# SunYangtian/UniGeo

Hardware: AMD Instinct MI355X
Metric: frames/sec (384x512, 25-frame clip, 25 denoise steps) (higher is better)
Workload: dtype fp16; 1 GPU; DepthCrafter SVD-UNet fp16, 25-step Euler, 25-frame 384x512 clips (BASELINE configs[1]); CLIP + VAE enc/dec + depth post-proc inside the timed region; one clip per ug_dc_run call, one call at a time (SURVEY 8d; reference eval.py:33-39); frames=25, height=384, width=512, denoise_steps=25, parallelism=clip-sharded x1, RCCL all_gather of depth, clips_in_flight_per_gpu=1, lanes=1

## Files before the change

### unigeo_amd/_lib.py

```python
import ctypes as C
import dataclasses
import json
import os

import numpy as np

_HERE = os.path.dirname(os.path.abspath(__file__))
LIB_PATH = os.environ.get("UG_LIB_PATH") or os.path.join(_HERE, "csrc", "libunigeo_hip.so")

EXPORTS = [
    "ug_unet_config_default", "ug_vae_config_default", "ug_clip_config_default",
    "ug_create", "ug_destroy", "ug_last_error", "ug_workspace_peak",
    "ug_load_tensor", "ug_bind_unet", "ug_bind_vae", "ug_bind_clip",
    "ug_dc_set_inputs", "ug_dc_run", "ug_dc_run_windows", "ug_dc_get_outputs", "ug_dc_device_ptrs", "ug_dc_set_trace", "ug_dc_set_guidance", "ug_unet_forward_pair", "ug_dc_set_inputs_ex", "ug_dc_get_noise", "ug_op_philox_u32", "ug_op_randn", "ug_op_u8_to_frames", "ug_set_vae_encode_fp32", "ug_set_concurrency", "ug_set_coscheduled", "ug_set_fp8_linears", "ug_op_linear_mx8", "ug_set_ff_fused", "ug_op_ff", "ug_op_ln_ff", "ug_bench_ff", "ug_bench_flash", "ug_tune_flash", "ug_tune_ff",
    "ug_eval_depth", "ug_eval_normal", "ug_depth_eval_opts_default", "ug_eval_depth_ex", "ug_op_masked_median", "ug_clip_embed", "ug_vae_encode", "ug_vae_decode", "ug_unet_forward", "ug_normals_from_depth",
    "ug_op_linear", "ug_op_conv", "ug_op_conv_gn", "ug_op_groupnorm", "ug_op_layernorm", "ug_op_flash_attn",
    "ug_op_temporal_attn", "ug_op_attention_generic", "ug_op_flash_attn_dh", "ug_op_euler_step",
    "ug_bind_stablenormal", "ug_sn_run", "ug_sn_unet_forward", "ug_sn_dino", "ug_sn_vae_decode", "ug_sn_vae_encode", "ug_resize_bilinear",
    "ug_profile_begin", "ug_profile_begin_shapes", "ug_profile_end", "ug_bench_gemm", "ug_bench_groupnorm", "ug_bench_mfma_peak", "ug_tune_force",
]


class UNetConfigC(C.Structure):
    _fields_ = [("in_channels", C.c_int), ("out_channels", C.c_int), ("num_levels", C.c_int),
                ("block_out_channels", C.c_int * 8), ("num_attention_heads", C.c_int * 8),
                ("down_has_attn", C.c_int * 8),
                ("layers_per_block", C.c_int), ("cross_attention_dim", C.c_int),
                ("addition_time_embed_dim", C.c_int), ("projection_class_embeddings_input_dim", C.c_int),
                ("norm_groups", C.c_int),
                ("eps_cross_attn_blocks", C.c_float), ("eps_plain_down_block", C.c_float),
                ("eps_mid_block", C.c_float), ("eps_up_blocks", C.c_float)]


class VAEConfigC(C.Structure):
    _fields_ = [("in_channels", C.c_int), ("out_channels", C.c_int), ("latent_channels", C.c_int),
                ("num_levels", C.c_int), ("block_out_channels", C.c_int * 8),
                ("layers_per_block", C.c_int), ("norm_groups", C.c_int), ("scaling_factor", C.c_float)]


class CLIPConfigC(C.Structure):
    _fields_ = [("hidden_size", C.c_int), ("intermediate_size", C.c_int), ("num_hidden_layers", C.c_int),
                ("num_attention_heads", C.c_int), ("image_size", C.c_int), ("patch_size", C.c_int),
                ("projection_dim", C.c_int), ("layer_norm_eps", C.c_float)]


class DepthEvalOptsC(C.Structure):
    _fields_ = [("alignment", C.c_int), ("max_depth", C.c_float), ("pre_clip_min", C.c_float), ("pre_clip_max", C.c_float),
                ("post_clip_min", C.c_float), ("post_clip_max", C.c_float)]


DEPTH_ALIGNMENTS = {"lstsq": 0, "median": 1, "scale": 2, "metric": 3}

_lib = None


def load_library():
    global _lib
    if _lib is not None:
        return _lib
    if not os.path.exists(LIB_PATH):
        raise RuntimeError(
            f"{LIB_PATH} not found: build it with `python -c 'import __graft_entry__ as g; g.build()'` "
            "(or `make -C unigeo_amd/csrc`).  The MI355X path has no CPU / PyTorch fallback.")
    lib = C.CDLL(LIB_PATH)
    fp, ip, vp = C.POINTER(C.c_float), C.c_int, C.c_void_p
    lib.ug_create.restype = vp
    lib.ug_create.argtypes = [ip, C.c_size_t, C.c_size_t]
    lib.ug_destroy.argtypes = [vp]
    lib.ug_last_error.restype = C.c_char_p
    lib.ug_last_error.argtypes = [vp]
    lib.ug_workspace_peak.restype = C.c_size_t
    lib.ug_workspace_peak.argtypes = [vp]
    lib.ug_load_tensor.argtypes = [vp, C.c_char_p, ip, ip, C.POINTER(C.c_int64), vp]
    lib.ug_bind_unet.argtypes = [vp, C.POINTER(UNetConfigC)]
    lib.ug_bind_vae.argtypes = [vp, C.POINTER(VAEConfigC)]
    lib.ug_bind_clip.argtypes = [vp, C.POINTER(CLIPConfigC)]
    lib.ug_dc_set_inputs.argtypes = [vp, vp, ip, ip, ip, vp, vp, vp]
    lib.ug_dc_run.argtypes = [vp, ip, ip, ip]
    lib.ug_dc_run_windows.argtypes = [vp, ip, ip, ip, ip, ip]
    lib.ug_dc_get_outputs.argtypes = [vp, vp, vp, vp]
    lib.ug_dc_set_trace.argtypes = [vp, vp, ip]
    lib.ug_set_vae_encode_fp32.argtypes = [vp, ip]
    try:
        lib.ug_set_fp8_linears.argtypes = [vp, ip]
        lib.ug_set_concurrency.argtypes = [vp, ip]
        lib.ug_set_coscheduled.argtypes = [vp, ip]
        lib.ug_set_ff_fused.argtypes = [vp, ip]
        lib.ug_bench_ff.argtypes = [vp, ip, ip, ip, ip, vp]
        lib.ug_bench_flash.argtypes = [vp, ip, ip, ip, ip, ip, vp]
        lib.ug_tune_flash.argtypes = [vp, ip]
        lib.ug_tune_ff.argtypes = [vp, ip]
        lib.ug_op_ff.argtypes = [vp, vp, ip, ip, vp, vp, vp, vp, vp, C.c_float, C.c_float, ip, vp]
        lib.ug_op_ln_ff.argtypes = [vp, vp, ip, ip, vp, vp, C.c_float, vp, ip, vp, vp, vp, vp, C.c_float, C.c_float, ip, vp]
        lib.ug_op_linear_mx8.argtypes = [vp, vp, ip, ip, vp, ip, vp, ip, vp, vp, vp]
    except AttributeError:
        if not os.environ.get("UG_LIB_PATH"):
            raise
    lib.ug_dc_device_ptrs.argtypes = [vp, C.POINTER(vp), C.POINTER(vp), C.POINTER(vp)]
    lib.ug_eval_depth.argtypes = [vp, vp, vp, vp, C.c_long, C.c_float, vp]
    lib.ug_eval_normal.argtypes = [vp, vp, vp, vp, C.c_long, vp]
    lib.ug_depth_eval_opts_default.restype = None
    lib.ug_depth_eval_opts_default.argtypes = [C.POINTER(DepthEvalOptsC)]
    lib.ug_eval_depth_ex.argtypes = [vp, vp, vp, vp, C.c_long, C.POINTER(DepthEvalOptsC), vp, vp]
    lib.ug_op_masked_median.argtypes = [vp, vp, vp, C.c_long, C.c_float, C.c_float, C.c_float, vp, C.POINTER(C.c_long)]
    lib.ug_clip_embed.argtypes = [vp, vp, ip, ip, ip, vp]
    lib.ug_vae_encode.argtypes = [vp, vp, ip, ip, ip, vp]
    lib.ug_vae_decode.argtypes = [vp, vp, ip, ip, ip, vp]
    lib.ug_unet_forward.argtypes = [vp, vp, ip, ip, ip, C.c_float, vp, vp]
    try:
        lib.ug_dc_set_guidance.argtypes = [vp, C.c_float]
        lib.ug_unet_forward_pair.argtypes = [vp, vp, vp, vp, vp, ip, ip, ip, C.c_float, vp, vp]
    except AttributeError:
        if not os.environ.get("UG_LIB_PATH"):
            raise
    try:
        lib.ug_dc_set_inputs_ex.argtypes = [vp, vp, ip, ip, ip, ip, vp, vp, C.c_uint64, vp]
        lib.ug_dc_get_noise.argtypes = [vp, vp, vp]
        lib.ug_op_philox_u32.argtypes = [vp, C.c_uint64, C.c_uint32, C.c_uint64, C.c_long, vp]
        lib.ug_op_randn.argtypes = [vp, C.c_uint64, C.c_uint32, C.c_uint64, C.c_long, C.c_long, vp]
        lib.ug_op_u8_to_frames.argtypes = [vp, vp, ip, ip, ip, vp]
    except AttributeError:
        if not os.environ.get("UG_LIB_PATH"):
            raise
    lib.ug_normals_from_depth.argtypes = [vp, vp, vp, ip, ip, ip, vp]
    lib.ug_op_linear.argtypes = [vp, vp, ip, ip, vp, ip, vp, vp, C.c_float, C.c_float, ip, ip, vp]
    lib.ug_op_conv.argtypes = [vp, vp, ip, vp, ip, ip, ip, ip, vp, vp, ip, ip, ip, ip, ip, ip, ip, vp]
    lib.ug_op_groupnorm.argtypes = [vp, vp, ip, vp, ip, ip, ip, ip, C.c_float, ip, ip, vp, vp, vp]
    lib.ug_op_conv_gn.argtypes = [vp, vp, ip, ip, ip, ip, vp, vp, vp, ip, ip, ip, ip, C.c_float, ip, vp, vp, vp, vp, vp, vp]
    lib.ug_op_layernorm.argtypes = [vp, vp, ip, ip, C.c_float, vp, vp, vp, ip, vp, vp]
    lib.ug_op_flash_attn.argtypes = [vp, vp, ip, ip, ip, vp]
    lib.ug_op_temporal_attn.argtypes = [vp, vp, ip, ip, ip, vp]
    lib.ug_op_attention_generic.argtypes = [vp, vp, ip, ip, ip, ip, vp]
    lib.ug_op_flash_attn_dh.argtypes = [vp, vp, ip, ip, ip, ip, vp]
    lib.ug_op_euler_step.argtypes = [vp, vp, vp, C.c_long, C.c_float, C.c_float]
    lib.ug_bind_stablenormal.argtypes = [vp, C.POINTER(UNetConfigC), C.POINTER(VAEConfigC), C.POINTER(CLIPConfigC)]
    lib.ug_sn_run.argtypes = [vp, vp, ip, ip, ip, vp, C.c_float, ip, vp, vp, vp, vp]
    lib.ug_sn_unet_forward.argtypes = [vp, ip, vp, vp, ip, ip, ip, C.c_float, C.c_float, vp, vp, ip, vp]
    lib.ug_sn_dino.argtypes = [vp, vp, ip, ip, ip, vp]
    lib.ug_sn_vae_decode.argtypes = [vp, vp, ip, ip, ip, vp]
    lib.ug_sn_vae_encode.argtypes = [vp, vp, ip, ip, ip, vp]
    lib.ug_resize_bilinear.argtypes = [vp, vp, ip, ip, ip, ip, ip, ip, ip, vp]
    lib.ug_profile_begin.argtypes = [vp]
    lib.ug_bench_gemm.argtypes = [vp] + [ip] * 16 + [vp]
    lib.ug_bench_groupnorm.argtypes = [vp, ip, ip, ip, ip, ip, ip, ip, vp]
    lib.ug_tune_force.argtypes = [vp, ip, ip]
    lib.ug_profile_begin_shapes.argtypes = [vp]
    lib.ug_profile_end.restype = C.c_char_p
    lib.ug_profile_end.argtypes = [vp]
    _lib = lib
    return lib


def _f32(a):
    return np.ascontiguousarray(a, dtype=np.float32)


def _ptr(a):
    return None if a is None else a.ctypes.data_as(C.c_void_p)


def _fill8(dst, vals):
    for i in range(8):
        dst[i] = int(vals[i]) if i < len(vals) else 0


class Engine:

    def __init__(self, device_id=0, workspace_bytes=2 << 30, persist_bytes=1 << 30):
        self.lib = load_library()
        self.ctx = self.lib.ug_create(int(device_id), int(workspace_bytes), int(persist_bytes))
        if not self.ctx:
            raise RuntimeError("ug_create failed: " + self.lib.ug_last_error(None).decode())
        self.device_id = device_id

    def close(self):
        if getattr(self, "ctx", None):
            self.lib.ug_destroy(self.ctx)
            self.ctx = None

    def __del__(self):
        try:
            self.close()
        except Exception:
            pass

    def _ck(self, rc):
        if rc != 0:
            raise RuntimeError("libunigeo_hip: " + self.lib.ug_last_error(self.ctx).decode())

    def load_state(self, prefix, state):
        for name, arr in state.items():
            a = np.ascontiguousarray(arr)
            if a.dtype == np.float16:
                dt = 0
            elif a.dtype == np.float32:
                dt = 1
            else:
                a = a.astype(np.float32); dt = 1
            shape = (C.c_int64 * max(a.ndim, 1))(*(a.shape if a.ndim else (1,)))
            self._ck(self.lib.ug_load_tensor(self.ctx, (prefix + name).encode(), dt, max(a.ndim, 1), shape, _ptr(a)))

    def bind_unet(self, cfg):
        c = UNetConfigC()
        c.in_channels, c.out_channels = cfg.in_channels, cfg.out_channels
        c.num_levels = len(cfg.block_out_channels)
        _fill8(c.block_out_channels, cfg.block_out_channels)
# ... 274 lines not shown
        k = _f32(intrinsics).reshape(T, 3, 3)
        out = np.empty((T, H, W, 3), np.float32)
        self._ck(self.lib.ug_normals_from_depth(self.ctx, _ptr(d), _ptr(k), T, H, W, _ptr(out)))
        return out

    DEPTH_KEYS = ["Abs Rel", "Sq Rel", "RMSE", "Log RMSE", "delta < 1.", "delta < 1.25", "delta < 1.25^2", "delta < 1.25^3"]
    NORMAL_KEYS = ["normal mean", "normal median", "normal rmse", "angle < 5", "angle < 7.5", "angle < 11.25", "angle < 22.5", "angle < 30"]

    def eval_depth(self, gt, mask=None, pred=None, max_depth=80.0, alignment="lstsq", pre_clip_min=None, pre_clip_max=None,
                   post_clip_min=None, post_clip_max=None, return_error_map=False):
        if alignment not in DEPTH_ALIGNMENTS:
            raise ValueError(f"alignment must be one of {sorted(DEPTH_ALIGNMENTS)}, not {alignment!r}")
        g = _f32(gt); n = g.size
        p = None if pred is None else _f32(pred)
        m = None if mask is None else np.ascontiguousarray(np.asarray(mask).astype(np.uint8))
        out = np.zeros(11, np.float64)
        clips = (pre_clip_min, pre_clip_max, post_clip_min, post_clip_max)
        emap = None
        if alignment == "lstsq" and max_depth is not None and not return_error_map and all(c is None for c in clips):
            self._ck(self.lib.ug_eval_depth(self.ctx, _ptr(p), _ptr(g), _ptr(m), n, float(max_depth), _ptr(out)))
        else:
            o = DepthEvalOptsC(DEPTH_ALIGNMENTS[alignment], float("nan") if max_depth is None else float(max_depth),
                               *[float("nan") if c is None else float(c) for c in clips])
            emap = np.empty(g.shape, np.float32) if return_error_map else None
            self._ck(self.lib.ug_eval_depth_ex(self.ctx, _ptr(p), _ptr(g), _ptr(m), n, C.byref(o), _ptr(out), _ptr(emap)))
        res = dict(zip(self.DEPTH_KEYS, out[:8].tolist()))
        res["valid_pixels"] = int(out[8])
        if return_error_map:
            return res, (float(out[9]), float(out[10])), emap
        return res, (float(out[9]), float(out[10]))

    def op_masked_median(self, pred, gt, max_depth=80.0, pre_clip_min=None, pre_clip_max=None):
        p, g = _f32(pred).reshape(-1), _f32(gt).reshape(-1)
        med = np.zeros(2, np.float32); cnt = C.c_long(0)
        nan = float("nan")
        self._ck(self.lib.ug_op_masked_median(self.ctx, _ptr(p), _ptr(g), p.size, nan if max_depth is None else float(max_depth),
                                              nan if pre_clip_min is None else float(pre_clip_min),
                                              nan if pre_clip_max is None else float(pre_clip_max), _ptr(med), C.byref(cnt)))
        return med[0], med[1], int(cnt.value)

    def eval_normal(self, gt, mask=None, pred=None):
        g = _f32(gt); n = g.size // 3
        p = None if pred is None else _f32(pred)
        m = None if mask is None else np.ascontiguousarray(np.asarray(mask).astype(np.uint8))
        out = np.zeros(8, np.float64)
        self._ck(self.lib.ug_eval_normal(self.ctx, _ptr(p), _ptr(g), _ptr(m), n, _ptr(out)))
        return dict(zip(self.NORMAL_KEYS, out.tolist()))

    def op_linear(self, A, W, bias=None, R1=None, c0=1.0, c1=1.0, act=0, geglu=False):
        A, W = _f32(A), _f32(W); M, K = A.shape; N = W.shape[0]
        b = None if bias is None else _f32(bias); r = None if R1 is None else _f32(R1)
        out = np.empty((M, N // 2 if geglu else N), np.float32)
        self._ck(self.lib.ug_op_linear(self.ctx, _ptr(A), M, K, _ptr(W), N, _ptr(b), _ptr(r), c0, c1, act, int(geglu), _ptr(out)))
        return out

    def op_conv(self, x0, weight, bias=None, x1=None, kt=1, k=3, stride=1, pad_t=1, pad_l=1, ups=1):
        x0 = _f32(x0); T, H, W, C0 = x0.shape
        x1a = None if x1 is None else _f32(x1); C1 = 0 if x1 is None else x1a.shape[-1]
        w = _f32(weight); O = w.shape[0]
        b = None if bias is None else _f32(bias)
        Ho, Wo = H * ups // stride, W * ups // stride
        out = np.empty((T, Ho, Wo, O), np.float32)
        self._ck(self.lib.ug_op_conv(self.ctx, _ptr(x0), C0, _ptr(x1a), C1, T, H, W, _ptr(w), _ptr(b), O, kt, k,
                                     stride, pad_t, pad_l, ups, _ptr(out)))
        return out

    def op_groupnorm(self, x0, G, eps, gamma, beta, x1=None, temporal=False, silu=False):
        x0 = _f32(x0); T, HW, C0 = x0.shape
        x1a = None if x1 is None else _f32(x1); C1 = 0 if x1 is None else x1a.shape[-1]
        out = np.empty((T, HW, C0 + C1), np.float32)
        self._ck(self.lib.ug_op_groupnorm(self.ctx, _ptr(x0), C0, _ptr(x1a), C1, T, HW, G, eps, int(temporal), int(silu),
                                          _ptr(_f32(gamma)), _ptr(_f32(beta)), _ptr(out)))
        return out

    def op_conv_gn(self, x, w, b, G, eps, gamma, beta, res=None, kt=1, k=3, temporal=False):
        x = _f32(x); T, H, W, C0 = x.shape; w = _f32(w); O = w.shape[0]
        r = None if res is None else _f32(res)
        co = np.empty((T, H, W, O), np.float32); y1 = np.empty_like(co); y2 = np.empty_like(co)
        rb = C.c_int(0)
        self._ck(self.lib.ug_op_conv_gn(self.ctx, _ptr(x), C0, T, H, W, _ptr(w), _ptr(None if b is None else _f32(b)), _ptr(r), O, kt, k, G, eps, int(temporal),
                                        _ptr(_f32(gamma)), _ptr(_f32(beta)), _ptr(co), _ptr(y1), _ptr(y2), C.byref(rb)))
        return co, y1, y2, rb.value

    def op_layernorm(self, x, eps, gamma, beta, addvec=None, rows_per_vec=1):
        x = _f32(x); M, Cc = x.shape
        out = np.empty((M, Cc), np.float32); xout = np.empty((M, Cc), np.float32)
        av = None if addvec is None else _f32(addvec)
        self._ck(self.lib.ug_op_layernorm(self.ctx, _ptr(x), M, Cc, eps, _ptr(_f32(gamma)), _ptr(_f32(beta)), _ptr(av),
                                          rows_per_vec, _ptr(out), _ptr(xout)))
        return (out, xout) if addvec is not None else out

    def op_flash_attn(self, qkv, B, H, S):
        q = _f32(qkv); out = np.empty((B * S, H * 64), np.float32)
        self._ck(self.lib.ug_op_flash_attn(self.ctx, _ptr(q), B, H, S, _ptr(out)))
        return out

    def op_temporal_attn(self, qkv, T, HW, H):
        q = _f32(qkv); out = np.empty((T * HW, H * 64), np.float32)
        self._ck(self.lib.ug_op_temporal_attn(self.ctx, _ptr(q), T, HW, H, _ptr(out)))
        return out

    def op_attention_generic(self, qkv, B, S, H, d):
        q = _f32(qkv); out = np.empty((B * S, H * d), np.float32)
        self._ck(self.lib.ug_op_attention_generic(self.ctx, _ptr(q), B, S, H, d, _ptr(out)))
        return out

    def op_flash_attn_dh(self, qkv, B, S, H, d):
        q = _f32(qkv); out = np.empty((B * S, H * d), np.float32)
        self._ck(self.lib.ug_op_flash_attn_dh(self.ctx, _ptr(q), B, S, H, d, _ptr(out)))
        return out

    def op_euler_step(self, v, lat, sigma, sigma_next):
        v = _f32(v); l = _f32(lat).copy()
        self._ck(self.lib.ug_op_euler_step(self.ctx, _ptr(v), _ptr(l), l.size, sigma, sigma_next))
        return l

    def bench_gemm(self, M=0, N=0, K=0, conv=None, cfg=-1, split=0, iters=20):
        out = np.zeros(8, np.float32)
        cv = conv or {}
        self._ck(self.lib.ug_bench_gemm(self.ctx, M, N, K, int(conv is not None), cv.get("T", 0), cv.get("H", 0), cv.get("W", 0),
                                        cv.get("C0", 0), cv.get("C1", 0), cv.get("kt", 1), cv.get("k", 1), cv.get("stride", 1),
                                        cv.get("ups", 1), cfg, split, iters, _ptr(out)))
        Mr, Kr = float(out[3]), float(out[4])
        return float(out[0]), 2.0 * Mr * N * Kr / (out[0] * 1e-3) / 1e12, int(out[1]), int(out[2])

    def bench_mfma_peak(self, iters=20000):
        out = np.zeros(1, np.float32)
        self.lib.ug_bench_mfma_peak.argtypes = [C.c_void_p, C.c_int, C.c_void_p]
        self._ck(self.lib.ug_bench_mfma_peak(self.ctx, int(iters), _ptr(out)))
        return float(out[0])

    def tune_force(self, cfg=-1, split=-1):
        self._ck(self.lib.ug_tune_force(self.ctx, int(cfg), int(split)))

    def bench_groupnorm(self, C0, C1, T, HW, temporal, mode, iters=20):
        out = np.zeros(1, np.float32)
        self._ck(self.lib.ug_bench_groupnorm(self.ctx, C0, C1, T, HW, int(temporal), mode, iters, _ptr(out)))
        return float(out[0])

    def profile_begin(self, shapes=False):
        self._ck((self.lib.ug_profile_begin_shapes if shapes else self.lib.ug_profile_begin)(self.ctx))

    def profile_end(self):
        prof = json.loads(self.lib.ug_profile_end(self.ctx).decode())
        self.last_profile_order = prof.pop("__order__", None)
        return prof

    def workspace_peak(self):
        return int(self.lib.ug_workspace_peak(self.ctx))
```

### unigeo_amd/csrc/capi.hip

```cpp
#include <math.h>
#include <stdlib.h>
#include <string.h>

#include <algorithm>
#include <cmath>
#include <vector>

#include "../../include/unigeo_hip.h"
#include "../../include/unigeo_hip_test.h"
#include "engine.h"

using namespace ug;

struct ug_ctx { Ctx c; };
static std::string g_create_err;

#define UG_TRY(ctx, ...)                                   \
  if (!(ctx)) return -1;                                   \
  try { UG_CHECK(hipSetDevice((ctx)->c.device)); __VA_ARGS__; return 0; } \
  catch (const std::exception& e) { (ctx)->c.err = e.what(); (void)hipGetLastError(); return 1; } \
  catch (...) { (ctx)->c.err = "unknown error"; return 2; }

extern "C" {

// ... 761 lines not shown
    f16* dO = c.ws.get<f16>((long)M * nout);
    GemmP p; memset(&p, 0, sizeof(p));
    p.A0 = (const f16*)a8; p.C0 = K; p.M = M; p.N = N; p.K = K; p.W = (const f16*)w8; p.ldw = K; p.bias = db; p.c0 = 1.f;
    p.Out = dO; p.ldo = nout; p.flags = geglu ? UG_F_GEGLU : 0; p.zero = c.zero; p.nb_inner = 1;
    p.sa = sa; p.ld_sa = ld_sa; p.sw = sw; p.ld_sw = ld_sw;
    gemm_apply_tune(p, c.tune);
    launch_gemm_mx8(p, c.stream);
    down16(c, dO, out, (long)M * nout);
    if (a8_out) UG_CHECK(hipMemcpy(a8_out, a8, (size_t)M * K, hipMemcpyDeviceToHost));
    if (sa_out) UG_CHECK(hipMemcpy(sa_out, sa, (size_t)(K / 128) * ld_sa * 4, hipMemcpyDeviceToHost));
  });
}

int ug_op_conv(ug_ctx* x, const float* x0, int C0, const float* x1, int C1, int T, int H, int W, const float* weight,
               const float* bias, int O, int kt, int k, int stride, int pad_t, int pad_l, int ups, float* out) {
  UG_TRY(x, {
    Ctx& c = x->c; Scope sc(c);
    const int I = C0 + C1, taps = kt * k * k;
    std::vector<float> wp((size_t)O * taps * I);
    const bool kch = (I % 64 == 0) && taps > 1 && !getenv("UG_NO_KCHUNK");
    for (int o = 0; o < O; ++o) for (int i = 0; i < I; ++i) for (int tp = 0; tp < taps; ++tp)
      wp[kch ? (((size_t)o * (I / 64) + i / 64) * taps + tp) * 64 + i % 64 : ((size_t)o * taps + tp) * I + i] = weight[((size_t)o * I + i) * taps + tp];
    const long px = (long)T * H * W;
    f16* d0 = up16(c, x0, px * C0); f16* d1 = C1 ? up16(c, x1, px * C1) : nullptr;
    f16* dW = up16(c, wp.data(), (long)wp.size()); f16* db = up16_opt(c, bias, O);
    const int Ho = H * ups / stride, Wo = W * ups / stride;
    f16* dO = c.ws.get<f16>((long)T * Ho * Wo * O);
    GemmP p; memset(&p, 0, sizeof(p));
    p.conv = 1; p.A0 = d0; p.A1 = d1; p.C0 = C0; p.C1 = C1; p.T = T; p.Hi = H; p.Wi = W; p.Ho = Ho; p.Wo = Wo;
    p.ups = ups; p.stride = stride; p.pad_t = pad_t; p.pad_l = pad_l; p.kt = kt; p.ky = k; p.kx = k;
    p.M = T * Ho * Wo; p.N = O; p.K = I * taps; p.W = dW; p.ldw = p.K; p.bias = db; p.c0 = 1.f;
    p.Out = dO; p.ldo = O; p.zero = c.zero; p.nb_inner = 1; p.kchunk = kch;
    gemm_apply_tune(p, c.tune);
    { int cf, sp; gemm_plan(p, 1, &cf, &sp); p.cfg_p1 = cf + 1; p.splitk = sp; if (sp > 1) p.partial = c.ws.get<float>((long)sp * p.M * p.N); }
    launch_gemm(p, 1, c.stream);
    down16(c, dO, out, (long)T * Ho * Wo * O);
  });
}

int ug_op_conv_gn(ug_ctx* x, const float* x0, int C0, int T, int H, int W, const float* weight, const float* bias, const float* res, int O, int kt, int k,
                  int G, float eps, int temporal, const float* gamma, const float* beta, float* conv_out, float* y_pass, float* y_epi, int* rb_out) {
  UG_TRY(x, {
    Ctx& c = x->c; Scope sc(c);
    const int I = C0, taps = kt * k * k;
    UG_REQUIRE(I % 64 == 0, "ug_op_conv_gn: channels must be a multiple of 64");
    std::vector<float> wp((size_t)O * taps * I);
    for (int o = 0; o < O; ++o) for (int i = 0; i < I; ++i) for (int tp = 0; tp < taps; ++tp)
      wp[(((size_t)o * (I / 64) + i / 64) * taps + tp) * 64 + i % 64] = weight[((size_t)o * I + i) * taps + tp];
    const long M = (long)T * H * W;
    f16* d0 = up16(c, x0, M * C0); f16* dW = up16(c, wp.data(), (long)wp.size()); f16* db = up16_opt(c, bias, O);
    f16* dR = up16_opt(c, res, M * O);
    f16* dg = up16(c, gamma, O); f16* dbt = up16(c, beta, O);
    f16* o1 = c.ws.get<f16>(M * O); f16* o2 = c.ws.get<f16>(M * O); f16* y1 = c.ws.get<f16>(M * O); f16* y2 = c.ws.get<f16>(M * O);
    float2* part = (float2*)c.ws.get<float>(((M + 47) / 48) * (long)O * 2);
    int rb = 0;
    for (int pass = 0; pass < 2; ++pass) {
      GemmP p; memset(&p, 0, sizeof(p));
      p.conv = 1; p.A0 = d0; p.C0 = C0; p.T = T; p.Hi = H; p.Wi = W; p.Ho = H; p.Wo = W;
      p.ups = 1; p.stride = 1; p.pad_t = k / 2; p.pad_l = k / 2; p.kt = kt; p.ky = k; p.kx = k;
      p.M = (int)M; p.N = O; p.K = I * taps; p.W = dW; p.ldw = p.K; p.bias = db; p.c0 = 1.f; p.R1 = dR; p.ldr1 = O; p.c1 = 1.f;
      p.Out = pass ? o2 : o1; p.ldo = O; p.zero = c.zero; p.nb_inner = 1; p.kchunk = taps > 1;
      gemm_apply_tune(p, c.tune);
      const size_t mk = c.ws.mark();
      { int cf, sp; gemm_plan(p, 1, &cf, &sp); p.cfg_p1 = cf + 1; p.splitk = sp; if (sp > 1) p.partial = c.ws.get<float>((long)sp * p.M * p.N); }
      if (pass) { p.stat_part = part; p.stat_hw = H * W; launch_gemm(p, 1, c.stream, &rb); } else launch_gemm(p, 1, c.stream);
      c.ws.release(mk);
      GroupNormP g; memset(&g, 0, sizeof(g));
      g.X0 = pass ? o2 : o1; g.C0 = O; g.T = T; g.HW = H * W; g.G = G; g.eps = eps; g.temporal = temporal; g.silu = 1; g.gamma = dg; g.beta = dbt;
      g.Y = pass ? y2 : y1; g.ws = c.ws.get<float>((long)groupnorm_ws_floats(T, H * W, O, G));
      if (pass && rb > 0) { g.part = part; g.part_rb = rb; }
      const bool used = launch_groupnorm(g, c.stream);
      if (pass && !used) rb = 0;
      c.ws.release(mk);
    }
    *rb_out = rb;
    down16(c, o1, conv_out, M * O);
    std::vector<float> tmp((size_t)M * O);
    down16(c, o2, tmp.data(), M * O);
    UG_REQUIRE(memcmp(tmp.data(), conv_out, tmp.size() * 4) == 0, "ug_op_conv_gn: the statistics epilogue changed the convolution's output");
    down16(c, y1, y_pass, M * O); down16(c, y2, y_epi, M * O);
  });
}

int ug_op_groupnorm(ug_ctx* x, const float* x0, int C0, const float* x1, int C1, int T, int HW, int G, float eps,
                    int temporal, int silu, const float* gamma, const float* beta, float* out) {
  UG_TRY(x, {
    Ctx& c = x->c; Scope sc(c);
    const int C = C0 + C1; const long M = (long)T * HW;
    GroupNormP p; memset(&p, 0, sizeof(p));
    p.X0 = up16(c, x0, M * C0); p.X1 = C1 ? up16(c, x1, M * C1) : nullptr; p.C0 = C0; p.C1 = C1;
    p.T = T; p.HW = HW; p.G = G; p.eps = eps; p.temporal = temporal; p.silu = silu;
    p.gamma = up16(c, gamma, C); p.beta = up16(c, beta, C);
    f16* y = c.ws.get<f16>(M * C); p.Y = y;
    p.ws = c.ws.get<float>((long)groupnorm_ws_floats(T, HW, C, G));
    launch_groupnorm(p, c.stream);
    down16(c, y, out, M * C);
  });
}

int ug_bench_groupnorm(ug_ctx* x, int C0, int C1, int T, int HW, int temporal, int mode, int iters, float* us_out) {
  UG_TRY(x, {
    Ctx& c = x->c; Scope sc(c);
    const int C = C0 + C1; const long M = (long)T * HW;
    GroupNormP p; memset(&p, 0, sizeof(p));
    f16* a0 = c.ws.get<f16>(M * C0); f16* a1 = C1 ? c.ws.get<f16>(M * C1) : nullptr;
    launch_fill_random(a0, M * C0, 1, c.stream); if (C1) launch_fill_random(a1, M * C1, 2, c.stream);
    f16* gm = c.ws.get<f16>(C); f16* bt = c.ws.get<f16>(C);
    launch_fill_random(gm, C, 3, c.stream); launch_fill_random(bt, C, 4, c.stream);
    p.X0 = a0; p.X1 = a1; p.C0 = C0; p.C1 = C1; p.T = T; p.HW = HW; p.G = 32; p.eps = 1e-5f; p.temporal = temporal; p.silu = 1;
    p.gamma = gm; p.beta = bt; p.Y = c.ws.get<f16>(M * C); p.mode = mode;
    p.ws = c.ws.get<float>((long)groupnorm_ws_floats(T, HW, C, 32));
    for (int i = 0; i < 3; ++i) launch_groupnorm(p, c.stream);
    hipEvent_t e0, e1; UG_CHECK(hipEventCreate(&e0)); UG_CHECK(hipEventCreate(&e1));
    UG_CHECK(hipEventRecord(e0, c.stream));
    for (int i = 0; i < iters; ++i) launch_groupnorm(p, c.stream);
    UG_CHECK(hipEventRecord(e1, c.stream)); UG_CHECK(hipEventSynchronize(e1));
    float ms; UG_CHECK(hipEventElapsedTime(&ms, e0, e1));
    (void)hipEventDestroy(e0); (void)hipEventDestroy(e1);
    us_out[0] = ms * 1000.f / iters;
  });
}

int ug_op_layernorm(ug_ctx* x, const float* xin, int M, int C, float eps, const float* gamma, const float* beta,
                    const float* addvec, int rows_per_vec, float* out, float* xout) {
  UG_TRY(x, {
    Ctx& c = x->c; Scope sc(c);
    LayerNormP p; memset(&p, 0, sizeof(p));
    p.X = up16(c, xin, (long)M * C); p.M = M; p.C = C; p.eps = eps; p.gamma = up16(c, gamma, C); p.beta = up16(c, beta, C);
    f16* y = c.ws.get<f16>((long)M * C); p.Y = y;
    f16* xo = nullptr;
    if (addvec) {
      const int nv = (M + rows_per_vec - 1) / rows_per_vec;
      p.addvec = up16(c, addvec, (long)nv * C); p.rows_per_vec = rows_per_vec;
      xo = c.ws.get<f16>((long)M * C); p.Xout = xo;
    }
    launch_layernorm(p, c.stream);
    down16(c, y, out, (long)M * C);
    if (xo && xout) down16(c, xo, xout, (long)M * C);
  });
}

int ug_op_flash_attn(ug_ctx* x, const float* qkv, int B, int H, int S, float* out) {
  UG_TRY(x, {
    Ctx& c = x->c; Scope sc(c);
    const int C = H * 64; const long M = (long)B * S;
    f16* d = up16(c, qkv, M * 3 * C); f16* o = c.ws.get<f16>(M * C);
    FlashP p; p.Q = d; p.K = d + C; p.V = d + 2 * C; p.ldq = p.ldk = p.ldv = 3 * C; p.O = o; p.ldo = C; p.variant = c.flash_variant;
    p.B = B; p.H = H; p.S = S; p.scale = 0.125f;
    launch_flash_attn64(p, c.stream);
    down16(c, o, out, M * C);
  });
}

int ug_op_temporal_attn(ug_ctx* x, const float* qkv, int T, int HW, int H, float* out) {
  UG_TRY(x, {
    Ctx& c = x->c; Scope sc(c);
    const int C = H * 64; const long M = (long)T * HW;
    f16* d = up16(c, qkv, M * 3 * C); f16* o = c.ws.get<f16>(M * C);
    TemporalAttnP p; p.Q = d; p.K = d + C; p.V = d + 2 * C; p.ld = 3 * C; p.O = o; p.ldo = C;
    p.T = T; p.HW = HW; p.H = H; p.scale = 0.125f;
    launch_temporal_attn64(p, c.stream);
    down16(c, o, out, M * C);
  });
}

int ug_op_attention_generic(ug_ctx* x, const float* qkv, int B, int S, int H, int d, float* out) {
// ... 152 lines not shown
```

### unigeo_amd/csrc/common.h

```cpp
#pragma once
#include <hip/hip_runtime.h>
#include <hip/hip_fp16.h>
#include <stdint.h>
#include <stdio.h>
#include <stdexcept>
#include <string>

typedef _Float16 f16;
typedef _Float16 f16x2 __attribute__((ext_vector_type(2)));
typedef _Float16 f16x4 __attribute__((ext_vector_type(4)));
typedef _Float16 f16x8 __attribute__((ext_vector_type(8)));
typedef float f32x4 __attribute__((ext_vector_type(4)));
typedef float f32x16 __attribute__((ext_vector_type(16)));

#define UG_CHECK(expr)                                                                        \
  do {                                                                                        \
    hipError_t _e = (expr);                                                                   \
    if (_e != hipSuccess)                                                                     \
      throw std::runtime_error(std::string(#expr) + " failed: " + hipGetErrorString(_e) +    \
                               " at " + __FILE__ + ":" + std::to_string(__LINE__));           \
  } while (0)

#define UG_REQUIRE(cond, msg)                                                                 \
  do {                                                                                        \
    if (!(cond))                                                                              \
      throw std::runtime_error(std::string("requirement failed: ") + #cond + " : " + (msg) + \
                               " at " + __FILE__ + ":" + std::to_string(__LINE__));           \
  } while (0)

static inline int cdiv(long a, long b) { return (int)((a + b - 1) / b); }
static inline int ug_dev_slot() { int d = 0; (void)hipGetDevice(&d); return d & 31; }

enum { UG_ACT_NONE = 0, UG_ACT_SILU = 1, UG_ACT_GELU = 2 };
enum { UG_F_GEGLU = 1, UG_F_OUT_F32 = 2, UG_F_NOXCD = 4, UG_F_PRIO = 8 ,
       UG_F_XCDROUND = 32 ,
       UG_F_R1_F32 = 16  };

struct GemmP {
  const f16* A0; const f16* A1;
  int C0, C1;
  int M, N, K;
  int conv;
  int T, Hi, Wi, Ho, Wo;
  int ups, stride, pad_t, pad_l;
  int kt, ky, kx;
  const f16* W; long ldw;
  const f16* bias; const f16* bias2;
  const f16* R1; long ldr1; float c1;
  const f16* R2; long ldr2; float c2;
  float c0;
  void* Out; long ldo;
  int act, flags;
  const f16* zero;
  int nb_inner;
  long sA_o, sA_i, sW_o, sW_i, sO_o, sO_i;
  int cfg_p1;
  int splitk;
  float* partial;
  void* trace;
  int up_phase;
  const unsigned* sa; const unsigned* sw; long ld_sa, ld_sw;
  int kchunk;
  int tm_T, tm_nb;
  int m_off;
  int group_m;
  int halo_tw, halo_lg;
  int tune_cfg_p1, tune_split_p1, tune_knobs;
  float2* stat_part; int stat_hw;
};
struct GemmTune { int cfg = -1, split = -1, knobs = 0; };
static inline void gemm_apply_tune(GemmP& p, const GemmTune& t) { p.tune_cfg_p1 = t.cfg + 1; p.tune_split_p1 = t.split + 1; p.tune_knobs = t.knobs; }
void launch_gemm_mx8(const GemmP& p, hipStream_t s);
void launch_quant_mx8(const f16* x, long ldx, long M, int K, unsigned char* q, unsigned* scales, long ld_s, hipStream_t s);
void launch_gemm(const GemmP& p, int batch, hipStream_t s, int* stat_rb = nullptr);
bool gemm_stream_supported(const GemmP& p, int batch);
void launch_gemm_stream(const GemmP& p, hipStream_t s);
bool conv_halo_supported(const GemmP& p, int batch, int bm, int bn);
void launch_conv_halo(const GemmP& p, int bm, int bn, hipStream_t s);
void gemm_plan(const GemmP& p, int batch, int* cfg_out, int* split_out);

struct FFusedP {
  const f16* X; const f16* W1; const f16* b1; const f16* W2; const f16* b2;
  const f16* R1; const f16* R2; float c0, c1, c2;
  f16* Out; int M, C; const f16* zero;
  const f16* ln_g; const f16* ln_b; float ln_eps; const f16* addvec; int rows_per_vec;
  int variant;
};
bool ff_fused_supported(int C);
void launch_ff_fused(const FFusedP& p, hipStream_t s);

struct GroupNormP {
  const f16* X0; const f16* X1; int C0, C1;
  int T, HW, G; float eps; int temporal; int silu;
  const f16* gamma; const f16* beta;
  f16* Y;
  float* ws;
  int mode;
  const float2* part; int part_rb;
};
bool launch_groupnorm(const GroupNormP& p, hipStream_t s);
bool groupnorm_uses_part(const GroupNormP& p, int part_rb);
size_t groupnorm_ws_floats(int T, int HW, int C, int G);

struct LayerNormP {
  const f16* X; f16* Y; int M, C; float eps;
  const f16* gamma; const f16* beta;
  const f16* addvec; int rows_per_vec; f16* Xout;
  long row0;
  unsigned char* Y8; unsigned* S8; long ld_s8;
};
void launch_layernorm(const LayerNormP& p, hipStream_t s);

struct FlashP {
  const f16* Q; const f16* K; const f16* V; long ldq, ldk, ldv;
  f16* O; long ldo;
  int B, H, S; float scale;
  int Sk = 0; int kv_shared = 0;
  int variant = -1;
};
void launch_flash_attn64(const FlashP& p, hipStream_t s);
bool flash_attn_dh_supported(int d);
void launch_flash_attn_dh(const FlashP& p, int d, hipStream_t s);

struct TemporalAttnP {
  const f16* Q; const f16* K; const f16* V; long ld;
  f16* O; long ldo;
  int T, HW, H; float scale;
  int nv = 1;
};
void launch_temporal_attn64(const TemporalAttnP& p, hipStream_t s);

void launch_softmax_rows(const float* in, long ld_in, f16* out, long ld_out, long rows, int S,
                         hipStream_t s);
void launch_transpose(const f16* in, long ldi, long sbi, f16* out, long ldo, long sbo, int B, int R,
                      int C, int nb_inner, long sbi_inner, long sbo_inner, hipStream_t s);

void launch_cast_f32_f16(const float* in, f16* out, long n, hipStream_t s);
void launch_cast_f16_f32(const f16* in, float* out, long n, hipStream_t s);
void launch_permute_conv_w(const f16* in, f16* out, int O, int I, int taps, int Ipad, int Opad,
                           hipStream_t s);
void launch_upsample_phase_w(const f16* w9, f16* w4, int O, int I, int Ipad, hipStream_t s);
void launch_rechunk_conv_w(const f16* in, f16* out, long O, int taps, int Ipad, hipStream_t s);
void launch_gather_rows(const f16* in, f16* out, const int* rowmap, int rows, int cols, hipStream_t s);
void launch_copy2d(const f16* in, long ldi, f16* out, long ldo, long rows, int cols, hipStream_t s);
void launch_fill_f16(f16* p, float v, long n, hipStream_t s);
void launch_fill_random(f16* p, long n, unsigned seed, hipStream_t s);
void launch_add_rowvec(const f16* x, const f16* vec, f16* y, long M, int C, int rows_per_vec,
                       hipStream_t s);
void launch_axpby(const f16* a, const f16* b, f16* y, float ca, float cb, long n, hipStream_t s);

void launch_prep_video(const float* frames, const float* noise, f16* clip_src, f16* vae_in,
                       int T, int H, int W, float noise_aug, hipStream_t s);
void launch_clip_patchify(const f16* video_m11, f16* patches, int T, int H, int W, int S224,
                          int P, int Kpad, hipStream_t s, int imagenet_norm = 0);
void launch_scale_rows(f16* w, const f16* gamma, int N, int K, hipStream_t s);
void launch_add_grid_nearest(f16* x, const f16* grid, int B, int h, int w, int g, int C, hipStream_t s);
void launch_sn_normals_out(const f16* dec, int ldd, float* out, long pixels, hipStream_t s);
void launch_resize_bilinear_aa(const float* in, float* out, int B, int Hi, int Wi, int Ho, int Wo, int C, int normalise, hipStream_t s);
void launch_init_latents2(const float* noise, f16* lat, float sigma0, int T, long hw, hipStream_t s);
void launch_silu_f16(const f16* in, f16* out, long n, hipStream_t s);
void launch_clip_assemble(const f16* patches, const f16* cls, const f16* pos, f16* tok, int T, int np, int d,
                          hipStream_t s);
void launch_make_unet_input(const f16* lat, const f16* cond, f16* x, long pixels, float inv_scale,
                            hipStream_t s);
void launch_euler_step(const f16* v, f16* lat, long n, float sigma, float sigma_next, hipStream_t s);
void launch_make_unet_input_cfg(const f16* lat, const f16* cond, f16* x, long pixels, float inv_scale, hipStream_t s);
void launch_euler_step_cfg(const f16* vc, const f16* vu, float g, f16* lat, long n, float sigma, float sigma_next, hipStream_t s);
void launch_scale_f16(const f16* in, f16* out, float sc, long n, hipStream_t s);
void launch_axpby_f16(const f16* x, float a, const f16* y, float b, f16* out, long n, hipStream_t s);
void launch_crossfade_f16(const f16* cur, f16* all, long frame_elems, int overlap, hipStream_t s);
void launch_pad_channels(const f16* in, int Cin, f16* out, int Cout, long pixels, hipStream_t s);
void launch_time_conv_out(const f16* x, const f16* w, const f16* b, float* frames_out, int T,
                          long HW, int Cs, hipStream_t s);
void launch_depth_post(const float* frames, float* depth, float* minmax_ws, long pixels,
                       hipStream_t s);
void launch_normals(const float* depth, const float* K33, float* normals, int T, int H, int W,
                    hipStream_t s);

void launch_philox_u32(uint32_t* out, long nblocks, uint64_t seed, uint32_t stream, uint64_t q0, hipStream_t s);
void launch_randn(float* out, long n, uint64_t seed, uint32_t stream, uint64_t e0, hipStream_t s);
void launch_u8_to_frames(const unsigned char* in_tchw, float* out_thwc, int T, long HW, hipStream_t s);

void launch_split_pair(const float* x, f16* y, long M, int C, hipStream_t s);
void launch_add_f32(const float* a, const float* b, float* y, long n, hipStream_t s);
void launch_take_cols_f16(const float* x, long ldx, f16* y, long M, int C, hipStream_t s);
// ... 27 lines not shown
```

### unigeo_amd/csrc/engine.hip

```cpp
#include "engine.h"
#include <chrono>

#include <math.h>
#include <stdlib.h>
#include <string.h>

#include <algorithm>
#include <exception>
#include <sstream>

namespace ug {

void Arena::init(size_t bytes) {
  UG_CHECK(hipMalloc((void**)&base_, bytes));
  cap_ = bytes; off_ = 0; peak_ = 0;
}
void Arena::destroy() { if (base_) (void)hipFree(base_); base_ = nullptr; cap_ = 0; }
void* Arena::alloc(size_t bytes) {
  const size_t a = (bytes + 255) & ~(size_t)255;
  if (off_ + a > cap_)
    throw std::runtime_error("device arena exhausted: need " + std::to_string(off_ + a) + " bytes, capacity " +
                             std::to_string(cap_) + " (raise workspace_bytes / persist_bytes in ug_create)");
  void* p = base_ + off_;
  off_ += a;
// ... 74 lines not shown
  for (int i : order) { const int l = (int)(std::min_element(load.begin(), load.end()) - load.begin()); plan[l].push_back(i); load[l] += need[i] + 1; }
  try {
    for (size_t k = 0;; ++k) {
      bool any = false;
      for (int l = 0; l < nl; ++l) {
        if (k >= plan[l].size()) continue;
        any = true;
        c.stream = c.lanes[l].stream;
        c.ws.view(base + (size_t)l * slice, slice);
        c.cur_lane = l + 1;
        body(plan[l][k]);
      }
      if (!any) break;
    }
  } catch (...) {
    c.stream = main_stream; c.ws = main_ws; c.cur_lane = 0;
    for (int l = 0; l < nl; ++l) (void)hipStreamSynchronize(c.lanes[l].stream);
    c.ws.release(mk);
    throw;
  }
  c.stream = main_stream; c.ws = main_ws; c.cur_lane = 0;
  for (int l = 0; l < nl; ++l) {
    UG_CHECK(hipEventRecord(c.lanes[l].done, c.lanes[l].stream));
    UG_CHECK(hipStreamWaitEvent(main_stream, c.lanes[l].done, 0));
  }
  c.ws.release(mk);
}

struct ProfScope {
  Ctx& c; int idx = -1;
  ProfScope(Ctx& c_, const char* name, double flops, double bytes) : c(c_) {
    if (!c.prof_on) return;
    ProfRec r; r.name = name; r.flops = flops; r.bytes = bytes;
    UG_CHECK(hipEventCreate(&r.e0)); UG_CHECK(hipEventCreate(&r.e1));
    UG_CHECK(hipEventRecord(r.e0, c.stream));
    c.prof.push_back(r); idx = (int)c.prof.size() - 1;
  }
  ~ProfScope() { if (idx >= 0) (void)hipEventRecord(c.prof[idx].e1, c.stream); }
};
void prof_begin(Ctx& c, bool shapes) { c.prof.clear(); c.prof_on = true; c.prof_shapes = shapes; }
std::string prof_end(Ctx& c) {
  c.prof_on = false;
  UG_CHECK(hipStreamSynchronize(c.stream));
  struct Agg { double ms = 0, flops = 0, bytes = 0; long calls = 0; };
  std::map<std::string, Agg> agg;
  for (auto& r : c.prof) {
    float ms = 0.f;
    UG_CHECK(hipEventElapsedTime(&ms, r.e0, r.e1));
    Agg& a = agg[r.name]; a.ms += ms; a.flops += r.flops; a.bytes += r.bytes; a.calls++;
    (void)hipEventDestroy(r.e0); (void)hipEventDestroy(r.e1);
  }
  std::ostringstream o;
  o << "{";
  bool first = true;
  if (c.prof_shapes) {
    o << "\"__order__\":[";
    bool f2 = true;
    for (auto& r : c.prof) {
      if (r.name.compare(0, 5, "gemm_") != 0) continue;
      if (!f2) o << ",";
      f2 = false;
      o << "[\"" << r.name << "\"," << r.bytes << "]";
    }
    o << "]";
    first = false;
  }
  c.prof.clear();
  for (auto& kv : agg) {
    if (!first) o << ",";
    first = false;
    o << "\"" << kv.first << "\":{\"ms\":" << kv.second.ms << ",\"calls\":" << kv.second.calls
      << ",\"flops\":" << kv.second.flops << ",\"bytes\":" << kv.second.bytes << "}";
  }
  o << "}";
  return o.str();
}

struct Epi {
  const f16* bias2 = nullptr; const f16* R1 = nullptr; long ldr1 = 0; float c1 = 1.f;
  const f16* R2 = nullptr; long ldr2 = 0; float c2 = 1.f; float c0 = 1.f; int act = 0; int flags = 0;
  const unsigned char* a8 = nullptr; const unsigned* sa8 = nullptr; long ld_sa8 = 0;
  float alg = 1.f;
  struct StatPart* so = nullptr; int stat_hw = 0;
};
struct StatPart { float2* part = nullptr; int rb = 0; };
static StatPart stat_alloc(Ctx& c, long M, int N, int T, int hw, int G, int temporal) {
  StatPart s;
  GroupNormP g; memset(&g, 0, sizeof(g));
  g.C0 = N; g.T = T; g.HW = hw; g.G = G; g.temporal = temporal; g.gamma = c.zero; g.beta = c.zero;
  if (!(c.tune.knobs & 131072) && M >= 8192 && N % G == 0 && groupnorm_uses_part(g, 16))
    s.part = (float2*)c.ws.get<float>(((M + 47) / 48) * (long)N * 2);
  return s;
}

static void run_gemm(Ctx& c, GemmP p, int batch, const char* tag, float alg = 1.f, StatPart* so = nullptr, int stat_hw = 0) {
  p.zero = c.zero;
  gemm_apply_tune(p, c.tune);
  if (p.nb_inner < 1) p.nb_inner = 1;
  char nm[128];
  if (c.prof_on && c.prof_shapes) snprintf(nm, sizeof(nm), "%s:%dx%dx%d%s", tag, p.M, p.N, p.K, batch > 1 ? "b" : "");
  else snprintf(nm, sizeof(nm), "%s", tag);
  int cfg, split;
  gemm_plan(p, batch, &cfg, &split);
  p.cfg_p1 = cfg + 1; p.splitk = split;
  const size_t mk = c.ws.mark();
  if (split > 1) p.partial = c.ws.get<float>((long)split * p.M * p.N);
  {
    const double nout = (p.flags & UG_F_GEGLU) ? p.N / 2 : p.N;
    const double a_el = p.conv ? (double)p.T * p.Hi * p.Wi * (p.C0 + p.C1) : (double)p.M * p.K;
    const double bytes = 2.0 * batch * (a_el + (double)p.N * p.K + (double)p.M * nout * ((p.flags & UG_F_OUT_F32) ? 2 : 1) +
                                        (p.R1 ? (double)p.M * nout : 0.0) + (p.R2 ? (double)p.M * nout : 0.0));
    ProfScope ps(c, nm, 2.0 * p.M * p.N * (double)p.K * batch * (p.up_phase ? 2.25 : 1.0) * alg, bytes);
    if (so && so->part) { p.stat_part = so->part; p.stat_hw = p.conv ? p.Ho * p.Wo : stat_hw; }
    launch_gemm(p, batch, c.stream, so && so->part ? &so->rb : nullptr);
  }
  c.ws.release(mk);
}

void* pinned(Ctx& c, int slot, size_t bytes) {
  if (c.pin_sz[slot] < bytes) {
    if (c.pin[slot]) UG_CHECK(hipHostFree(c.pin[slot]));
    c.pin[slot] = nullptr; c.pin_sz[slot] = 0;
    UG_CHECK(hipHostMalloc(&c.pin[slot], bytes, hipHostMallocDefault));
    c.pin_sz[slot] = bytes;
  }
  return c.pin[slot];
}

static inline long pad256(long x) { return (x + 255) / 256 * 256; }
static void linear(Ctx& c, const f16* A, long M, const Lin& l, f16* out, const Epi& e = Epi(), long lda = 0,
                   long ldo = 0) {
  GemmP p; memset(&p, 0, sizeof(p));
  if (c.fp8_linears && l.w8 && M >= 256 && !(e.flags & UG_F_OUT_F32)) {
    const size_t mk = c.ws.mark();
    const int K = l.in;
    const unsigned char* a8 = e.a8; const unsigned* sa = e.sa8; long ld_sa = e.ld_sa8;
    unsigned char* a8w = nullptr; unsigned* saw = nullptr;
    if (!a8) {
      a8w = (unsigned char*)c.ws.alloc((size_t)M * K);
      ld_sa = pad256(M);
      saw = (unsigned*)c.ws.alloc((size_t)(K / 128) * ld_sa * 4);
      a8 = a8w; sa = saw;
    }
    char nmq[96], nmg[96];
    if (c.prof_on && c.prof_shapes) { snprintf(nmq, sizeof(nmq), "quant_mx8:%ldx%d", M, K); snprintf(nmg, sizeof(nmg), "gemm_linear_mx8:%ldx%dx%d", M, l.out, K); }
    else { snprintf(nmq, sizeof(nmq), "quant_mx8"); snprintf(nmg, sizeof(nmg), "gemm_linear_mx8"); }
    if (a8w) {
      ProfScope ps(c, nmq, 0, (double)M * K * 3.0);
      launch_quant_mx8(A, lda ? lda : K, M, K, a8w, saw, ld_sa, c.stream);
    }
    p.A0 = (const f16*)a8; p.C0 = K; p.M = (int)M; p.N = l.out; p.K = K;
    p.W = (const f16*)l.w8; p.ldw = K; p.bias = l.b; p.bias2 = e.bias2;
    p.R1 = e.R1; p.ldr1 = e.ldr1; p.c1 = e.c1; p.R2 = e.R2; p.ldr2 = e.ldr2; p.c2 = e.c2; p.c0 = e.c0;
    p.act = e.act; p.flags = e.flags;
    const int nout = (e.flags & UG_F_GEGLU) ? l.out / 2 : l.out;
    p.Out = out; p.ldo = ldo ? ldo : nout;
    if (p.R1 && !p.ldr1) p.ldr1 = nout;
    if (p.R2 && !p.ldr2) p.ldr2 = nout;
    p.sa = sa; p.ld_sa = ld_sa; p.sw = l.sw8; p.ld_sw = l.ld_sw8; p.zero = c.zero; p.nb_inner = 1;
    gemm_apply_tune(p, c.tune);
    {
      ProfScope ps(c, nmg, 2.0 * M * (double)l.out * K, (double)M * K + (double)l.out * K + 2.0 * M * nout);
      launch_gemm_mx8(p, c.stream);
    }
    c.ws.release(mk);
    return;
  }
  p.A0 = A; p.C0 = (int)(lda ? lda : l.in); p.M = (int)M; p.N = l.out; p.K = l.in;
  p.W = l.w; p.ldw = l.in; p.bias = l.b; p.bias2 = e.bias2;
  p.R1 = e.R1; p.ldr1 = e.ldr1; p.c1 = e.c1; p.R2 = e.R2; p.ldr2 = e.ldr2; p.c2 = e.c2; p.c0 = e.c0;
  p.act = e.act; p.flags = e.flags;
  const int nout = (e.flags & UG_F_GEGLU) ? l.out / 2 : l.out;
  p.Out = out; p.ldo = ldo ? ldo : nout;
  if (p.R1 && !p.ldr1) p.ldr1 = nout;
  if (p.R2 && !p.ldr2) p.ldr2 = nout;
  run_gemm(c, p, 1, "gemm_linear", e.alg, e.so, e.stat_hw);
}

static void conv(Ctx& c, const f16* x0, int C0, const f16* x1, int C1, int T, int Hi, int Wi, const Conv& cv,
                 int stride, int pad_t, int pad_l, int ups, f16* out, const Epi& e = Epi(), long ldo = 0) {
  UG_REQUIRE(C0 + C1 == cv.cinp, "conv input channels do not match the bound weight");
  if (ups == 2 && cv.wphase && stride == 1 && pad_t == 1 && pad_l == 1) {
    for (int ph = 0; ph < 4; ++ph) {
      GemmP p; memset(&p, 0, sizeof(p));
      p.conv = 1; p.A0 = x0; p.A1 = x1; p.C0 = C0; p.C1 = C1;
      p.T = T; p.Hi = Hi; p.Wi = Wi; p.ups = 1; p.stride = 1; p.pad_t = (ph >> 1) ? 0 : 1; p.pad_l = (ph & 1) ? 0 : 1;
      p.kt = 1; p.ky = 2; p.kx = 2; p.Ho = Hi; p.Wo = Wi;
      p.M = T * Hi * Wi; p.N = cv.cout; p.K = cv.cinp * 4;
      p.W = cv.wphase + (long)ph * cv.cout * 4 * cv.cinp; p.ldw = p.K; p.bias = cv.b; p.bias2 = e.bias2;
      p.c0 = e.c0; p.act = e.act; p.flags = e.flags; p.Out = out; p.ldo = ldo ? ldo : cv.cout; p.up_phase = 1 + ph; p.kchunk = cv.kchunk;
      UG_REQUIRE(!e.R1 && !e.R2, "sub-pixel upsample conv does not take residuals");
      run_gemm(c, p, 1, "gemm_conv_up2x2");
    }
    return;
  }
  GemmP p; memset(&p, 0, sizeof(p));
  p.conv = 1; p.A0 = x0; p.A1 = x1; p.C0 = C0; p.C1 = C1;
  p.T = T; p.Hi = Hi; p.Wi = Wi; p.ups = ups; p.stride = stride; p.pad_t = pad_t; p.pad_l = pad_l;
  p.kt = cv.kt; p.ky = cv.ky; p.kx = cv.kx;
  p.Ho = (Hi * ups) / stride; p.Wo = (Wi * ups) / stride;
  p.M = T * p.Ho * p.Wo; p.N = cv.cout; p.K = cv.cinp * cv.kt * cv.ky * cv.kx;
  p.W = cv.w; p.ldw = p.K; p.bias = cv.b; p.bias2 = e.bias2;
  p.R1 = e.R1; p.ldr1 = e.ldr1 ? e.ldr1 : cv.cout; p.c1 = e.c1;
  p.R2 = e.R2; p.ldr2 = e.ldr2 ? e.ldr2 : cv.cout; p.c2 = e.c2; p.c0 = e.c0; p.act = e.act; p.flags = e.flags;
  p.Out = out; p.ldo = ldo ? ldo : cv.cout; p.kchunk = cv.kchunk;
  run_gemm(c, p, 1, cv.kt > 1 ? "gemm_tconv" : (cv.ky > 1 ? "gemm_conv3x3" : "gemm_conv1x1"), e.alg, e.so);
}

static void groupnorm(Ctx& c, const f16* x0, int C0, const f16* x1, int C1, int T, int HW, int G, const Norm& n,
                      int temporal, int silu, f16* y, const StatPart* sp = nullptr) {
  UG_REQUIRE(C0 + C1 == n.c, "groupnorm channel mismatch");
  GroupNormP p; memset(&p, 0, sizeof(p));
  if (sp && sp->part && sp->rb > 0 && C1 == 0 && HW % sp->rb == 0) { p.part = sp->part; p.part_rb = sp->rb; }
  p.X0 = x0; p.X1 = x1; p.C0 = C0; p.C1 = C1; p.T = T; p.HW = HW; p.G = G; p.eps = n.eps;
  p.temporal = temporal; p.silu = silu; p.gamma = n.g; p.beta = n.b; p.Y = y;
  const size_t mk = c.ws.mark();
  p.ws = c.ws.get<float>((long)groupnorm_ws_floats(T, HW, n.c, G));
  {
    char nm[96];
    if (c.prof_on && c.prof_shapes) snprintf(nm, sizeof(nm), "groupnorm:T%dxHW%dxC%d%s", T, HW, n.c, temporal ? "t" : "");
    else snprintf(nm, sizeof(nm), "groupnorm");
    ProfScope ps(c, nm, 0, (double)T * HW * n.c * 2.0 * 3.0);
    const bool from_part = launch_groupnorm(p, c.stream);
    if (from_part && ps.idx >= 0 && c.prof_shapes) c.prof[ps.idx].name += ":ep";
  }
  c.ws.release(mk);
}

struct QAct { unsigned char* a8 = nullptr; unsigned* sa = nullptr; long ld = 0; };
static QAct qact_alloc(Ctx& c, long M, int K) {
  QAct q; q.a8 = (unsigned char*)c.ws.alloc((size_t)M * K); q.ld = pad256(M);
  q.sa = (unsigned*)c.ws.alloc((size_t)(K / 128) * q.ld * 4);
  return q;
}
static void layernorm(Ctx& c, const f16* x, long M, const Norm& n, f16* y, const f16* addvec = nullptr,
                      long rows_per_vec = 1, f16* xout = nullptr, const QAct* q = nullptr, long row0 = 0) {
  LayerNormP p; memset(&p, 0, sizeof(p));
  p.X = x; p.Y = y; p.M = (int)M; p.C = n.c; p.eps = n.eps; p.gamma = n.g; p.beta = n.b;
  p.addvec = addvec; p.rows_per_vec = (int)rows_per_vec; p.Xout = xout; p.row0 = row0;
  if (q) { p.Y8 = q->a8; p.S8 = q->sa; p.ld_s8 = q->ld; }
  ProfScope ps(c, "layernorm", 0, (double)M * n.c * 2.0 * (addvec ? 3.0 : 2.0));
  launch_layernorm(p, c.stream);
}


void upload_raw(Ctx& c, const std::string& name, int dtype, const std::vector<long>& shape, const void* host) {
  UG_REQUIRE(dtype == 0 || dtype == 1, "dtype must be 0 (fp16) or 1 (fp32)");
  RawTensor t; t.dtype = dtype; t.shape = shape; t.numel = 1;
  for (long d : shape) t.numel *= d;
  const size_t bytes = (size_t)t.numel * (dtype == 0 ? 2 : 4);
  UG_CHECK(hipMalloc(&t.dev, bytes ? bytes : 4));
  UG_CHECK(hipMemcpy(t.dev, host, bytes, hipMemcpyHostToDevice));
  auto it = c.raw.find(name);
  if (it != c.raw.end()) { (void)hipFree(it->second.dev); c.raw.erase(it); }
  c.raw[name] = t;
}

static RawTensor& raw_get(Ctx& c, const std::string& name, std::initializer_list<long> shape) {
  auto it = c.raw.find(name);
  if (it == c.raw.end()) throw std::runtime_error("missing weight tensor: " + name);
  RawTensor& t = it->second;
  std::vector<long> want(shape);
  if (t.shape != want) {
    std::string s = "weight " + name + " has shape [";
    for (long d : t.shape) s += std::to_string(d) + ",";
    s += "] expected [";
    for (long d : want) s += std::to_string(d) + ",";
    throw std::runtime_error(s + "]");
  }
  t.used = true;
  return t;
}

static const f16* raw_f16(Ctx& c, RawTensor& t, bool copy) {
  if (t.dtype == 0 && !copy) return (const f16*)t.dev;
  f16* d = c.persist.get<f16>(t.numel);
  if (t.dtype == 0) UG_CHECK(hipMemcpyAsync(d, t.dev, (size_t)t.numel * 2, hipMemcpyDeviceToDevice, c.stream));
  else launch_cast_f32_f16((const float*)t.dev, d, t.numel, c.stream);
  return d;
}
static const f16* persist_f16(Ctx& c, RawTensor& t) { return raw_f16(c, t, true); }

static float raw_scalar(Ctx& c, const std::string& name) {
  RawTensor& t = raw_get(c, name, {1});
  UG_CHECK(hipStreamSynchronize(c.stream));
  if (t.dtype == 1) { float v; UG_CHECK(hipMemcpy(&v, t.dev, 4, hipMemcpyDeviceToHost)); return v; }
  uint16_t h; UG_CHECK(hipMemcpy(&h, t.dev, 2, hipMemcpyDeviceToHost));
  f16 hv; memcpy(&hv, &h, 2);
  return (float)hv;
}

static Norm bind_norm(Ctx& c, const std::string& p, int ch, float eps) {
  Norm n; n.c = ch; n.eps = eps;
  n.g = persist_f16(c, raw_get(c, p + ".weight", {ch}));
  n.b = persist_f16(c, raw_get(c, p + ".bias", {ch}));
  return n;
}
static Lin bind_lin(Ctx& c, const std::string& p, int in, int out, bool bias) {
  Lin l; l.in = in; l.out = out;
  l.w = persist_f16(c, raw_get(c, p + ".weight", {out, in}));
  l.b = bias ? persist_f16(c, raw_get(c, p + ".bias", {out})) : nullptr;
  return l;
}
static Lin bind_lin_cat(Ctx& c, const std::vector<std::string>& ps, int in, int out_each, bool bias) {
  Lin l; l.in = in; l.out = out_each * (int)ps.size();
  f16* w = c.persist.get<f16>((long)l.out * in);
  f16* b = bias ? c.persist.get<f16>(l.out) : nullptr;
  for (size_t i = 0; i < ps.size(); ++i) {
    RawTensor& t = raw_get(c, ps[i] + ".weight", {out_each, in});
// ... 336 lines not shown
  {
    RawTensor& t = raw_get(c, v + "embeddings.patch_embedding.weight", {d, 3, P, P});
    const int K = 3 * P * P; m.patch_k = pad8(K);
    f16* w = c.persist.get<f16>((long)d * m.patch_k);
    const size_t mk = c.persist.mark();
    launch_permute_conv_w(raw_f16(c, t, false), w, d, K, 1, m.patch_k, d, c.stream);
    UG_CHECK(hipStreamSynchronize(c.stream));
    c.persist.release(mk);
    m.patch_w = w;
  }
  m.pre = bind_norm(c, v + "pre_layrnorm", d, cfg.eps);
  for (int i = 0; i < cfg.layers; ++i) {
    const std::string p = v + "encoder.layers." + std::to_string(i);
    CLIPLayer l;
    l.ln1 = bind_norm(c, p + ".layer_norm1", d, cfg.eps);
    l.qkv = bind_lin_cat(c, {p + ".self_attn.q_proj", p + ".self_attn.k_proj", p + ".self_attn.v_proj"}, d, d, true);
    l.out = bind_lin(c, p + ".self_attn.out_proj", d, d, true);
    l.ln2 = bind_norm(c, p + ".layer_norm2", d, cfg.eps);
    l.fc1 = bind_lin(c, p + ".mlp.fc1", d, cfg.inter, true);
    l.fc2 = bind_lin(c, p + ".mlp.fc2", cfg.inter, d, true);
    m.layers.push_back(l);
  }
  m.post = bind_norm(c, v + "post_layernorm", d, cfg.eps);
  m.proj = bind_lin(c, pre + "visual_projection", d, cfg.proj, false);
  m.bound = true;
}

void finish_binding(Ctx& c, const std::string& prefix) {
  UG_CHECK(hipStreamSynchronize(c.stream));
  std::vector<std::string> unused;
  for (auto it = c.raw.begin(); it != c.raw.end();) {
    if (it->first.compare(0, prefix.size(), prefix) != 0) { ++it; continue; }
    const bool ignorable = it->first.size() >= 12 && it->first.compare(it->first.size() - 12, 12, "position_ids") == 0;
    if (!it->second.used && !ignorable) unused.push_back(it->first);
    (void)hipFree(it->second.dev);
    it = c.raw.erase(it);
  }
  if (!unused.empty()) {
    std::string s = "unexpected tensors in state dict (architecture restatement mismatch): ";
    for (size_t i = 0; i < unused.size() && i < 8; ++i) s += unused[i] + " ";
    throw std::runtime_error(s + "(" + std::to_string(unused.size()) + " total)");
  }
}

static void unfused_attention(Ctx& c, const f16* qkv, long ldqkv, int B, int S, int heads, int d, f16* out, long ldo) {
  const int Spad = pad8(S), C = heads * d;
  const size_t mk = c.ws.mark();
  float* sc = c.ws.get<float>((long)B * heads * S * Spad);
  f16* P = c.ws.get<f16>((long)B * heads * S * Spad);
  f16* Vt = c.ws.get<f16>((long)B * heads * d * Spad);
  GemmP p; memset(&p, 0, sizeof(p));
  p.A0 = qkv; p.C0 = (int)ldqkv; p.M = S; p.N = S; p.K = d; p.W = qkv + C; p.ldw = ldqkv;
  p.c0 = 1.0f / sqrtf((float)d); p.Out = sc; p.ldo = Spad; p.flags = UG_F_OUT_F32;
  p.nb_inner = heads; p.sA_o = (long)S * ldqkv; p.sA_i = d; p.sW_o = (long)S * ldqkv; p.sW_i = d;
  p.sO_o = (long)heads * S * Spad; p.sO_i = (long)S * Spad;
  run_gemm(c, p, B * heads, "gemm_attn_qk");
  {
    ProfScope ps(c, "softmax_rows", 0, (double)B * heads * S * Spad * 6.0);
    launch_softmax_rows(sc, Spad, P, Spad, (long)B * heads * S, S, c.stream);
  }
  {
    ProfScope ps(c, "transpose", 0, (double)B * heads * S * d * 4.0);
    launch_transpose(qkv + 2 * C, ldqkv, (long)S * ldqkv, Vt, Spad, (long)heads * d * Spad, B * heads, S, d, heads, d,
                     (long)d * Spad, c.stream);
  }
  GemmP q; memset(&q, 0, sizeof(q));
  q.A0 = P; q.C0 = Spad; q.M = S; q.N = d; q.K = Spad; q.W = Vt; q.ldw = Spad; q.c0 = 1.f;
  q.Out = out; q.ldo = ldo; q.nb_inner = heads;
  q.sA_o = (long)heads * S * Spad; q.sA_i = (long)S * Spad; q.sW_o = (long)heads * d * Spad; q.sW_i = (long)d * Spad;
  q.sO_o = (long)S * ldo; q.sO_i = d;
  run_gemm(c, q, B * heads, "gemm_attn_pv");
  c.ws.release(mk);
}

void test_unfused_attention(Ctx& c, const f16* qkv, long ld, int B, int S, int H, int d, f16* out, long ldo) {
  unfused_attention(c, qkv, ld, B, S, H, d, out, ldo);
}

static void res2d_forward(Ctx& c, const Res2D& r, const f16* x0, int C0, const f16* x1, int C1, int T, int h, int w,
                          int G, const f16* tproj, f16* out, StatPart* out_stats = nullptr, const StatPart* in_stats = nullptr) {
  const long M = (long)T * h * w;
  const int cin = C0 + C1, cout = r.c1.cout;
  const size_t mk = c.ws.mark();
  f16* a = c.ws.get<f16>(M * cin);
  groupnorm(c, x0, C0, x1, C1, T, h * w, G, r.n1, 0, 1, a, C1 == 0 ? in_stats : nullptr);
  f16* hb = c.ws.get<f16>(M * cout);
  StatPart sh = stat_alloc(c, M, cout, T, h * w, G, 0);
  { Epi e; e.bias2 = tproj; e.so = &sh; conv(c, a, cin, nullptr, 0, T, h, w, r.c1, 1, 1, 1, 1, hb, e); }
  f16* b = c.ws.get<f16>(M * cout);
  groupnorm(c, hb, cout, nullptr, 0, T, h * w, G, r.n2, 0, 1, b, &sh);
  const f16* res = x0;
  if (r.has_sc) {
    f16* scb = hb;
    conv(c, x0, C0, x1, C1, T, h, w, r.sc, 1, 0, 0, 1, scb);
    res = scb;
  } else {
    UG_REQUIRE(C1 == 0, "identity shortcut needs a single source");
  }
  { Epi e; e.R1 = res; e.ldr1 = cout; e.so = out_stats; conv(c, b, cout, nullptr, 0, T, h, w, r.c2, 1, 1, 1, 1, out, e); }
  c.ws.release(mk);
}

static f16* stres_forward(Ctx& c, const STRes& rb, const f16* x0, int C0, const f16* x1, int C1, int T, int h, int w,
                          int G, const f16* tproj_s, const f16* tproj_t, StatPart* out_stats = nullptr, const StatPart* in_stats = nullptr,
                          int nv = 1) {
  const long Mv = (long)T * h * w, M = nv * Mv;
  const int cout = rb.cout;
  f16* out = c.ws.get<f16>(M * cout);
  if (out_stats) *out_stats = stat_alloc(c, M, cout, nv * T, h * w, G, 0);
  const size_t mk = c.ws.mark();
  f16* xs = c.ws.get<f16>(M * cout);
  StatPart sx = stat_alloc(c, M, cout, T, h * w, G, 1), sh = stat_alloc(c, M, cout, T, h * w, G, 1);
  res2d_forward(c, rb.s, x0, C0, x1, C1, nv * T, h, w, G, tproj_s, xs, &sx, in_stats);
  auto view = [&](const StatPart& sp, int v) {
    StatPart r = sp;
    if (v > 0) { if (sp.part && sp.rb > 0 && Mv % sp.rb == 0) r.part = sp.part + v * (Mv / sp.rb) * cout; else r.rb = 0; }
    return r;
  };
  auto tconv = [&](const Conv& cv, const f16* in, f16* o, Epi e, StatPart* so) {
    if (nv == 1) { e.so = so; conv(c, in, cout, nullptr, 0, T, h, w, cv, 1, 0, 0, 1, o, e); return; }
    const f16* r1 = e.R1;
    int rb0 = 0;
    for (int v = 0; v < nv; ++v) {
      const long off = v * Mv * cout;
      StatPart sv;
      if (so && so->part) { sv.part = so->part; if (v > 0 && rb0 > 0 && Mv % rb0 == 0) sv.part += v * (Mv / rb0) * cout; }
      Epi ev = e; ev.so = (so && so->part) ? &sv : nullptr;
      if (r1) ev.R1 = r1 + off;
      conv(c, in + off, cout, nullptr, 0, T, h, w, cv, 1, 0, 0, 1, o + off, ev);
      if (v == 0) rb0 = sv.rb; else if (sv.rb != rb0) rb0 = 0;
    }
    if (so && so->part) so->rb = (rb0 > 0 && Mv % rb0 == 0) ? rb0 : 0;
  };
  f16* a = c.ws.get<f16>(M * cout);
  for (int v = 0; v < nv; ++v) { const StatPart sv = view(sx, v); groupnorm(c, xs + v * Mv * cout, cout, nullptr, 0, T, h * w, G, rb.t.n1, 1, 1, a + v * Mv * cout, &sv); }
  f16* hb = c.ws.get<f16>(M * cout);
  { Epi e; e.bias2 = tproj_t; tconv(rb.t.c1, a, hb, e, &sh); }
  for (int v = 0; v < nv; ++v) { const StatPart sv = view(sh, v); groupnorm(c, hb + v * Mv * cout, cout, nullptr, 0, T, h * w, G, rb.t.n2, 1, 1, a + v * Mv * cout, &sv); }
  { Epi e; e.c0 = 1.f - rb.alpha; e.R1 = xs; e.ldr1 = cout; e.c1 = 1.f; tconv(rb.t.c2, a, out, e, out_stats); }
  c.ws.release(mk);
  return out;
}

static bool ff_pair_fusable(const Ctx& c, long M, const Lin& f1, const Lin& f2, const Epi& e2) {
  const int C4 = f1.out / 2, C = f2.out;
  return (c.ff_fused & 1) && !c.fp8_linears && ff_fused_supported(C) && f1.in == C && C4 == 4 * C && M >= 32768 && f1.b && !e2.act && !e2.flags &&
         (!e2.R1 || !e2.ldr1 || e2.ldr1 == C) && (!e2.R2 || !e2.ldr2 || e2.ldr2 == C) && !e2.bias2;
}
struct PreNorm { const f16* g; const f16* b; float eps; const f16* addvec; long rows_per_vec; };
static long ff_fused_rows(const Ctx& c, long M) {
  const long ntile = (M + 127) / 128, full = ntile / 256 * 256, rem = ntile - full;
  static const bool nosplit = getenv("UG_FF_NOSPLIT") != nullptr;
  return (full > 0 && rem > 0 && rem <= 160 && !nosplit && !c.cosched) ? full * 128 : M;
}
static void ff_pair(Ctx& c, const f16* a, long M, const Lin& f1, const Lin& f2, f16* mid, f16* out, const Epi& e2, const QAct* q = nullptr,
                    const PreNorm* pre = nullptr, bool no_fuse = false) {
  const int C4 = f1.out / 2, C = f2.out;
  UG_REQUIRE(!pre || ff_pair_fusable(c, M, f1, f2, e2), "ff_pair: pre-norm only with the fused kernel");
  if (ff_pair_fusable(c, M, f1, f2, e2) && !no_fuse) {
    FFusedP p; memset(&p, 0, sizeof(p));
    p.X = a; p.W1 = f1.w; p.b1 = f1.b; p.W2 = f2.w; p.b2 = f2.b; p.R1 = e2.R1; p.R2 = e2.R2; p.c0 = e2.c0; p.c1 = e2.c1; p.c2 = e2.c2;
    p.Out = out; p.M = (int)M; p.C = C; p.zero = c.zero; p.variant = c.ff_variant;
    if (pre) { p.ln_g = pre->g; p.ln_b = pre->b; p.ln_eps = pre->eps; p.addvec = pre->addvec; p.rows_per_vec = (int)pre->rows_per_vec; }
    char nm[64];
    if (c.prof_on && c.prof_shapes) snprintf(nm, sizeof(nm), "gemm_ff_fused:%ldx%d", M, C); else snprintf(nm, sizeof(nm), "gemm_ff_fused");
    ProfScope ps(c, nm, 2.0 * M * (double)(2 * C4) * C + 2.0 * M * (double)C * C4,
                 2.0 * ((double)M * C * (2 + (e2.R1 ? 1 : 0) + (e2.R2 ? 1 : 0)) + 3.0 * (double)C4 * C));
    launch_ff_fused(p, c.stream);
    return;
  }
  const long bytes = M * C4 * 2;
  int nchunk = 1;
  if (bytes > (96L << 20) && getenv("UG_FF_CHUNK") && !q) nchunk = (int)((bytes + (48L << 20) - 1) / (48L << 20));
  const long rows = ((M + nchunk - 1) / nchunk + 255) / 256 * 256;
  for (long r0 = 0; r0 < M; r0 += rows) {
    const long m = std::min(rows, M - r0);
    { Epi e; e.flags = UG_F_GEGLU; if (q && nchunk == 1) { e.a8 = q->a8; e.sa8 = q->sa; e.ld_sa8 = q->ld; } linear(c, a + r0 * f1.in, m, f1, mid + r0 * C4, e); }
    Epi e = e2;
    if (e.R1) e.R1 += r0 * (e.ldr1 ? e.ldr1 : C);
    if (e.R2) e.R2 += r0 * (e.ldr2 ? e.ldr2 : C);
    linear(c, mid + r0 * C4, m, f2, out + r0 * C, e);
  }
// ... 735 lines not shown
```

### unigeo_amd/csrc/kernels/conv_halo.hip

```cpp
#include "gemm_common.h"
#include <algorithm>
#include <cstdlib>
#include <type_traits>

template <int BM, int BN, int LG, bool ST = false>
__global__ __launch_bounds__(12 * 64, 3) void conv_halo_kernel(const GemmP p) {
  constexpr int BK = 64, NCW = 8, WMW = 4, WNW = 2;
  constexpr unsigned SENT = 0x80000000u;
  constexpr int WTM = BM / WMW, WTN = BN / WNW;
  constexpr int MT = WTM / 16, NT = WTN / 16;
  constexpr int WID = 4 * NT;
  constexpr int LB = BN / 32;
  constexpr int WSLOT = BN * BK;
  constexpr int TW = 1 << LG, TH = BM >> LG;
  constexpr int PITCH = (TW + 2 + 7) & ~7;
  constexpr int GPR = PITCH / 8;
  constexpr int NG = (TH + 2) * GPR;
  constexpr int HALO = NG * 8 * BK;
  constexpr int HL = 2;
  constexpr int HSLOTS = 7 * HL;
  static_assert(TH * TW == BM && TW >= 16 && (NG + 3) / 4 <= HSLOTS, "tile geometry");
  static_assert((2 * HALO + 3 * WSLOT) * 2 <= 160 * 1024, "LDS");
  extern __shared__ __attribute__((aligned(16))) f16 smem[];
  f16* halo = smem;
  f16* ring = smem + 2 * HALO;

  const int tid = threadIdx.x, lane = tid & 63;
  const int wave = __builtin_amdgcn_readfirstlane(tid >> 6);
  const bool producer = wave >= NCW;
  const int ntn = (p.N + BN - 1) / BN, ntm = p.M / BM;
  const int ntiles = ntm * ntn;
  const int Cin = p.C0 + p.C1, nchunks = Cin / BK, nk = nchunks * 9;
  const int txn = p.Wo >> LG, tpf = (p.Ho / TH) * txn;

  const int nwg = gridDim.x, w = blockIdx.x;
  const TileWalk tw = tile_walk(p.flags, ntiles, nwg, w);
  const int my_tiles = tw.count;
  const int total_it = my_tiles * nk;

  auto tile_origin = [&](int tile, int& t, int& y0, int& x0, int& n0) {
    int tm, tn; tile_coord_p(p, tile, ntm, ntn, tm, tn);
    const int tmg = tm + p.m_off / BM;
    t = tmg / tpf;
    const int rem = tmg - t * tpf;
    const int tyi = rem / txn, txi = rem - tyi * txn;
    y0 = tyi * TH; x0 = txi * TW; n0 = tn * BN;
  };

  if (producer) {
    const int pw = wave - NCW;
    const int pc = lane & 7, lrow = lane >> 3;
    const int lc16_0 = (pc ^ ((0 + (lrow >> 1)) & 7)) * 16, lc16_1 = (pc ^ ((4 + (lrow >> 1)) & 7)) * 16;
    const int lc16_h = (pc ^ (((lrow >> 1) & 3) * 2)) * 16;
    const __amdgpu_buffer_rsrc_t rA0 = __builtin_amdgcn_make_buffer_rsrc((void*)p.A0, 0, (int)SENT, 0x00020000);
    const __amdgpu_buffer_rsrc_t rA1 = __builtin_amdgcn_make_buffer_rsrc((void*)(p.A1 ? p.A1 : p.A0), 0, (int)SENT, 0x00020000);
    const __amdgpu_buffer_rsrc_t rW = __builtin_amdgcn_make_buffer_rsrc((void*)p.W, 0, (int)SENT, 0x00020000);
    constexpr int ngw_max = (NG + 3) / 4;
    const int ngw = (NG - pw + 3) >> 2;
    int h_pix[HSLOTS];
    auto halo_setup = [&](int tile) {
      int t, y0, x0, n0; tile_origin(tile, t, y0, x0, n0);
#pragma unroll
      for (int k = 0; k < ngw_max; ++k) {
        const int grp = pw + 4 * k;
        const int hy = grp / GPR, hx = (grp - hy * GPR) * 8 + lrow;
        const int y = y0 - 1 + hy, x = x0 - 1 + hx;
        const bool ok = grp < NG && hx < TW + 2 && y >= 0 && y < p.Hi && x >= 0 && x < p.Wi;
        h_pix[k] = ok ? (t * p.Hi + y) * p.Wi + x : -1;
      }
    };
    auto halo_issue = [&](int k, int chunk, int hb) {
      const int cb = chunk * BK;
      const bool src0 = cb < p.C0;
      const int Cs2 = (src0 ? p.C0 : p.C1) * 2;
      const int soff = (src0 ? cb : cb - p.C0) * 2;
      const unsigned voff = h_pix[k] >= 0 ? (unsigned)h_pix[k] * (unsigned)Cs2 + (unsigned)lc16_h : SENT;
      __builtin_amdgcn_raw_ptr_buffer_load_lds(src0 ? rA0 : rA1, (lptr_t)(halo + hb * HALO + (pw + 4 * k) * 8 * BK), 16, (int)voff, soff, 0, 0);
    };
    unsigned b_off[LB];
    int ld_ti = 0, ld_ks = 0, ld_slot = 0;
    int ld_gc = 0;
    int h_tile = -1;
    auto issue = [&]() -> int {
      if (ld_ks == 0) {
        int t, y0, x0, n0; tile_origin(tw.first + ld_ti * tw.step, t, y0, x0, n0);
#pragma unroll
        for (int l = 0; l < LB; ++l) {
          const int rg = pw * LB + l;
          const int lr = rg * 8 + lrow;
          const int part = lr / WTN, rem = lr % WTN;
          const int jj = rem >> 4, i = rem & 15;
          const int n = n0 + part * WTN + (i >> 2) * WID + jj * 4 + (i & 3);
          b_off[l] = n < p.N ? (unsigned)n * (unsigned)(p.ldw * 2) + ((rg & 1) ? lc16_1 : lc16_0) : SENT;
        }
      }
      f16* Bs = ring + ld_slot * WSLOT;
      const int kt2 = ld_ks * BK * 2;
#pragma unroll
      for (int l = 0; l < LB; ++l)
        __builtin_amdgcn_raw_ptr_buffer_load_lds(rW, (lptr_t)(Bs + (pw * LB + l) * 8 * BK), 16, (int)b_off[l], kt2, 0, 0);
      int nh = 0;
      const int chunk = ld_ks / 9, sp = ld_ks - chunk * 9;
      if (sp >= 2) {
        int tchunk = chunk + 1, ttile = ld_ti;
        if (tchunk == nchunks) { tchunk = 0; ++ttile; }
        if (ttile < my_tiles) {
          if (ttile != h_tile) { halo_setup(tw.first + ttile * tw.step); h_tile = ttile; }
#pragma unroll
          for (int u = 0; u < HL; ++u) {
            const int k = (sp - 2) * HL + u;
            if (k < ngw) {
#pragma unroll
              for (int kk = 0; kk < ngw_max; ++kk) if (kk == k) halo_issue(kk, tchunk, (ld_gc + 1) & 1);
              ++nh;
            }
          }
        }
      }
      if (++ld_ks == nk) { ld_ks = 0; ++ld_ti; }
      if (ld_ks % 9 == 0) ++ld_gc;
      if (++ld_slot == 3) ld_slot = 0;
      return nh;
    };
    if (total_it > 0) {
      halo_setup(tw.first); h_tile = 0;
#pragma unroll
      for (int k = 0; k < ngw_max; ++k) if (k < ngw) halo_issue(k, 0, 0);
      issue();
    }
    if (total_it > 1) issue();
    if (total_it > 1) asm volatile("s_waitcnt vmcnt(%0)" ::"n"(LB) : "memory");
    else asm volatile("s_waitcnt vmcnt(0)" ::: "memory");
    __builtin_amdgcn_s_barrier();
    for (int fi = 0; fi < total_it; ++fi) {
      if (fi + 2 < total_it) {
        const int nh = issue();
        if (nh == 2) asm volatile("s_waitcnt vmcnt(%0)" ::"n"(LB + 2) : "memory");
        else if (nh == 1) asm volatile("s_waitcnt vmcnt(%0)" ::"n"(LB + 1) : "memory");
        else asm volatile("s_waitcnt vmcnt(%0)" ::"n"(LB) : "memory");
      } else {
        asm volatile("s_waitcnt vmcnt(0)" ::: "memory");
      }
      __builtin_amdgcn_s_barrier();
    }
    return;
  }

  const int wm = wave / WNW, wn = wave % WNW;
  f32x4 acc[MT][NT];
#pragma unroll
  for (int i = 0; i < MT; ++i)
#pragma unroll
    for (int j = 0; j < NT; ++j) acc[i][j] = (f32x4){0.f, 0.f, 0.f, 0.f};
  const int l15 = lane & 15, g = lane >> 4;
  const int sw = swz<BK>(l15);
  const int r0 = wm * WTM;
  const int hpb = (r0 >> LG) * PITCH + (r0 & (TW - 1)) + l15;
  auto DI = [](int i) constexpr { return TW >= 64 ? i * 16 : TW == 32 ? (i >> 1) * PITCH + (i & 1) * 16 : i * PITCH; };
  static_assert(TW >= 64 || (TW == 32 && WTM % 32 == 0) || TW == 16, "row-block offsets");
  int a_pre[3][2], b_pre[2];
#pragma unroll
  for (int dx = 0; dx < 3; ++dx)
#pragma unroll
    for (int kk = 0; kk < 2; ++kk) {
      const int hp = hpb + dx;
      a_pre[dx][kk] = (hp * BK + (((kk * 4 + g) ^ (((hp >> 1) & 3) * 2)) * 8)) * 2;
    }
#pragma unroll
  for (int kk = 0; kk < 2; ++kk) b_pre[kk] = ((wn * WTN + l15) * BK + (((kk * 4 + g) ^ sw) * 8)) * 2;
  const char* ringb = (const char*)ring;
  int cp_ti = 0, cp_gc = 0;
  __builtin_amdgcn_s_barrier();
  asm volatile("" ::: "memory");
  const char* Hb = nullptr;
  int ti = 0;
  bool last_chunk = false;
  const bool lean = !ST && BN != 160 && tile_epilogue_lean_ok(p, WTN, true) && !(p.tune_knobs & 8388608);
  auto step = [&](auto TAP) {
    constexpr int tap = decltype(TAP)::value;
    constexpr int dy = tap / 3, dx = tap - dy * 3;
    constexpr int slot = tap % 3;
    {
      f16x8 af[2][MT], bf[2][NT];
#pragma unroll
      for (int kk = 0; kk < 2; ++kk) {
#pragma unroll
        for (int j = 0; j < NT; ++j) bf[kk][j] = *(const f16x8*)(ringb + b_pre[kk] + (slot * WSLOT + j * 16 * BK) * 2);
#pragma unroll
        for (int i = 0; i < MT; ++i) af[kk][i] = *(const f16x8*)(Hb + a_pre[dx][kk] + (dy * PITCH + DI(i)) * BK * 2);
      }
#pragma unroll
      for (int kk = 0; kk < 2; ++kk)
#pragma unroll
        for (int i = 0; i < MT; ++i)
#pragma unroll
          for (int j = 0; j < NT; ++j)
            acc[i][j] = __builtin_amdgcn_mfma_f32_16x16x32_f16(bf[kk][j], af[kk][i], acc[i][j], 0, 0, 0);
      constexpr int R = MT + NT, Q = MT * NT;
      __builtin_amdgcn_sched_group_barrier(0x100, R, 0);
#pragma unroll
      for (int r = 0; r < R; ++r) {
        __builtin_amdgcn_sched_group_barrier(0x008, Q / R, 0);
        __builtin_amdgcn_sched_group_barrier(0x100, 1, 0);
      }
      __builtin_amdgcn_sched_group_barrier(0x008, Q - R * (Q / R), 0);
      __builtin_amdgcn_sched_group_barrier(0x008, Q, 0);
    }
    asm volatile("s_waitcnt lgkmcnt(0)" ::: "memory");
    __builtin_amdgcn_s_barrier();
    asm volatile("" ::: "memory");
    if (tap == 8 && last_chunk) {
      int t, y0, x0, n0; tile_origin(tw.first + ti * tw.step, t, y0, x0, n0);
      const int m0 = (t * p.Ho + y0) * p.Wo + x0 - p.m_off;
      if constexpr (ST) tile_epilogue_stats<MT, NT, WTM, WTN>(p, acc, m0, n0, wm, wn, lane, (t * tpf + (y0 / TH) * txn + (x0 >> LG)) * (BM / WTM) + wm);
      else if constexpr (BN != 160) { if (lean) tile_epilogue_lean<MT, NT, WTM, WTN, false, true>(p, acc, m0, n0, wm, wn, lane, 0, nullptr); else tile_epilogue<MT, NT, WTM, WTN>(p, acc, m0, n0, wm, wn, lane, 0); }
      else tile_epilogue<MT, NT, WTM, WTN>(p, acc, m0, n0, wm, wn, lane, 0);
    }
  };
  for (ti = 0; ti < my_tiles; ++ti) {
    for (int c = 0; c < nchunks; ++c, ++cp_gc) {
      Hb = (const char*)(halo + (cp_gc & 1) * HALO);
      last_chunk = c == nchunks - 1;
      step(std::integral_constant<int, 0>{}); step(std::integral_constant<int, 1>{}); step(std::integral_constant<int, 2>{});
      step(std::integral_constant<int, 3>{}); step(std::integral_constant<int, 4>{}); step(std::integral_constant<int, 5>{});
      step(std::integral_constant<int, 6>{}); step(std::integral_constant<int, 7>{}); step(std::integral_constant<int, 8>{});
    }
  }
  (void)cp_ti;
}

static bool halo_geom_ok(const GemmP& p, int bm, int lg) {
  const int tw = 1 << lg, th = bm >> lg;
  if (th < 1 || th * tw != bm || p.Wo % tw || p.Ho % th) return false;
  const long band = (long)th * p.Wo;
  return p.m_off % band == 0 && p.M % band == 0;
}
static int halo_pick_lg(const GemmP& p, int bm, int bn) {
  if (bm == 256 && bn == 160) return halo_geom_ok(p, 256, 5) ? 5 : -1;
  if (bm == 256) { for (int lg : {4, 5, 6}) if (halo_geom_ok(p, 256, lg)) return lg; return -1; }
  return halo_geom_ok(p, 192, 4) ? 4 : -1;
}

bool conv_halo_supported(const GemmP& p, int batch, int bm, int bn) {
  if (!p.conv || batch != 1 || p.kt != 1 || p.ky != 3 || p.kx != 3 || p.stride != 1 || p.ups != 1 || p.pad_t != 1 || p.pad_l != 1) return false;
  if (!p.kchunk || p.up_phase || p.splitk > 1 || p.Hi != p.Ho || p.Wi != p.Wo) return false;
  const int Cin = p.C0 + p.C1;
  if (Cin % 64 || p.C0 % 64 || p.M % bm || p.m_off % bm || p.N % 16) return false;
  const long lim = (1L << 31) - 64;
  if ((long)p.T * p.Hi * p.Wi * std::max(p.C0, p.C1) * 2 >= lim || (long)p.N * p.ldw * 2 >= lim) return false;
  if (p.m_off == 0 && p.M != p.T * p.Ho * p.Wo) return false;
  return halo_pick_lg(p, bm, bn) >= 0;
}

template <int BM, int BN, int LG, bool ST = false>
static void launch_halo_t(const GemmP& p, hipStream_t s) {
  constexpr int TW = 1 << LG, TH = BM >> LG, PITCH = (TW + 2 + 7) & ~7, NG = (TH + 2) * (PITCH / 8);
  const size_t lds = 2 * (size_t)NG * 1024 + 3 * (size_t)BN * 128;
  static bool attr[32] = {};
  bool& at = attr[ug_dev_slot()];
  if (!at) {
    UG_CHECK(hipFuncSetAttribute((const void*)conv_halo_kernel<BM, BN, LG, ST>, hipFuncAttributeMaxDynamicSharedMemorySize, 160 * 1024));
    at = true;
  }
  const int ntiles = (p.M / BM) * cdiv(p.N, BN);
  int gx = std::min(256, ntiles);
  static const bool dbg = getenv("UG_HALO_DEBUG") != nullptr;
  if (dbg) fprintf(stderr, "[halo] %dx%d M %d (m_off %d) N %d C %d+%d  %dx%d  tile %dx%d pitch %d  lds %zu  grid %d\n", BM, BN, p.M, p.m_off, p.N, p.C0, p.C1, p.Ho, p.Wo, TH, TW, PITCH, lds, gx);
  GemmP q = p; q.halo_lg = LG; q.halo_tw = TW; q.splitk = 1;
  hipLaunchKernelGGL((conv_halo_kernel<BM, BN, LG, ST>), dim3(gx), dim3(12 * 64), lds, s, q);
}

void launch_conv_halo(const GemmP& p, int bm, int bn, hipStream_t s) {
  const int lg = halo_pick_lg(p, bm, bn);
  UG_REQUIRE(lg >= 0, "halo conv: no tile geometry");
  if (p.stat_part) {
    UG_REQUIRE(bn == 128, "halo conv: epilogue statistics on 128-column tiles only");
    if (bm == 192) launch_halo_t<192, 128, 4, true>(p, s);
    else if (lg == 4) launch_halo_t<256, 128, 4, true>(p, s); else if (lg == 5) launch_halo_t<256, 128, 5, true>(p, s); else launch_halo_t<256, 128, 6, true>(p, s);
    return;
  }
  if (bm == 256 && bn == 160) launch_halo_t<256, 160, 5>(p, s);
  else if (bm == 256) { if (lg == 4) launch_halo_t<256, 128, 4>(p, s); else if (lg == 5) launch_halo_t<256, 128, 5>(p, s); else launch_halo_t<256, 128, 6>(p, s); }
  else if (bn == 160) launch_halo_t<192, 160, 4>(p, s);
  else launch_halo_t<192, 128, 4>(p, s);
}
```

### unigeo_amd/csrc/kernels/gemm.hip

```cpp
#include "../common.h"
#include <algorithm>

#include "gemm_common.h"

template <int BM, int BN, int BK, int NST, int WMW, int WNW> struct GemmOcc {
  static constexpr int lds = NST * (BM + BN) * BK * 2;
  static constexpr int wg_lds = (160 * 1024) / lds;
  static constexpr int wg = wg_lds < 1 ? 1 : (wg_lds > 4 ? 4 : wg_lds);
  static constexpr int wps_raw = wg * WMW * WNW / 4;
  static constexpr int wps = wps_raw < 1 ? 1 : (wps_raw > 4 ? 4 : wps_raw);
};

#ifdef UG_GEMM_TRACE
#define UG_STAMP(slot)                                                                                   \
  do {                                                                                                   \
    if (traced && fi >= 8 && fi < 32) {                                                                  \
      unsigned long long c_;                                                                             \
      asm volatile("s_memtime %0\n\ts_waitcnt lgkmcnt(0)" : "=s"(c_)::"memory");                         \
      if (lane == 0) tr_lds[(fi - 8) * 5 + (slot)] = (unsigned)c_;                                       \
    }                                                                                                    \
  } while (0)
#else
#define UG_STAMP(slot) do {} while (0)
#endif
// ... 1159 lines not shown
      } else if (!p.conv && t64 <= 64 && nk >= 16) {
        const int sp = (int)std::min<long>(256 / t64, nk / 5);
        if (sp >= 2) { cfg = 3; split = sp; }
      }
    }
    if (!(p.tune_knobs & 8192) && plain_epi && p.N >= 128) {
      const long t192 = (long)cdiv(p.M, 192) * cdiv(p.N, 128), t64b = (long)cdiv(p.M, 128) * cdiv(p.N, 64);
      if (p.conv && p.M > 128 && t192 <= 128 && nk >= 16 && gemm_can_bufa(p, 64, true)) {
        cfg = 63; split = (int)std::max<long>(1, std::min<long>(std::min<long>(160 / t192, nk / 8), 8));
      } else if (p.conv && p.M <= 128 && nk >= 64) {
        const int sp = (int)std::min<long>(std::min<long>(240 / t64b, nk / 7), 24);
        if (sp >= 2) { cfg = 3; split = sp; }
      } else if (!p.conv && split == 1 && nk >= 32 && t64b <= 128 && t64b > 64) split = 2;
    }
    if (!(p.tune_knobs & 2048) && plain_epi && p.M > 1024 && p.N >= 1024 && p.N < 2048 && gemm_can_bufa(p, 64, true)) {
      if (p.conv && nk >= 128) { cfg = 59; split = 4; }
      else if (p.conv && nk >= 48) { cfg = 63; split = 3; }
      else if (!p.conv && nk >= 64) { cfg = 59; split = 3; }
    }
  } else if (!(p.tune_knobs & 512) && plain_epi && p.M <= 8192 && tiles128 <= 256 && p.N >= 128 && p.N < 2048 && (p.conv ? nk >= 32 : nk >= 16)) {
    const long t192u = (long)cdiv(p.M, 192) * cdiv(p.N, 128);
    if (p.conv && !(p.tune_knobs & 8192) && t192u <= 128 && gemm_can_bufa(p, 64, true)) {
      cfg = 63; split = (int)std::max<long>(1, std::min<long>(std::min<long>(160 / t192u, nk / 8), 8));
    } else if (p.conv) {
      int sp = (int)std::min<long>(std::min<long>(512 / tiles128, nk / 8), 8);
      while (sp >= 2 && (512 / sp) < tiles128) --sp;
      cfg = 0; split = std::max(1, sp);
    } else {
      const long t64 = (long)cdiv(p.M, 128) * cdiv(p.N, 64);
      cfg = 3;
      const int sp = (int)std::min<long>(std::min<long>(512 / t64, nk / 8), 8);
      split = std::max(1, sp);
      if (!(p.tune_knobs & 8192) && t64 > 128) split = 1;
    }
  } else if (!geglu && !p.conv && p.M <= 512 && p.N >= 2048) {
    cfg = 3;
  } else if (!(p.tune_knobs & 8192) && !geglu && !p.conv && batch == 1 && p.M <= 8192 && p.K <= 384 && p.N <= 384) {
    cfg = 3;
  }
  if ((p.tune_cfg_p1 - 1) >= 0 && !(geglu && (p.tune_cfg_p1 - 1) != 0 && (p.tune_cfg_p1 - 1) != 4 && (p.tune_cfg_p1 - 1) != 8 && (p.tune_cfg_p1 - 1) != 15 && (p.tune_cfg_p1 - 1) != 35 && (p.tune_cfg_p1 - 1) != 54 && (p.tune_cfg_p1 - 1) != 62 && (p.tune_cfg_p1 - 1) != 64)) cfg = (p.tune_cfg_p1 - 1);
  if ((p.tune_split_p1 - 1) >= 0) split = plain_epi ? std::max(1, (p.tune_split_p1 - 1)) : 1;
  *cfg_out = cfg; *split_out = split;
}

static int pick_group_m(const GemmP& p, int cfg, int batch, int split) {
  if ((p.conv && (p.tune_knobs & 64)) || batch > 1 || (p.tune_knobs & 32)) return 1;
  if ((double)p.N * p.K * 2.0 <= 3.0 * (1 << 20)) return 1;
  int bm = 256, bn = 128, percu = 1;
  switch (cfg) {
    case 0: bm = 128; bn = 128; percu = 2; break;
    case 1: case 3: bm = 128; bn = 64; percu = cfg == 1 ? 3 : 2; break;
    case 12: bm = 64; bn = 64; percu = 5; break;
    case 14: case 34: bm = 256; bn = 64; percu = 2; break;
    case 15: case 35: bm = 256; bn = 256; break;
    case 60: case 70: bm = 256; bn = 160; break;
    case 61: case 62: case 63: case 64: case 72: bm = 192; bn = 128; break;
    case 73: bm = 192; bn = 160; break;
    default: break;
  }
  const int ntm = cdiv(p.M, bm), ntn = cdiv(p.N, bn);
  if (ntm < 2 || ntn < 2) return 1;
  const double P = 32.0 * percu;
  int g = 1;
  while (g * 2 <= ntm && (double)(g * 2) * (g * 2) <= P * bn / bm * 1.5) g *= 2;
  if (!(p.tune_knobs & 1048576) && (double)g * ntn <= P) g = 1;
  return g;
}

static bool cfg_geom(int cfg, int& bm, int& bn, int& wmw, int& wnw) {
  switch (cfg) {
    case 0: bm = 128; bn = 128; wmw = 2; wnw = 2; return true;
    case 1: case 3: bm = 128; bn = 64; wmw = 2; wnw = 2; return true;
    case 4: case 8: case 54: bm = 256; bn = 128; wmw = 4; wnw = 2; return true;
    case 12: bm = 64; bn = 64; wmw = 2; wnw = 2; return true;
    case 14: case 34: bm = 256; bn = 64; wmw = 4; wnw = 2; return true;
    case 15: case 35: bm = 256; bn = 256; wmw = 2; wnw = 4; return true;
    case 19: case 39: case 59: bm = 256; bn = 128; wmw = 2; wnw = 4; return true;
    case 61: case 63: bm = 192; bn = 128; wmw = 2; wnw = 4; return true;
    case 62: case 64: bm = 192; bn = 128; wmw = 4; wnw = 2; return true;
    default: return false;
  }
}

void launch_gemm(const GemmP& p0, int batch, hipStream_t s, int* stat_rb) {
  GemmP p = p0;
  if (stat_rb) *stat_rb = 0;
  if (!stat_rb) p.stat_part = nullptr;
  if (p.tune_knobs & 2) p.flags |= UG_F_NOXCD;
  if (p.tune_knobs & 128) p.flags |= UG_F_XCDROUND;
  if (p.tune_knobs & 16) p.flags |= UG_F_PRIO;
  UG_REQUIRE(p.K % 8 == 0, "GEMM K must be a multiple of 8");
  UG_REQUIRE(p.ldw % 8 == 0, "GEMM ldw must be a multiple of 8");
  UG_REQUIRE(p.M > 0 && p.N > 0 && p.K > 0, "empty GEMM");
  UG_REQUIRE(p.zero != nullptr, "zero page missing");
  UG_REQUIRE(p.nb_inner >= 1, "nb_inner");
  if (p.flags & UG_F_GEGLU) UG_REQUIRE(p.N % 128 == 0, "GEGLU GEMM needs N % 128 == 0");
  if (p.conv) {
    UG_REQUIRE(p.C0 % 8 == 0 && p.C1 % 8 == 0, "conv channel counts must be multiples of 8");
    UG_REQUIRE(p.K == (p.C0 + p.C1) * p.kt * p.ky * p.kx, "conv K mismatch");
    UG_REQUIRE(p.M == p.T * p.Ho * p.Wo && p.m_off == 0, "conv M mismatch");
    UG_REQUIRE(p.ups == 1 || p.ups == 2, "ups");
  } else {
    UG_REQUIRE(p.C0 % 8 == 0, "dense lda must be a multiple of 8");
  }
  int cfg = p.cfg_p1 - 1, split = p.splitk;
  if (cfg < 0 || split < 1) { int c2, s2; gemm_plan(p, batch, &c2, &s2); if (cfg < 0) cfg = c2; if (split < 1) split = s2; }
  if (p.flags & UG_F_GEGLU) UG_REQUIRE(cfg == 0 || cfg == 4 || cfg == 8 || cfg == 15 || cfg == 35 || cfg == 54 || cfg == 62 || cfg == 64, "GEGLU needs a 64-column wave tile");
  p.splitk = split;
  bool planned = p0.cfg_p1 == 0;
  if (!planned && (p.tune_cfg_p1 - 1) < 0) { int c2, s2; gemm_plan(p0, batch, &c2, &s2); planned = (c2 == cfg && s2 == split); }
  const bool halo_on = planned && !(p.tune_knobs & 16384) && split == 1 && (p.tune_cfg_p1 - 1) < 0 && !(p.flags & UG_F_GEGLU);
  const bool halo_l0 = halo_on && p.N % 160 == 0 && p.N <= 320 && p.C1 == 0 && !(p.tune_knobs & 32768) && conv_halo_supported(p, batch, 256, 128);
  if (!halo_l0 && planned && p.conv && p.kt == 1 && p.ky == 3 && p.kx == 3 && p.N % 160 == 0 && p.N <= 320 && split == 1 && batch == 1 && !p.up_phase && !(p.flags & (UG_F_OUT_F32 | UG_F_GEGLU)) &&
      (p.tune_cfg_p1 - 1) < 0 && !(p.tune_knobs & 1024) && gemm_can_bufa(p, 64, true)) {
    const long ntn = p.N / 160, tiles = (long)cdiv(p.M, 256) * ntn, whole = tiles / 256 * 256, rem = tiles - whole;
    if (whole > 0 && rem > 0 && rem * 2 <= 256) {
      const int M1 = (int)(whole / ntn) * 256;
      const bool halo = false;
      GemmP a = p; a.M = M1; a.cfg_p1 = 61;
      a.stat_part = nullptr;
      GemmP b = p0; b.stat_part = nullptr; b.M = p.M - M1; b.m_off = M1; b.Out = (void*)((f16*)p.Out + (long)M1 * p.ldo);
      b.flags |= p.flags & (UG_F_NOXCD | UG_F_XCDROUND);
      if (b.R1) b.R1 += (long)M1 * p.ldr1;
      if (b.R2) b.R2 += (long)M1 * p.ldr2;
      int cb, sb; gemm_plan(b, 1, &cb, &sb);
      if (cb != 59 && cb != 60 && cb != 63 && cb != 64 && cb != 54) cb = 63;
      b.cfg_p1 = cb + 1; b.splitk = 1;
      a.splitk = 1;
      a.group_m = pick_group_m(a, 60, 1, 1); a.tm_T = a.tm_nb = 0;
      launch_cfg(halo && conv_halo_supported(a, 1, 256, 160) ? 70 : 60, a, 1, s);
      if (halo && conv_halo_supported(b, 1, 256, 160)) cb = 70;
      b.group_m = pick_group_m(b, cb, 1, 1); b.tm_T = b.tm_nb = 0;
      launch_cfg(cb, b, 1, s);
      UG_CHECK(hipGetLastError());
      return;
    }
  }
  if (halo_on) {
    int best = -1; double bfill = 0.0;
    for (int c = 70; c <= 73; ++c) {
      const int bm = c <= 71 ? 256 : 192, bn = (c == 70 || c == 73) ? 160 : 128;
      if (!conv_halo_supported(p, batch, bm, bn)) continue;
      const long tiles = (long)(p.M / bm) * cdiv(p.N, bn);
      const double useful = (double)p.N / (cdiv(p.N, bn) * bn);
      const double fill = (double)tiles / (cdiv(tiles, 256) * 256.0) * useful * (bm == 256 ? 1.0 : 0.97);
      if (fill > bfill) { bfill = fill; best = c; }
    }
    if (halo_l0) best = 71;
    else if (p.N % 160 == 0 && p.N <= 320) best = -1;
    if (best >= 0) cfg = best;
  }
  if (planned && !(p.tune_knobs & 65536) && (p.tune_cfg_p1 - 1) < 0 && split == 1 && gemm_stream_supported(p, batch)) {
    cfg = 80;
  }
  if (split > 1) UG_REQUIRE(p.partial != nullptr, "split-K needs a partial buffer");
  p.group_m = pick_group_m(p, cfg, batch, split);
  p.tm_T = p.tm_nb = 0;
  if (p.conv && p.kt > 1 && p.T > 1 && batch == 1 && !(p.tune_knobs & 256)) {
    int bm = 256;
    switch (cfg) { case 0: case 1: case 3: bm = 128; break; case 12: bm = 64; break; case 61: case 62: case 63: case 64: bm = 192; break; default: break; }
    const long hw = (long)p.Ho * p.Wo;
    if (hw % bm == 0 && hw / bm >= 1) { p.tm_T = p.T; p.tm_nb = (int)(hw / bm); }
  }
  if (p.stat_part) {
    int bm = 0, wmw = 0;
    {
      int gbm, gbn, gwm, gwn;
      const bool sym = (cfg == 14 || cfg == 19) && p.conv && gemm_can_bufa(p, 64, false) && !(p.tune_knobs & 4);
      const bool pk = (cfg == 35 || cfg == 54 || cfg == 59 || cfg == 63 || cfg == 64) && p.conv && gemm_can_bufa(p, 64, true);
      if (cfg == 71) { bm = 256; wmw = 4; }
      else if (cfg == 72) { bm = 192; wmw = 4; }
      else if ((sym || pk) && cfg_geom(cfg, gbm, gbn, gwm, gwn)) { bm = gbm; wmw = gwm; }
    }
    const int wtm = bm ? bm / wmw : 0;
    const bool ok = bm && split == 1 && batch == 1 && !(p.flags & (UG_F_GEGLU | UG_F_OUT_F32 | UG_F_R1_F32)) && !p.up_phase && !(p.tune_knobs & 131072) &&
                    p.M % bm == 0 && p.m_off == 0 && p.stat_hw > 0 && p.stat_hw % wtm == 0 && p.N % 16 == 0 && p.ldo % 8 == 0 &&
                    (!p.R1 || p.ldr1 % 8 == 0) && (!p.R2 || p.ldr2 % 8 == 0);
    static const bool sdbg = getenv("UG_STAT_DEBUG") != nullptr;
    if (sdbg) fprintf(stderr, "[stat] M %d N %d K %d conv %d kt %d hw %d cfg %d split %d -> rb %d\n", p.M, p.N, p.K, p.conv, p.kt, p.stat_hw, cfg, split, ok ? wtm : 0);
    if (ok) *stat_rb = wtm; else p.stat_part = nullptr;
  }
  launch_cfg(cfg, p, batch, s);
  if (split > 1) {
    const long nvec = (long)p.M * (p.N / 8);
    int grid = (int)std::min<long>((nvec + 255) / 256, 256 * 8);
    hipLaunchKernelGGL(splitk_epilogue, dim3(grid), dim3(256), 0, s, p);
  }
  UG_CHECK(hipGetLastError());
}
```

### unigeo_amd/csrc/kernels/gemm_common.h

```cpp
#pragma once
#include "../common.h"
#include <type_traits>

typedef const __attribute__((address_space(1))) void* gptr_t;
typedef __attribute__((address_space(3))) void* lptr_t;

__device__ __forceinline__ float erf_as(float x) {
  const float ax = fabsf(x);
  const float t = __frcp_rn(1.0f + 0.3275911f * ax);
  const float y = ((((1.061405429f * t - 1.453152027f) * t + 1.421413741f) * t - 0.284496736f) * t + 0.254829592f) * t;
  const float r = 1.0f - y * __expf(-ax * ax);
  return copysignf(r, x);
}
__device__ __forceinline__ float gelu_f(float x) { return 0.5f * x * (1.0f + erf_as(x * 0.70710678118654752f)); }
__device__ __forceinline__ float silu_f(float x) { return x * __builtin_amdgcn_rcpf(1.0f + __expf(-x)); }

typedef float f32x2 __attribute__((ext_vector_type(2)));
__device__ __forceinline__ f32x2 geglu2(f32x2 h, f32x2 g) {
  const f32x2 ag = {__builtin_fabsf(g.x), __builtin_fabsf(g.y)};
  const f32x2 u = ag * 0.23164189f + 1.0f;
  const f32x2 t = {__builtin_amdgcn_rcpf(u.x), __builtin_amdgcn_rcpf(u.y)};
  f32x2 y = t * 0.5307027145f - 0.7265760135f;
  y = y * t + 0.7107068705f;
  y = y * t - 0.142248368f;
  y = y * t + 0.127414796f;
  y = y * t;
  const f32x2 w = (g * g) * -0.72134752044f;
  const f32x2 e = {__builtin_amdgcn_exp2f(w.x), __builtin_amdgcn_exp2f(w.y)};
  const f32x2 q = 0.5f - y * e;
  const f32x2 phi = {0.5f + __builtin_copysignf(q.x, g.x), 0.5f + __builtin_copysignf(q.y, g.y)};
  return h * g * phi;
}

template <int BK> __device__ __forceinline__ int swz(int row) {
  if (BK == 64) return (row >> 1) & 7;
  else return (row >> 2) & 3;
}

__device__ __forceinline__ void tile_coord(int tile, int ntm, int ntn, int group_m, int& tm, int& tn) {
  if (group_m <= 1) { tm = tile / ntn; tn = tile - tm * ntn; return; }
  const int per = group_m * ntn;
  const int grp = tile / per, local = tile - grp * per;
  const int first = grp * group_m;
  const int gm = min(ntm - first, group_m);
  tn = local / gm;
  tm = first + (local - tn * gm);
}
__device__ __forceinline__ void tile_coord_p(const GemmP& p, int tile, int ntm, int ntn, int& tm, int& tn) {
  tile_coord(tile, ntm, ntn, p.group_m, tm, tn);
  if (p.tm_T) { const int q = tm / p.tm_T; tm = (tm - q * p.tm_T) * p.tm_nb + q; }
}

struct TileWalk { int first, step, count; };
__device__ __forceinline__ TileWalk tile_walk(int flags, int ntiles, int nwg, int w) {
  TileWalk t;
  if (nwg % 8 != 0 || (flags & UG_F_NOXCD)) { t.first = w; t.step = nwg; t.count = (ntiles - w + nwg - 1) / nwg; return t; }
  const int x = w & 7, j = w >> 3, npx = nwg >> 3;
  if (flags & UG_F_XCDROUND) { t.first = x * npx + j; t.step = nwg; t.count = (ntiles - t.first + nwg - 1) / nwg; return t; }
  const int lo = (int)(((long)x * ntiles) >> 3), hi = (int)(((long)(x + 1) * ntiles) >> 3);
  t.first = lo + j; t.step = npx; t.count = max(0, (hi - lo - j + npx - 1) / npx);
  return t;
}

template <int N> struct HVec;
template <> struct HVec<8> { typedef f16x8 type; };
template <> struct HVec<4> { typedef f16x4 type; };

template <int MT, int NT> struct EpiPre {
  static constexpr int WID = 4 * NT, CH = (WID % 8 == 0) ? 8 : 4, NV = WID / CH;
  typedef typename HVec<CH>::type hvec;
  hvec b1[NV], b2[NV];
  hvec r1[MT][NV];
};
template <int MT, int NT, int WTM, int WTN>
__device__ __forceinline__ void epi_pre_cols(const GemmP& p, int n0, int wn, int lane, EpiPre<MT, NT>& pre) {
  typedef EpiPre<MT, NT> P;
  typedef typename P::hvec hvec;
  const int g = lane >> 4;
  const int nb = n0 + wn * WTN + g * P::WID;
  if (nb + P::WID > p.N) return;
  if (p.bias) {
#pragma unroll
    for (int v = 0; v < P::NV; ++v) pre.b1[v] = *(const hvec*)(p.bias + nb + v * P::CH);
  }
  if (p.bias2) {
#pragma unroll
    for (int v = 0; v < P::NV; ++v) pre.b2[v] = *(const hvec*)(p.bias2 + nb + v * P::CH);
  }
}
__device__ __forceinline__ bool epi_pre_r1_ok(const GemmP& p) {
  return p.R1 && !(p.flags & (UG_F_R1_F32 | UG_F_GEGLU)) && (p.ldo & 7) == 0 && (p.ldr1 & 7) == 0 && (!p.R2 || (p.ldr2 & 7) == 0);
}
template <int MT, int NT, int WTM, int WTN>
__device__ __forceinline__ void epi_pre_rows(const GemmP& p, int m0, int n0, int wm, int wn, int lane, EpiPre<MT, NT>& pre) {
  typedef EpiPre<MT, NT> P;
  typedef typename P::hvec hvec;
  const int l15 = lane & 15, g = lane >> 4;
  const int nb = n0 + wn * WTN + g * P::WID;
// ... 381 lines not shown
```

### unigeo_amd/csrc/kernels/norm.hip

```cpp
#include "../common.h"
#include <algorithm>
#include <cstdlib>
#include <type_traits>

#define GN_THREADS 256
#define GN_MAXV 3

__device__ __forceinline__ float silu_f(float x) { return x * __builtin_amdgcn_rcpf(1.0f + __expf(-x)); }

struct GnGeom { int nvec, tpr, rpi, vpt; };
static __host__ __device__ inline GnGeom gn_geom(int C) {
  GnGeom g;
  g.nvec = C / 8;
  if (g.nvec <= GN_THREADS) { g.tpr = g.nvec; g.rpi = GN_THREADS / g.nvec; g.vpt = 1; }
  else { g.tpr = GN_THREADS; g.rpi = 1; g.vpt = (g.nvec + GN_THREADS - 1) / GN_THREADS; }
  return g;
}

__device__ __forceinline__ f16x8 gn_load(const GroupNormP& p, long m, int c) {
  return (c < p.C0) ? *(const f16x8*)(p.X0 + m * p.C0 + c) : *(const f16x8*)(p.X1 + m * p.C1 + (c - p.C0));
}

__device__ __forceinline__ void gn_stats_body(const GroupNormP& p, int t, int chunk, int nchunk, int rows_per_chunk, float* red) {
  const int C = p.C0 + p.C1;
  const GnGeom gg = gn_geom(C);
  const int tid = threadIdx.x;
  const int rsub = tid / gg.tpr, v0 = tid - rsub * gg.tpr;
  const bool active = rsub < gg.rpi;
  const int r0 = chunk * rows_per_chunk;
  const int r1 = min(r0 + rows_per_chunk, p.HW);
  float s[GN_MAXV][8], q[GN_MAXV][8];
#pragma unroll
  for (int k = 0; k < GN_MAXV; ++k)
#pragma unroll
    for (int e = 0; e < 8; ++e) { s[k][e] = 0.f; q[k][e] = 0.f; }
  if (active) {
    if (gg.vpt == 1) {
      const int c = v0 * 8;
      int r = r0 + rsub;
      for (; r + 3 * gg.rpi < r1; r += 4 * gg.rpi) {
        f16x8 x[4];
#pragma unroll
        for (int u = 0; u < 4; ++u) x[u] = gn_load(p, (long)t * p.HW + r + u * gg.rpi, c);
#pragma unroll
        for (int u = 0; u < 4; ++u)
#pragma unroll
          for (int e = 0; e < 8; ++e) { const float f = (float)x[u][e]; s[0][e] += f; q[0][e] += f * f; }
      }
      for (; r < r1; r += gg.rpi) {
        const f16x8 x = gn_load(p, (long)t * p.HW + r, c);
#pragma unroll
        for (int e = 0; e < 8; ++e) { const float f = (float)x[e]; s[0][e] += f; q[0][e] += f * f; }
      }
    } else
    for (int r = r0 + rsub; r < r1; r += gg.rpi) {
      const long m = (long)t * p.HW + r;
#pragma unroll
      for (int k = 0; k < GN_MAXV; ++k) {
        const int v = v0 + k * GN_THREADS;
        if (k < gg.vpt && v < gg.nvec) {
          const f16x8 x = gn_load(p, m, v * 8);
#pragma unroll
          for (int e = 0; e < 8; ++e) { const float f = (float)x[e]; s[k][e] += f; q[k][e] += f * f; }
        }
      }
    }
#pragma unroll
    for (int k = 0; k < GN_MAXV; ++k) {
      const int v = v0 + k * GN_THREADS;
      if (k < gg.vpt && v < gg.nvec) {
#pragma unroll
        for (int e = 0; e < 8; ++e) {
          red[((long)rsub * C + v * 8 + e) * 2 + 0] = s[k][e];
          red[((long)rsub * C + v * 8 + e) * 2 + 1] = q[k][e];
        }
      }
    }
  }
  __syncthreads();
  const int cpg = C / p.G;
  for (int g = tid; g < p.G; g += GN_THREADS) {
    float a = 0.f, b = 0.f;
    for (int rs = 0; rs < gg.rpi; ++rs)
      for (int c = g * cpg; c < (g + 1) * cpg; ++c) {
        a += red[((long)rs * C + c) * 2 + 0];
        b += red[((long)rs * C + c) * 2 + 1];
      }
    float* dst = p.ws + (((long)t * nchunk + chunk) * p.G + g) * 2;
    dst[0] = a; dst[1] = b;
  }
}
// ... 52 lines not shown
  const int S = p.HW / p.part_rb;
  const bool pooled = p.temporal && !FRAME_PART;
  const int tlo = pooled ? 0 : blockIdx.y, thi = pooled ? p.T : blockIdx.y + 1;
  const int nitem = (thi - tlo) * S * cpg;
  const float2* src = p.part + (long)tlo * S * C + g * cpg;
  double a = 0.0, b = 0.0;
  auto at = [&](int it) { const int bs = it / cpg, cc = it - bs * cpg; return src[(long)bs * C + cc]; };
  int it = tid;
  for (; it + 3 * NT < nitem; it += 4 * NT) {
    const float2 v0 = at(it), v1 = at(it + NT), v2 = at(it + 2 * NT), v3 = at(it + 3 * NT);
    a += (double)v0.x; b += (double)v0.y; a += (double)v1.x; b += (double)v1.y;
    a += (double)v2.x; b += (double)v2.y; a += (double)v3.x; b += (double)v3.y;
  }
  for (; it < nitem; it += NT) { const float2 v = at(it); a += (double)v.x; b += (double)v.y; }
  sa[tid] = a; sb[tid] = b;
  __syncthreads();
  for (int st = NT / 2; st > 0; st >>= 1) {
    if (tid < st) { sa[tid] += sa[tid + st]; sb[tid] += sb[tid + st]; }
    __syncthreads();
  }
  if (FRAME_PART) {
    if (tid == 0) scratch[(long)blockIdx.y * p.G + g] = make_double2(sa[0], sb[0]);
    return;
  }
  const double n = (double)cpg * p.HW * (thi - tlo);
  const double mean = sa[0] / n;
  double var = sb[0] / n - mean * mean;
  if (var < 0.0) var = 0.0;
  const float mf = (float)mean, rf = (float)(1.0 / sqrt(var + (double)p.eps));
  for (int i = tid; i < (thi - tlo) * cpg; i += NT) {
    const int t = tlo + i / cpg, c = g * cpg + i % cpg;
    const float ga = p.gamma ? (float)p.gamma[c] : 1.f, be = p.beta ? (float)p.beta[c] : 0.f;
    const float sc = rf * ga;
    ab[((long)t * C + c) * 2 + 0] = sc;
    ab[((long)t * C + c) * 2 + 1] = be - mf * sc;
  }
}
__global__ __launch_bounds__(64) void gn_finalize_pool(const GroupNormP p, const double2* scratch, float* ab) {
  const int C = p.C0, cpg = C / p.G, g = blockIdx.x, tid = threadIdx.x;
  double a = 0.0, b = 0.0;
  for (int t = 0; t < p.T; ++t) { const double2 v = scratch[(long)t * p.G + g]; a += v.x; b += v.y; }
  const double n = (double)cpg * p.HW * p.T;
  const double mean = a / n;
  double var = b / n - mean * mean;
  if (var < 0.0) var = 0.0;
  const float mf = (float)mean, rf = (float)(1.0 / sqrt(var + (double)p.eps));
  for (int i = tid; i < p.T * cpg; i += 64) {
    const int t = i / cpg, c = g * cpg + i % cpg;
    const float ga = p.gamma ? (float)p.gamma[c] : 1.f, be = p.beta ? (float)p.beta[c] : 0.f;
    const float sc = rf * ga;
    ab[((long)t * C + c) * 2 + 0] = sc;
    ab[((long)t * C + c) * 2 + 1] = be - mf * sc;
  }
}

template <bool SILU, typename F>
__device__ __forceinline__ void gn_apply_body(const GroupNormP& p, int t, int chunk, int rows_per_chunk, F coef) {
  const int C = p.C0 + p.C1;
  const GnGeom gg = gn_geom(C);
  const int tid = threadIdx.x;
  const int rsub = tid / gg.tpr, v0 = tid - rsub * gg.tpr;
  if (rsub >= gg.rpi) return;
  const int r0 = chunk * rows_per_chunk;
  const int r1 = min(r0 + rows_per_chunk, p.HW);
  float a[GN_MAXV][8], b[GN_MAXV][8];
#pragma unroll
  for (int k = 0; k < GN_MAXV; ++k) {
    const int v = v0 + k * GN_THREADS;
    if (k < gg.vpt && v < gg.nvec) {
#pragma unroll
      for (int e = 0; e < 8; ++e) {
        coef(v * 8 + e, a[k][e], b[k][e]);
      }
    }
  }
  if (gg.vpt == 1) {
    const int c = v0 * 8;
    int r = r0 + rsub;
    for (; r + 3 * gg.rpi < r1; r += 4 * gg.rpi) {
      f16x8 x[4];
#pragma unroll
      for (int u = 0; u < 4; ++u) x[u] = gn_load(p, (long)t * p.HW + r + u * gg.rpi, c);
#pragma unroll
      for (int u = 0; u < 4; ++u) {
        f16x8 y;
#pragma unroll
        for (int e = 0; e < 8; ++e) {
          float f = (float)x[u][e] * a[0][e] + b[0][e];
          if (SILU) f = silu_f(f);
          y[e] = (f16)f;
        }
        *(f16x8*)(p.Y + ((long)t * p.HW + r + u * gg.rpi) * C + c) = y;
      }
    }
    for (; r < r1; r += gg.rpi) {
      const f16x8 x = gn_load(p, (long)t * p.HW + r, c);
      f16x8 y;
#pragma unroll
      for (int e = 0; e < 8; ++e) {
        float f = (float)x[e] * a[0][e] + b[0][e];
        if (SILU) f = silu_f(f);
        y[e] = (f16)f;
      }
      *(f16x8*)(p.Y + ((long)t * p.HW + r) * C + c) = y;
    }
    return;
  }
  for (int r = r0 + rsub; r < r1; r += gg.rpi) {
    const long m = (long)t * p.HW + r;
#pragma unroll
    for (int k = 0; k < GN_MAXV; ++k) {
      const int v = v0 + k * GN_THREADS;
      if (k < gg.vpt && v < gg.nvec) {
        const f16x8 x = gn_load(p, m, v * 8);
        f16x8 y;
#pragma unroll
        for (int e = 0; e < 8; ++e) {
          float f = (float)x[e] * a[k][e] + b[k][e];
          if (SILU) f = silu_f(f);
          y[e] = (f16)f;
        }
        *(f16x8*)(p.Y + m * C + v * 8) = y;
      }
    }
  }
}

template <bool SILU>
__global__ __launch_bounds__(GN_THREADS) void gn_apply(const GroupNormP p, int rows_per_chunk, const float* ab) {
  const int C = p.C0 + p.C1, t = blockIdx.y;
  gn_apply_body<SILU>(p, t, blockIdx.x, rows_per_chunk, [&](int c, float& a, float& b) { a = ab[((long)t * C + c) * 2 + 0]; b = ab[((long)t * C + c) * 2 + 1]; });
}
static void launch_gn_apply(const GroupNormP& p, int nchunk, int rpc, const float* ab, hipStream_t s) {
  if (p.silu) hipLaunchKernelGGL(gn_apply<true>, dim3(nchunk, p.T), dim3(GN_THREADS), 0, s, p, rpc, ab);
  else hipLaunchKernelGGL(gn_apply<false>, dim3(nchunk, p.T), dim3(GN_THREADS), 0, s, p, rpc, ab);
}

__global__ __launch_bounds__(256) void gn_small(const GroupNormP p) {
  __shared__ float rs[256], rq[256];
  __shared__ float mr[2];
  const int C = p.C0 + p.C1, cpg = C / p.G, vpg = cpg / 4;
  const int g = blockIdx.x, tid = threadIdx.x;
  const long row0 = p.temporal ? 0 : (long)blockIdx.y * p.HW;
  const long rows = p.temporal ? (long)p.T * p.HW : p.HW;
  const long nitem = rows * vpg;
  auto ld = [&](long m, int c) -> f16x4 {
    return (c < p.C0) ? *(const f16x4*)(p.X0 + m * p.C0 + c) : *(const f16x4*)(p.X1 + m * p.C1 + (c - p.C0));
  };
  float s = 0.f, q = 0.f;
  for (long it = tid; it < nitem; it += 256) {
    const long r = it / vpg; const int v = (int)(it - r * vpg);
    const f16x4 x = ld(row0 + r, g * cpg + v * 4);
#pragma unroll
    for (int e = 0; e < 4; ++e) { const float f = (float)x[e]; s += f; q += f * f; }
  }
  rs[tid] = s; rq[tid] = q;
  __syncthreads();
  for (int o = 128; o > 0; o >>= 1) {
    if (tid < o) { rs[tid] += rs[tid + o]; rq[tid] += rq[tid + o]; }
    __syncthreads();
  }
  if (tid == 0) {
    const double n = (double)rows * cpg;
    const double mean = (double)rs[0] / n;
    double var = (double)rq[0] / n - mean * mean;
    if (var < 0.0) var = 0.0;
    mr[0] = (float)mean; mr[1] = (float)(1.0 / sqrt(var + (double)p.eps));
  }
  __syncthreads();
  const float mean = mr[0], rstd = mr[1];
  for (long it = tid; it < nitem; it += 256) {
    const long r = it / vpg; const int v = (int)(it - r * vpg);
    const int c = g * cpg + v * 4;
    const f16x4 x = ld(row0 + r, c);
    const f16x4 ga = *(const f16x4*)(p.gamma + c), be = *(const f16x4*)(p.beta + c);
    f16x4 y;
#pragma unroll
    for (int e = 0; e < 4; ++e) {
      const float a = rstd * (float)ga[e];
      const float f = (float)x[e] * a + ((float)be[e] - mean * a);
      y[e] = (f16)(p.silu ? silu_f(f) : f);
    }
    *(f16x4*)(p.Y + (row0 + r) * C + c) = y;
  }
}

template <int NT>
__device__ __forceinline__ float gn_block_sum(float v, float* red) {
#pragma unroll
  for (int o = 32; o > 0; o >>= 1) v += __shfl_xor(v, o);
  __syncthreads();
  if ((threadIdx.x & 63) == 0) red[threadIdx.x >> 6] = v;
  __syncthreads();
  float t = 0.f;
#pragma unroll
  for (int w = 0; w < NT / 64; ++w) t += red[w];
  return t;
}

template <int NT, int VMAX, int MODE>
__global__ __launch_bounds__(NT) void gn_slab(const GroupNormP p) {
  typedef unsigned u32x2_t __attribute__((ext_vector_type(2)));
  __shared__ float red[NT / 64];
  const int C = p.C0 + p.C1, cpg = C / p.G, vpg = cpg / 4;
  const int g = blockIdx.x, tid = threadIdx.x;
// ... 84 lines not shown
template <int MODE>
static void gn_slab_launch(const GroupNormP& p, int snt, int svmax, dim3 grid, hipStream_t s) {
  if (snt == 256) {
    if (svmax <= 4) hipLaunchKernelGGL((gn_slab<256, 4, MODE>), grid, dim3(256), 0, s, p);
    else hipLaunchKernelGGL((gn_slab<256, 8, MODE>), grid, dim3(256), 0, s, p);
  } else {
    switch (svmax) {
      case 4: hipLaunchKernelGGL((gn_slab<1024, 4, MODE>), grid, dim3(1024), 0, s, p); break;
      case 8: hipLaunchKernelGGL((gn_slab<1024, 8, MODE>), grid, dim3(1024), 0, s, p); break;
      case 16: hipLaunchKernelGGL((gn_slab<1024, 16, MODE>), grid, dim3(1024), 0, s, p); break;
      case 32: hipLaunchKernelGGL((gn_slab<1024, 32, MODE>), grid, dim3(1024), 0, s, p); break;
      default: hipLaunchKernelGGL((gn_slab<1024, 48, MODE>), grid, dim3(1024), 0, s, p); break;
    }
  }
}

static inline int gn_slab_plan(const GroupNormP& p, int& vmax, bool per_frame = false) {
  const int C = p.C0 + p.C1, cpg = C / p.G;
  const bool pooled = p.temporal && !per_frame;
  if (cpg % 4 || p.C0 % cpg || !p.gamma || !p.beta || cpg / 4 > 64) return 0;
  if ((pooled ? (long)p.T * p.HW : (long)p.HW) * C * 2 >= (1L << 31)) return 0;
  const int vpg = cpg / 4;
  const long R = pooled ? (long)p.T * p.HW : p.HW;
  for (int nt : {256, 1024}) {
    const long k = (R + nt / vpg - 1) / (nt / vpg);
    const int cap = nt == 256 ? 8 : 48;
    if (k <= cap) { vmax = k <= 4 ? 4 : k <= 8 ? 8 : k <= 16 ? 16 : k <= 32 ? 32 : 48; return nt; }
  }
  return 0;
}

static inline void gn_chunks2(int T, int HW, int C, int& nchunk, int& rpc) {
  const GnGeom gg = gn_geom(C);
  static const int total_want = getenv("UG_GN_WANT") ? atoi(getenv("UG_GN_WANT")) : 1024;
  const int want = cdiv(total_want, T);
  rpc = cdiv(HW, want);
  const int min_rpc = 4 * gg.rpi;
  if (rpc < min_rpc) rpc = min_rpc;
  nchunk = cdiv(HW, rpc);
  if (nchunk > 128) { nchunk = 128; rpc = cdiv(HW, nchunk); nchunk = cdiv(HW, rpc); }
}

size_t groupnorm_ws_floats(int T, int HW, int C, int G) {
  int nchunk, rpc;
  gn_chunks2(T, HW, C, nchunk, rpc);
  return (size_t)T * nchunk * G * 2 + (size_t)T * C * 2;
}

static int gn_pick_mode(const GroupNormP& p, int* snt_o = nullptr, int* svmax_o = nullptr, int* tnt_o = nullptr, int* tvmax_o = nullptr) {
  const int C = p.C0 + p.C1;
  const int cpg = C / p.G;
  const long slab = (long)p.HW * cpg * (p.temporal ? p.T : 1);
  const bool small_ok = !p.temporal && cpg % 4 == 0 && p.C0 % 4 == 0 && p.gamma && p.beta;
  int mode = p.mode;
  int svmax = 0, tvmax = 0;
  const int snt = gn_slab_plan(p, svmax);
  const int tnt = p.temporal ? gn_slab_plan(p, tvmax, true) : 0;
  if (mode == 0) {
    const bool narrow_ok = p.HW <= 256 || cpg >= 32;
    static const bool noslab = getenv("UG_GN_NOSLAB") != nullptr;
    static const bool not2 = getenv("UG_GN_NOT2") != nullptr;
    if (small_ok && slab <= 16384 && narrow_ok) mode = (snt && !noslab) ? 4 : 2;
    else if (!p.temporal && snt && svmax <= 16 && narrow_ok && p.G * p.T >= 256 && !noslab) mode = 4;
    else if (p.temporal && tnt && tvmax <= 16 && p.HW <= 256 && p.G * p.T >= 256 && !not2) mode = 6;
    else mode = 1;
  }
  if (mode == 4 && !snt) mode = p.temporal ? 1 : 2;
  if (mode == 2 && !small_ok) mode = 1;
  if (mode == 3) mode = 1;
  if (mode == 6 && !tnt) mode = 1;
  if (snt_o) *snt_o = snt;
  if (svmax_o) *svmax_o = svmax;
  if (tnt_o) *tnt_o = tnt;
  if (tvmax_o) *tvmax_o = tvmax;
  return mode;
}
bool groupnorm_uses_part(const GroupNormP& p0, int part_rb) {
  GroupNormP p = p0;
  if ((p.C0 + p.C1) % p.G != 0 || p.C1 != 0 || p.mode != 0 || part_rb <= 0 || p.HW % part_rb != 0) return false;
  const int mode = gn_pick_mode(p);
  return mode == 1 || mode == 6;
}

bool launch_groupnorm(const GroupNormP& p, hipStream_t s) {
  const int C = p.C0 + p.C1;
  UG_REQUIRE(p.C0 % 8 == 0 && p.C1 % 8 == 0, "GroupNorm channels must be multiples of 8");
  UG_REQUIRE(C % p.G == 0 && p.G <= 256 && 256 % p.G == 0, "GroupNorm group count must divide 256");
  UG_REQUIRE(C <= GN_MAXV * GN_THREADS * 8, "GroupNorm too many channels");
  const int cpg = C / p.G;
  int snt = 0, svmax = 0, tnt = 0, tvmax = 0;
  int mode = gn_pick_mode(p, &snt, &svmax, &tnt, &tvmax);
  if (p.part && p.mode == 0 && (mode == 1 || mode == 6)) {
    UG_REQUIRE(p.C1 == 0 && p.part_rb > 0 && p.HW % p.part_rb == 0, "GroupNorm: epilogue statistics need a single source and whole blocks per frame");
    int nchunk, rpc;
    gn_chunks2(p.T, p.HW, C, nchunk, rpc);
    float* ab = p.ws + (size_t)p.T * nchunk * p.G * 2;
    const long nitem = (long)(p.temporal ? p.T : 1) * (p.HW / p.part_rb) * cpg;
    const long per_frame = (long)(p.HW / p.part_rb) * cpg;
    if (p.temporal && p.T > 1 && per_frame >= 2048 && (size_t)p.T * p.G * 4 <= (size_t)p.T * nchunk * p.G * 2) {
      double2* scratch = (double2*)p.ws;
      hipLaunchKernelGGL(gn_finalize_cols<true>, dim3(p.G, p.T), dim3(1024), 0, s, p, ab, scratch);
      hipLaunchKernelGGL(gn_finalize_pool, dim3(p.G), dim3(64), 0, s, p, (const double2*)scratch, ab);
    } else {
      hipLaunchKernelGGL(gn_finalize_cols<false>, dim3(p.G, p.temporal ? 1 : p.T), dim3(nitem > 2048 ? 1024 : 256), 0, s, p, ab, (double2*)nullptr);
    }
    launch_gn_apply(p, nchunk, rpc, (const float*)ab, s);
    UG_CHECK(hipGetLastError());
    return true;
  }
  if (mode == 4) {
    gn_slab_launch<0>(p, snt, svmax, dim3(p.G, p.temporal ? 1 : p.T), s);
  } else if (mode == 6) {
    gn_slab_launch<1>(p, tnt, tvmax, dim3(p.G, p.T), s);
    gn_slab_launch<2>(p, tnt, tvmax, dim3(p.G, p.T), s);
  } else if (mode == 2) {
    hipLaunchKernelGGL(gn_small, dim3(p.G, p.T), dim3(256), 0, s, p);
  } else {
    int nchunk, rpc;
    gn_chunks2(p.T, p.HW, C, nchunk, rpc);
    const GnGeom gg = gn_geom(C);
    const size_t lds = (size_t)gg.rpi * C * 2 * sizeof(float);
    float* ab = p.ws + (size_t)p.T * nchunk * p.G * 2;
    hipLaunchKernelGGL(gn_stats, dim3(nchunk, p.T), dim3(GN_THREADS), lds, s, p, nchunk, rpc);
    const int fin_threads = ((p.temporal ? p.T : 1) * nchunk > 64) ? 1024 : 256;
    hipLaunchKernelGGL(gn_finalize, dim3(p.T), dim3(fin_threads), 0, s, p, nchunk, ab);
    launch_gn_apply(p, nchunk, rpc, (const float*)ab, s);
  }
  UG_CHECK(hipGetLastError());
  return false;
}

template <int VPL>
__global__ __launch_bounds__(256) void ln_kernel(const LayerNormP p) {
  const int lane = threadIdx.x & 63;
  const long row = (long)blockIdx.x * 4 + (threadIdx.x >> 6);
  if (row >= p.M) return;
  const int nvec = p.C / 8;
  float x[VPL][8];
  float sum = 0.f;
#pragma unroll
  for (int k = 0; k < VPL; ++k) {
    const int v = lane + k * 64;
    if (v < nvec) {
      const f16x8 h = *(const f16x8*)(p.X + row * p.C + v * 8);
#pragma unroll
      for (int e = 0; e < 8; ++e) x[k][e] = (float)h[e];
      if (p.addvec) {
        const f16x8 a = *(const f16x8*)(p.addvec + ((row + p.row0) / p.rows_per_vec) * p.C + v * 8);
        f16x8 o;
#pragma unroll
        for (int e = 0; e < 8; ++e) { o[e] = (f16)(x[k][e] + (float)a[e]); x[k][e] = (float)o[e]; }
        if (p.Xout) *(f16x8*)(p.Xout + row * p.C + v * 8) = o;
      }
#pragma unroll
      for (int e = 0; e < 8; ++e) sum += x[k][e];
    } else {
#pragma unroll
      for (int e = 0; e < 8; ++e) x[k][e] = 0.f;
    }
  }
#pragma unroll
  for (int o = 32; o > 0; o >>= 1) sum += __shfl_xor(sum, o);
  const float mean = sum / p.C;
  float var = 0.f;
#pragma unroll
  for (int k = 0; k < VPL; ++k) {
    const int v = lane + k * 64;
    if (v < nvec) {
#pragma unroll
      for (int e = 0; e < 8; ++e) { const float d = x[k][e] - mean; var += d * d; }
    }
  }
#pragma unroll
  for (int o = 32; o > 0; o >>= 1) var += __shfl_xor(var, o);
  const float rstd = rsqrtf(var / p.C + p.eps);
#pragma unroll
  for (int k = 0; k < VPL; ++k) {
    const int v = lane + k * 64;
    if (v < nvec) {
      const f16x8 g = *(const f16x8*)(p.gamma + v * 8);
      const f16x8 b = *(const f16x8*)(p.beta + v * 8);
      f16x8 y;
#pragma unroll
      for (int e = 0; e < 8; ++e) y[e] = (f16)((x[k][e] - mean) * rstd * (float)g[e] + (float)b[e]);
      if (!p.Y8) { *(f16x8*)(p.Y + row * p.C + v * 8) = y; continue; }
      float amax = 0.f;
#pragma unroll
      for (int e = 0; e < 8; ++e) amax = fmaxf(amax, fabsf((float)y[e]));
      amax = fmaxf(amax, __shfl_xor(amax, 1));
      amax = fmaxf(amax, __shfl_xor(amax, 2));
      int ex = 0;
      if (amax > 0.f) { (void)frexpf(amax, &ex); ex = ex - 1 - 8; }
      ex = min(max(ex, -127), 127);
      const float inv = ldexpf(1.0f, -ex);
      float t[8];
#pragma unroll
      for (int e = 0; e < 8; ++e) t[e] = fminf(fmaxf((float)y[e] * inv, -448.f), 448.f);
      int p0 = __builtin_amdgcn_cvt_pk_fp8_f32(t[0], t[1], 0, false); p0 = __builtin_amdgcn_cvt_pk_fp8_f32(t[2], t[3], p0, true);
      int p1 = __builtin_amdgcn_cvt_pk_fp8_f32(t[4], t[5], 0, false); p1 = __builtin_amdgcn_cvt_pk_fp8_f32(t[6], t[7], p1, true);
      *(uint2*)(p.Y8 + row * p.C + v * 8) = make_uint2((unsigned)p0, (unsigned)p1);
      if ((lane & 3) == 0)
        ((unsigned char*)(p.S8 + (long)(v >> 4) * p.ld_s8 + row))[(v & 15) >> 2] = (unsigned char)(ex + 127);
    }
  }
}

template <int L>
__global__ __launch_bounds__(256) void ln40_kernel(const LayerNormP p) {
  constexpr int RPW = 64 / L, NV = 5;
  const int lane = threadIdx.x & 63, sub = lane / L, l = lane % L;
  const long row = ((long)blockIdx.x * 4 + (threadIdx.x >> 6)) * RPW + sub;
  const bool ok = row < p.M;
// ... 88 lines not shown
```

Baseline: 27.92 frames/s.

## Fuse GroupNorm+SiLU apply into the 3x3 halo conv prologue in ResNet blocks

Splits GroupNorm into a stats/finalize phase and an apply phase, then folds the per-channel affine and SiLU into the A-operand load of the halo-tiled 3x3 convolution. When the conv plan qualifies, the ResNet block no longer writes and rereads a normalized copy of the activation. This removes one full activation round-trip and an apply launch per norm+conv pair. In exchange the conv inner loop does extra arithmetic per loaded element, an extra shortcut buffer is needed, and the halo tile choice is factored into a shared helper.

```diff
diff --git a/unigeo_amd/_lib.py b/unigeo_amd/_lib.py
--- a/unigeo_amd/_lib.py
+++ b/unigeo_amd/_lib.py
@@ -14,7 +14,7 @@
     "ug_load_tensor", "ug_bind_unet", "ug_bind_vae", "ug_bind_clip",
     "ug_dc_set_inputs", "ug_dc_run", "ug_dc_run_windows", "ug_dc_get_outputs", "ug_dc_device_ptrs", "ug_dc_set_trace", "ug_dc_set_guidance", "ug_unet_forward_pair", "ug_dc_set_inputs_ex", "ug_dc_get_noise", "ug_op_philox_u32", "ug_op_randn", "ug_op_u8_to_frames", "ug_set_vae_encode_fp32", "ug_set_concurrency", "ug_set_coscheduled", "ug_set_fp8_linears", "ug_op_linear_mx8", "ug_set_ff_fused", "ug_op_ff", "ug_op_ln_ff", "ug_bench_ff", "ug_bench_flash", "ug_tune_flash", "ug_tune_ff",
     "ug_eval_depth", "ug_eval_normal", "ug_depth_eval_opts_default", "ug_eval_depth_ex", "ug_op_masked_median", "ug_clip_embed", "ug_vae_encode", "ug_vae_decode", "ug_unet_forward", "ug_normals_from_depth",
-    "ug_op_linear", "ug_op_conv", "ug_op_conv_gn", "ug_op_groupnorm", "ug_op_layernorm", "ug_op_flash_attn",
+    "ug_op_linear", "ug_op_conv", "ug_op_conv_gn", "ug_op_gn_conv", "ug_op_groupnorm", "ug_op_layernorm", "ug_op_flash_attn",
     "ug_op_temporal_attn", "ug_op_attention_generic", "ug_op_flash_attn_dh", "ug_op_euler_step",
     "ug_bind_stablenormal", "ug_sn_run", "ug_sn_unet_forward", "ug_sn_dino", "ug_sn_vae_decode", "ug_sn_vae_encode", "ug_resize_bilinear",
     "ug_profile_begin", "ug_profile_begin_shapes", "ug_profile_end", "ug_bench_gemm", "ug_bench_groupnorm", "ug_bench_mfma_peak", "ug_tune_force",
@@ -122,6 +122,11 @@
     except AttributeError:
         if not os.environ.get("UG_LIB_PATH"):
             raise
+    try:
+        lib.ug_op_gn_conv.argtypes = [vp, vp, ip, vp, ip, ip, ip, ip, ip, C.c_float, vp, vp, ip, vp, vp, ip, ip, ip, vp, vp, vp, vp]
+    except AttributeError:
+        if not os.environ.get("UG_LIB_PATH"):
+            raise
     lib.ug_normals_from_depth.argtypes = [vp, vp, vp, ip, ip, ip, vp]
     lib.ug_op_linear.argtypes = [vp, vp, ip, ip, vp, ip, vp, vp, C.c_float, C.c_float, ip, ip, vp]
     lib.ug_op_conv.argtypes = [vp, vp, ip, vp, ip, ip, ip, ip, vp, vp, ip, ip, ip, ip, ip, ip, ip, vp]
@@ -562,6 +567,18 @@
                                         _ptr(_f32(gamma)), _ptr(_f32(beta)), _ptr(co), _ptr(y1), _ptr(y2), C.byref(rb)))
         return co, y1, y2, rb.value
 
+    def op_gn_conv(self, x0, G, eps, gamma, beta, w, b=None, x1=None, gn_mode=0, halo_grid=0, want_stats=False):
+        x0 = _f32(x0); T, H, W, C0 = x0.shape
+        x1a = None if x1 is None else _f32(x1); C1 = 0 if x1 is None else x1a.shape[-1]
+        w = _f32(w); O = w.shape[0]
+        out = np.empty((T, H, W, O), np.float32)
+        M = T * H * W
+        part = np.zeros(((M + 47) // 48, O, 2), np.float32)
+        rb = C.c_int(0); fused = C.c_int(0)
+        self._ck(self.lib.ug_op_gn_conv(self.ctx, _ptr(x0), C0, _ptr(x1a), C1, T, H, W, G, eps, _ptr(_f32(gamma)), _ptr(_f32(beta)), int(gn_mode), _ptr(w),
+                                        _ptr(None if b is None else _f32(b)), O, int(halo_grid), int(want_stats), _ptr(out), _ptr(part), C.byref(rb), C.byref(fused)))
+        return out, bool(fused.value), (part[:M // rb.value].copy() if rb.value > 0 else None), rb.value
+
     def op_layernorm(self, x, eps, gamma, beta, addvec=None, rows_per_vec=1):
         x = _f32(x); M, Cc = x.shape
         out = np.empty((M, Cc), np.float32); xout = np.empty((M, Cc), np.float32)
diff --git a/unigeo_amd/csrc/capi.hip b/unigeo_amd/csrc/capi.hip
--- a/unigeo_amd/csrc/capi.hip
+++ b/unigeo_amd/csrc/capi.hip
@@ -867,6 +867,47 @@
   });
 }
 
+int ug_op_gn_conv(ug_ctx* x, const float* x0, int C0, const float* x1, int C1, int T, int H, int W, int G, float eps, const float* gamma, const float* beta,
+                  int gn_mode, const float* weight, const float* bias, int O, int halo_grid, int want_stats, float* out, float* part_out, int* rb_out, int* fused_out) {
+  UG_TRY(x, {
+    Ctx& c = x->c; Scope sc(c);
+    const int I = C0 + C1, taps = 9;
+    UG_REQUIRE(I % 64 == 0, "ug_op_gn_conv: channels must be a multiple of 64");
+    std::vector<float> wp((size_t)O * taps * I);
+    for (int o = 0; o < O; ++o) for (int i = 0; i < I; ++i) for (int tp = 0; tp < taps; ++tp)
+      wp[(((size_t)o * (I / 64) + i / 64) * taps + tp) * 64 + i % 64] = weight[((size_t)o * I + i) * taps + tp];
+    const long M = (long)T * H * W;
+    f16* d0 = up16(c, x0, M * C0); f16* d1 = C1 ? up16(c, x1, M * C1) : nullptr;
+    f16* dW = up16(c, wp.data(), (long)wp.size()); f16* db = up16_opt(c, bias, O);
+    f16* dg = up16(c, gamma, I); f16* dbt = up16(c, beta, I);
+    f16* dO = c.ws.get<f16>(M * O);
+    float2* part = want_stats ? (float2*)c.ws.get<float>(((M + 47) / 48) * (long)O * 2) : nullptr;
+    GroupNormP g; memset(&g, 0, sizeof(g));
+    g.X0 = d0; g.X1 = d1; g.C0 = C0; g.C1 = C1; g.T = T; g.HW = H * W; g.G = G; g.eps = eps; g.silu = 1; g.gamma = dg; g.beta = dbt; g.mode = gn_mode;
+    g.ws = c.ws.get<float>((long)groupnorm_ws_floats(T, H * W, I, G));
+    GemmP p; memset(&p, 0, sizeof(p));
+    p.conv = 1; p.A0 = d0; p.A1 = d1; p.C0 = C0; p.C1 = C1; p.T = T; p.Hi = H; p.Wi = W; p.Ho = H; p.Wo = W;
+    p.ups = 1; p.stride = 1; p.pad_t = 1; p.pad_l = 1; p.kt = 1; p.ky = 3; p.kx = 3;
+    p.M = (int)M; p.N = O; p.K = I * taps; p.W = dW; p.ldw = p.K; p.bias = db; p.c0 = 1.f;
+    p.Out = dO; p.ldo = O; p.zero = c.zero; p.nb_inner = 1; p.kchunk = 1; p.halo_grid = halo_grid;
+    gemm_apply_tune(p, c.tune);
+    { int cf, sp; gemm_plan(p, 1, &cf, &sp); p.cfg_p1 = cf + 1; p.splitk = sp; if (sp > 1) p.partial = c.ws.get<float>((long)sp * p.M * p.N); }
+    const bool fused = !(c.tune.knobs & 33554432) && I % G == 0 && groupnorm_splits(g) && conv_gn_fusable(p, 1);
+    if (fused) {
+      p.gn_ab = launch_groupnorm_stats(g, c.stream);
+    } else {
+      g.Y = c.ws.get<f16>(M * I);
+      launch_groupnorm(g, c.stream);
+      p.A0 = g.Y; p.A1 = nullptr; p.C0 = I; p.C1 = 0;
+    }
+    int rb = 0;
+    if (want_stats) { p.stat_part = part; p.stat_hw = H * W; launch_gemm(p, 1, c.stream, &rb); } else launch_gemm(p, 1, c.stream);
+    down16(c, dO, out, M * O);
+    if (want_stats && rb > 0) UG_CHECK(hipMemcpy(part_out, part, (size_t)(M / rb) * O * 2 * sizeof(float), hipMemcpyDeviceToHost));
+    *rb_out = rb; *fused_out = fused ? 1 : 0;
+  });
+}
+
 int ug_op_groupnorm(ug_ctx* x, const float* x0, int C0, const float* x1, int C1, int T, int HW, int G, float eps,
                     int temporal, int silu, const float* gamma, const float* beta, float* out) {
   UG_TRY(x, {
diff --git a/unigeo_amd/csrc/common.h b/unigeo_amd/csrc/common.h
--- a/unigeo_amd/csrc/common.h
+++ b/unigeo_amd/csrc/common.h
@@ -27,6 +27,19 @@
       throw std::runtime_error(std::string("requirement failed: ") + #cond + " : " + (msg) + \
                                " at " + __FILE__ + ":" + std::to_string(__LINE__));           \
   } while (0)
+
+__device__ __forceinline__ float silu_f(float x) { return x * __builtin_amdgcn_rcpf(1.0f + __expf(-x)); }
+template <bool SILU>
+__device__ __forceinline__ f16x8 gn_affine_act8(const f16x8 x, const float* a, const float* b) {
+  f16x8 y;
+#pragma unroll
+  for (int e = 0; e < 8; ++e) {
+    float f = (float)x[e] * a[e] + b[e];
+    if (SILU) f = silu_f(f);
+    y[e] = (f16)f;
+  }
+  return y;
+}
 
 static inline int cdiv(long a, long b) { return (int)((a + b - 1) / b); }
 static inline int ug_dev_slot() { int d = 0; (void)hipGetDevice(&d); return d & 31; }
@@ -67,6 +80,8 @@
   int halo_tw, halo_lg;
   int tune_cfg_p1, tune_split_p1, tune_knobs;
   float2* stat_part; int stat_hw;
+  const float* gn_ab;
+  int halo_grid;
 };
 struct GemmTune { int cfg = -1, split = -1, knobs = 0; };
 static inline void gemm_apply_tune(GemmP& p, const GemmTune& t) { p.tune_cfg_p1 = t.cfg + 1; p.tune_split_p1 = t.split + 1; p.tune_knobs = t.knobs; }
@@ -78,6 +93,8 @@
 bool conv_halo_supported(const GemmP& p, int batch, int bm, int bn);
 void launch_conv_halo(const GemmP& p, int bm, int bn, hipStream_t s);
 void gemm_plan(const GemmP& p, int batch, int* cfg_out, int* split_out);
+bool conv_halo_gn_supported(int bm, int bn);
+bool conv_gn_fusable(const GemmP& p, int batch);
 
 struct FFusedP {
   const f16* X; const f16* W1; const f16* b1; const f16* W2; const f16* b2;
@@ -101,6 +118,8 @@
 bool launch_groupnorm(const GroupNormP& p, hipStream_t s);
 bool groupnorm_uses_part(const GroupNormP& p, int part_rb);
 size_t groupnorm_ws_floats(int T, int HW, int C, int G);
+bool groupnorm_splits(const GroupNormP& p);
+const float* launch_groupnorm_stats(const GroupNormP& p, hipStream_t s, bool* from_part = nullptr);
 
 struct LayerNormP {
   const f16* X; f16* Y; int M, C; float eps;
diff --git a/unigeo_amd/csrc/engine.hip b/unigeo_amd/csrc/engine.hip
--- a/unigeo_amd/csrc/engine.hip
+++ b/unigeo_amd/csrc/engine.hip
@@ -180,6 +180,7 @@
   const unsigned char* a8 = nullptr; const unsigned* sa8 = nullptr; long ld_sa8 = 0;
   float alg = 1.f;
   struct StatPart* so = nullptr; int stat_hw = 0;
+  const float* gn_ab = nullptr;
 };
 struct StatPart { float2* part = nullptr; int rb = 0; };
 static StatPart stat_alloc(Ctx& c, long M, int N, int T, int hw, int G, int temporal) {
@@ -196,7 +197,7 @@
   gemm_apply_tune(p, c.tune);
   if (p.nb_inner < 1) p.nb_inner = 1;
   char nm[128];
-  if (c.prof_on && c.prof_shapes) snprintf(nm, sizeof(nm), "%s:%dx%dx%d%s", tag, p.M, p.N, p.K, batch > 1 ? "b" : "");
+  if (c.prof_on && c.prof_shapes) snprintf(nm, sizeof(nm), "%s:%dx%dx%d%s%s", tag, p.M, p.N, p.K, batch > 1 ? "b" : "", p.gn_ab ? ":gn" : "");
   else snprintf(nm, sizeof(nm), "%s", tag);
   int cfg, split;
   gemm_plan(p, batch, &cfg, &split);
@@ -275,6 +276,20 @@
   run_gemm(c, p, 1, "gemm_linear", e.alg, e.so, e.stat_hw);
 }
 
+static GemmP conv_params(const f16* x0, int C0, const f16* x1, int C1, int T, int Hi, int Wi, const Conv& cv,
+                         int stride, int pad_t, int pad_l, int ups, f16* out, const Epi& e, long ldo) {
+  GemmP p; memset(&p, 0, sizeof(p));
+  p.conv = 1; p.A0 = x0; p.A1 = x1; p.C0 = C0; p.C1 = C1;
+  p.T = T; p.Hi = Hi; p.Wi = Wi; p.ups = ups; p.stride = stride; p.pad_t = pad_t; p.pad_l = pad_l;
+  p.kt = cv.kt; p.ky = cv.ky; p.kx = cv.kx;
+  p.Ho = (Hi * ups) / stride; p.Wo = (Wi * ups) / stride;
+  p.M = T * p.Ho * p.Wo; p.N = cv.cout; p.K = cv.cinp * cv.kt * cv.ky * cv.kx;
+  p.W = cv.w; p.ldw = p.K; p.bias = cv.b; p.bias2 = e.bias2;
+  p.R1 = e.R1; p.ldr1 = e.ldr1 ? e.ldr1 : cv.cout; p.c1 = e.c1;
+  p.R2 = e.R2; p.ldr2 = e.ldr2 ? e.ldr2 : cv.cout; p.c2 = e.c2; p.c0 = e.c0; p.act = e.act; p.flags = e.flags;
+  p.Out = out; p.ldo = ldo ? ldo : cv.cout; p.kchunk = cv.kchunk; p.gn_ab = e.gn_ab;
+  return p;
+}
 static void conv(Ctx& c, const f16* x0, int C0, const f16* x1, int C1, int T, int Hi, int Wi, const Conv& cv,
                  int stride, int pad_t, int pad_l, int ups, f16* out, const Epi& e = Epi(), long ldo = 0) {
   UG_REQUIRE(C0 + C1 == cv.cinp, "conv input channels do not match the bound weight");
@@ -292,26 +307,15 @@
     }
     return;
   }
-  GemmP p; memset(&p, 0, sizeof(p));
-  p.conv = 1; p.A0 = x0; p.A1 = x1; p.C0 = C0; p.C1 = C1;
-  p.T = T; p.Hi = Hi; p.Wi = Wi; p.ups = ups; p.stride = stride; p.pad_t = pad_t; p.pad_l = pad_l;
-  p.kt = cv.kt; p.ky = cv.ky; p.kx = cv.kx;
-  p.Ho = (Hi * ups) / stride; p.Wo = (Wi * ups) / stride;
-  p.M = T * p.Ho * p.Wo; p.N = cv.cout; p.K = cv.cinp * cv.kt * cv.ky * cv.kx;
-  p.W = cv.w; p.ldw = p.K; p.bias = cv.b; p.bias2 = e.bias2;
-  p.R1 = e.R1; p.ldr1 = e.ldr1 ? e.ldr1 : cv.cout; p.c1 = e.c1;
-  p.R2 = e.R2; p.ldr2 = e.ldr2 ? e.ldr2 : cv.cout; p.c2 = e.c2; p.c0 = e.c0; p.act = e.act; p.flags = e.flags;
-  p.Out = out; p.ldo = ldo ? ldo : cv.cout; p.kchunk = cv.kchunk;
+  GemmP p = conv_params(x0, C0, x1, C1, T, Hi, Wi, cv, stride, pad_t, pad_l, ups, out, e, ldo);
   run_gemm(c, p, 1, cv.kt > 1 ? "gemm_tconv" : (cv.ky > 1 ? "gemm_conv3x3" : "gemm_conv1x1"), e.alg, e.so);
 }
 
+static GroupNormP groupnorm_params(const f16* x0, int C0, const f16* x1, int C1, int T, int HW, int G, const Norm& n, int temporal, int silu, f16* y, const struct StatPart* sp);
 static void groupnorm(Ctx& c, const f16* x0, int C0, const f16* x1, int C1, int T, int HW, int G, const Norm& n,
                       int temporal, int silu, f16* y, const StatPart* sp = nullptr) {
   UG_REQUIRE(C0 + C1 == n.c, "groupnorm channel mismatch");
-  GroupNormP p; memset(&p, 0, sizeof(p));
-  if (sp && sp->part && sp->rb > 0 && C1 == 0 && HW % sp->rb == 0) { p.part = sp->part; p.part_rb = sp->rb; }
-  p.X0 = x0; p.X1 = x1; p.C0 = C0; p.C1 = C1; p.T = T; p.HW = HW; p.G = G; p.eps = n.eps;
-  p.temporal = temporal; p.silu = silu; p.gamma = n.g; p.beta = n.b; p.Y = y;
+  GroupNormP p = groupnorm_params(x0, C0, x1, C1, T, HW, G, n, temporal, silu, y, sp);
   const size_t mk = c.ws.mark();
   p.ws = c.ws.get<float>((long)groupnorm_ws_floats(T, HW, n.c, G));
   {
@@ -323,6 +327,37 @@
     if (from_part && ps.idx >= 0 && c.prof_shapes) c.prof[ps.idx].name += ":ep";
   }
   c.ws.release(mk);
+}
+
+static GroupNormP groupnorm_params(const f16* x0, int C0, const f16* x1, int C1, int T, int HW, int G, const Norm& n, int temporal, int silu, f16* y, const StatPart* sp) {
+  GroupNormP p; memset(&p, 0, sizeof(p));
+  if (sp && sp->part && sp->rb > 0 && C1 == 0 && HW % sp->rb == 0) { p.part = sp->part; p.part_rb = sp->rb; }
+  p.X0 = x0; p.X1 = x1; p.C0 = C0; p.C1 = C1; p.T = T; p.HW = HW; p.G = G; p.eps = n.eps;
+  p.temporal = temporal; p.silu = silu; p.gamma = n.g; p.beta = n.b; p.Y = y;
+  return p;
+}
+static bool gn_conv_fusable(Ctx& c, const f16* x0, int C0, const f16* x1, int C1, int T, int h, int w, int G, const Norm& n, const Conv& cv, const Epi& e, const StatPart* sp) {
+  if (c.tune.knobs & 33554432) return false;
+  if (cv.kt != 1 || cv.ky != 3 || cv.kx != 3 || C0 + C1 != cv.cinp || C0 + C1 != n.c) return false;
+  const GroupNormP g = groupnorm_params(x0, C0, x1, C1, T, h * w, G, n, 0, 1, nullptr, sp);
+  if (g.C0 % 8 || g.C1 % 8 || (C0 + C1) % G || !groupnorm_splits(g)) return false;
+  GemmP p = conv_params(x0, C0, x1, C1, T, h, w, cv, 1, 1, 1, 1, nullptr, e, 0);
+  p.zero = c.zero; gemm_apply_tune(p, c.tune); p.nb_inner = 1;
+  int cfg, split; gemm_plan(p, 1, &cfg, &split);
+  p.cfg_p1 = cfg + 1; p.splitk = split;
+  return conv_gn_fusable(p, 1);
+}
+static const float* groupnorm_stats(Ctx& c, const f16* x0, int C0, const f16* x1, int C1, int T, int HW, int G, const Norm& n, const StatPart* sp) {
+  GroupNormP p = groupnorm_params(x0, C0, x1, C1, T, HW, G, n, 0, 1, nullptr, sp);
+  p.ws = c.ws.get<float>((long)groupnorm_ws_floats(T, HW, n.c, G));
+  char nm[96];
+  if (c.prof_on && c.prof_shapes) snprintf(nm, sizeof(nm), "groupnorm_stats:T%dxHW%dxC%d", T, HW, n.c);
+  else snprintf(nm, sizeof(nm), "groupnorm");
+  ProfScope ps(c, nm, 0, (double)T * HW * n.c * 2.0 * (p.part ? 0.0 : 1.0));
+  bool from_part = false;
+  const float* ab = launch_groupnorm_stats(p, c.stream, &from_part);
+  if (from_part && ps.idx >= 0 && c.prof_shapes) c.prof[ps.idx].name += ":ep";
+  return ab;
 }
 
 struct QAct { unsigned char* a8 = nullptr; unsigned* sa = nullptr; long ld = 0; };
@@ -825,22 +860,39 @@
   const long M = (long)T * h * w;
   const int cin = C0 + C1, cout = r.c1.cout;
   const size_t mk = c.ws.mark();
-  f16* a = c.ws.get<f16>(M * cin);
-  groupnorm(c, x0, C0, x1, C1, T, h * w, G, r.n1, 0, 1, a, C1 == 0 ? in_stats : nullptr);
   f16* hb = c.ws.get<f16>(M * cout);
   StatPart sh = stat_alloc(c, M, cout, T, h * w, G, 0);
-  { Epi e; e.bias2 = tproj; e.so = &sh; conv(c, a, cin, nullptr, 0, T, h, w, r.c1, 1, 1, 1, 1, hb, e); }
-  f16* b = c.ws.get<f16>(M * cout);
-  groupnorm(c, hb, cout, nullptr, 0, T, h * w, G, r.n2, 0, 1, b, &sh);
+  {
+    Epi e; e.bias2 = tproj; e.so = &sh;
+    const StatPart* sp1 = C1 == 0 ? in_stats : nullptr;
+    if (gn_conv_fusable(c, x0, C0, x1, C1, T, h, w, G, r.n1, r.c1, e, sp1)) {
+      const size_t mk1 = c.ws.mark();
+      e.gn_ab = groupnorm_stats(c, x0, C0, x1, C1, T, h * w, G, r.n1, sp1);
+      conv(c, x0, C0, x1, C1, T, h, w, r.c1, 1, 1, 1, 1, hb, e);
+      c.ws.release(mk1);
+    } else {
+      const size_t mk1 = c.ws.mark();
+      f16* a = c.ws.get<f16>(M * cin);
+      groupnorm(c, x0, C0, x1, C1, T, h * w, G, r.n1, 0, 1, a, sp1);
+      conv(c, a, cin, nullptr, 0, T, h, w, r.c1, 1, 1, 1, 1, hb, e);
+      c.ws.release(mk1);
+    }
+  }
+  Epi e2; e2.so = out_stats; e2.R1 = x0; e2.ldr1 = cout;
+  const bool fuse2 = gn_conv_fusable(c, hb, cout, nullptr, 0, T, h, w, G, r.n2, r.c2, e2, &sh);
+  f16* b = nullptr;
+  if (fuse2) e2.gn_ab = groupnorm_stats(c, hb, cout, nullptr, 0, T, h * w, G, r.n2, &sh);
+  else { b = c.ws.get<f16>(M * cout); groupnorm(c, hb, cout, nullptr, 0, T, h * w, G, r.n2, 0, 1, b, &sh); }
   const f16* res = x0;
   if (r.has_sc) {
-    f16* scb = hb;
+    f16* scb = fuse2 ? c.ws.get<f16>(M * cout) : hb;
     conv(c, x0, C0, x1, C1, T, h, w, r.sc, 1, 0, 0, 1, scb);
     res = scb;
   } else {
     UG_REQUIRE(C1 == 0, "identity shortcut needs a single source");
   }
-  { Epi e; e.R1 = res; e.ldr1 = cout; e.so = out_stats; conv(c, b, cout, nullptr, 0, T, h, w, r.c2, 1, 1, 1, 1, out, e); }
+  e2.R1 = res; e2.ldr1 = cout;
+  conv(c, fuse2 ? hb : b, cout, nullptr, 0, T, h, w, r.c2, 1, 1, 1, 1, out, e2);
   c.ws.release(mk);
 }
 
diff --git a/unigeo_amd/csrc/kernels/conv_halo.hip b/unigeo_amd/csrc/kernels/conv_halo.hip
--- a/unigeo_amd/csrc/kernels/conv_halo.hip
+++ b/unigeo_amd/csrc/kernels/conv_halo.hip
@@ -3,7 +3,7 @@
 #include <cstdlib>
 #include <type_traits>
 
-template <int BM, int BN, int LG, bool ST = false>
+template <int BM, int BN, int LG, bool ST = false, bool GN = false>
 __global__ __launch_bounds__(12 * 64, 3) void conv_halo_kernel(const GemmP p) {
   constexpr int BK = 64, NCW = 8, WMW = 4, WNW = 2;
   constexpr unsigned SENT = 0x80000000u;
@@ -20,7 +20,8 @@
   constexpr int HL = 2;
   constexpr int HSLOTS = 7 * HL;
   static_assert(TH * TW == BM && TW >= 16 && (NG + 3) / 4 <= HSLOTS, "tile geometry");
-  static_assert((2 * HALO + 3 * WSLOT) * 2 <= 160 * 1024, "LDS");
+  constexpr int COEFW = 2 * BK;
+  static_assert((2 * HALO + 3 * WSLOT) * 2 + (GN ? 4 * COEFW * 4 : 0) <= 160 * 1024, "LDS");
   extern __shared__ __attribute__((aligned(16))) f16 smem[];
   f16* halo = smem;
   f16* ring = smem + 2 * HALO;
@@ -55,11 +56,16 @@
     const __amdgpu_buffer_rsrc_t rA0 = __builtin_amdgcn_make_buffer_rsrc((void*)p.A0, 0, (int)SENT, 0x00020000);
     const __amdgpu_buffer_rsrc_t rA1 = __builtin_amdgcn_make_buffer_rsrc((void*)(p.A1 ? p.A1 : p.A0), 0, (int)SENT, 0x00020000);
     const __amdgpu_buffer_rsrc_t rW = __builtin_amdgcn_make_buffer_rsrc((void*)p.W, 0, (int)SENT, 0x00020000);
+    const __amdgpu_buffer_rsrc_t rAB = __builtin_amdgcn_make_buffer_rsrc((void*)(GN ? (const void*)p.gn_ab : (const void*)p.W), 0, (int)SENT, 0x00020000);
+    float* coefw = (float*)(ring + 3 * WSLOT) + pw * COEFW;
+    float ca[8], cb[8];
+    int h_t = 0;
     constexpr int ngw_max = (NG + 3) / 4;
     const int ngw = (NG - pw + 3) >> 2;
     int h_pix[HSLOTS];
     auto halo_setup = [&](int tile) {
       int t, y0, x0, n0; tile_origin(tile, t, y0, x0, n0);
+      h_t = t;
 #pragma unroll
       for (int k = 0; k < ngw_max; ++k) {
         const int grp = pw + 4 * k;
@@ -77,6 +83,27 @@
       const unsigned voff = h_pix[k] >= 0 ? (unsigned)h_pix[k] * (unsigned)Cs2 + (unsigned)lc16_h : SENT;
       __builtin_amdgcn_raw_ptr_buffer_load_lds(src0 ? rA0 : rA1, (lptr_t)(halo + hb * HALO + (pw + 4 * k) * 8 * BK), 16, (int)voff, soff, 0, 0);
     };
+    auto coef_issue = [&](int chunk) {
+      const int soff = (h_t * Cin + chunk * BK) * 2 * 4;
+      __builtin_amdgcn_raw_ptr_buffer_load_lds(rAB, (lptr_t)coefw, 4, lane * 4, soff, 0, 0);
+      __builtin_amdgcn_raw_ptr_buffer_load_lds(rAB, (lptr_t)(coefw + 64), 4, lane * 4, soff + 256, 0, 0);
+    };
+    auto coef_read = [&]() {
+      const f32x4* cp = (const f32x4*)(coefw + lc16_h);
+#pragma unroll
+      for (int q = 0; q < 4; ++q) {
+        const f32x4 v = cp[q];
+        ca[2 * q] = v[0]; cb[2 * q] = v[1]; ca[2 * q + 1] = v[2]; cb[2 * q + 1] = v[3];
+      }
+    };
+    auto halo_transform = [&](int k, int hb) {
+      if (h_pix[k] >= 0) {
+        f16x8* hp = (f16x8*)(halo + hb * HALO + (pw + 4 * k) * 8 * BK + lane * 8);
+        *hp = gn_affine_act8<true>(*hp, ca, cb);
+      }
+    };
+    int pend_k0 = 0, pend_n = 0, pend_hb = 0;
+    bool pend_coef = false;
     unsigned b_off[LB];
     int ld_ti = 0, ld_ks = 0, ld_slot = 0;
     int ld_gc = 0;
@@ -96,16 +123,20 @@
       }
       f16* Bs = ring + ld_slot * WSLOT;
       const int kt2 = ld_ks * BK * 2;
+      const int chunk = ld_ks / 9, sp = ld_ks - chunk * 9;
+      int tchunk = chunk + 1, ttile = ld_ti;
+      if (tchunk == nchunks) { tchunk = 0; ++ttile; }
+      if (sp == 2 && ttile < my_tiles) {
+        if (ttile != h_tile) { halo_setup(tw.first + ttile * tw.step); h_tile = ttile; }
+        if constexpr (GN) { coef_issue(tchunk); pend_coef = true; }
+      }
 #pragma unroll
       for (int l = 0; l < LB; ++l)
         __builtin_amdgcn_raw_ptr_buffer_load_lds(rW, (lptr_t)(Bs + (pw * LB + l) * 8 * BK), 16, (int)b_off[l], kt2, 0, 0);
       int nh = 0;
-      const int chunk = ld_ks / 9, sp = ld_ks - chunk * 9;
       if (sp >= 2) {
-        int tchunk = chunk + 1, ttile = ld_ti;
-        if (tchunk == nchunks) { tchunk = 0; ++ttile; }
         if (ttile < my_tiles) {
-          if (ttile != h_tile) { halo_setup(tw.first + ttile * tw.step); h_tile = ttile; }
+          pend_k0 = (sp - 2) * HL; pend_hb = (ld_gc + 1) & 1;
 #pragma unroll
           for (int u = 0; u < HL; ++u) {
             const int k = (sp - 2) * HL + u;
@@ -115,6 +146,7 @@
               ++nh;
             }
           }
+          pend_n = nh;
         }
       }
       if (++ld_ks == nk) { ld_ks = 0; ++ld_ti; }
@@ -124,6 +156,7 @@
     };
     if (total_it > 0) {
       halo_setup(tw.first); h_tile = 0;
+      if constexpr (GN) coef_issue(0);
 #pragma unroll
       for (int k = 0; k < ngw_max; ++k) if (k < ngw) halo_issue(k, 0, 0);
       issue();
@@ -131,8 +164,19 @@
     if (total_it > 1) issue();
     if (total_it > 1) asm volatile("s_waitcnt vmcnt(%0)" ::"n"(LB) : "memory");
     else asm volatile("s_waitcnt vmcnt(0)" ::: "memory");
+    if constexpr (GN) {
+      if (total_it > 0) {
+        coef_read();
+#pragma unroll
+        for (int k = 0; k < ngw_max; ++k) if (k < ngw) halo_transform(k, 0);
+        asm volatile("s_waitcnt lgkmcnt(0)" ::: "memory");
+      }
+    }
     __builtin_amdgcn_s_barrier();
     for (int fi = 0; fi < total_it; ++fi) {
+      const int tk0 = pend_k0, tn = pend_n, thb = pend_hb;
+      const bool tcoef = pend_coef;
+      pend_n = 0; pend_coef = false;
       if (fi + 2 < total_it) {
         const int nh = issue();
         if (nh == 2) asm volatile("s_waitcnt vmcnt(%0)" ::"n"(LB + 2) : "memory");
@@ -140,6 +184,18 @@
         else asm volatile("s_waitcnt vmcnt(%0)" ::"n"(LB) : "memory");
       } else {
         asm volatile("s_waitcnt vmcnt(0)" ::: "memory");
+      }
+      if constexpr (GN) {
+        if (tcoef) coef_read();
+        if (tn > 0) {
+#pragma unroll
+          for (int u = 0; u < HL; ++u)
+            if (u < tn) {
+#pragma unroll
+              for (int kk = 0; kk < ngw_max; ++kk) if (kk == tk0 + u) halo_transform(kk, thb);
+            }
+          asm volatile("s_waitcnt lgkmcnt(0)" ::: "memory");
+        }
       }
       __builtin_amdgcn_s_barrier();
     }
@@ -252,35 +308,49 @@
   return halo_pick_lg(p, bm, bn) >= 0;
 }
 
-template <int BM, int BN, int LG, bool ST = false>
+bool conv_halo_gn_supported(int bm, int bn) { return (bm == 256 && bn == 128) || (bm == 192 && (bn == 128 || bn == 160)); }
+
+template <int BM, int BN, int LG, bool ST = false, bool GN = false>
 static void launch_halo_t(const GemmP& p, hipStream_t s) {
   constexpr int TW = 1 << LG, TH = BM >> LG, PITCH = (TW + 2 + 7) & ~7, NG = (TH + 2) * (PITCH / 8);
-  const size_t lds = 2 * (size_t)NG * 1024 + 3 * (size_t)BN * 128;
+  const size_t lds = 2 * (size_t)NG * 1024 + 3 * (size_t)BN * 128 + (GN ? 4 * 512 : 0);
   static bool attr[32] = {};
   bool& at = attr[ug_dev_slot()];
   if (!at) {
-    UG_CHECK(hipFuncSetAttribute((const void*)conv_halo_kernel<BM, BN, LG, ST>, hipFuncAttributeMaxDynamicSharedMemorySize, 160 * 1024));
+    UG_CHECK(hipFuncSetAttribute((const void*)conv_halo_kernel<BM, BN, LG, ST, GN>, hipFuncAttributeMaxDynamicSharedMemorySize, 160 * 1024));
     at = true;
   }
   const int ntiles = (p.M / BM) * cdiv(p.N, BN);
   int gx = std::min(256, ntiles);
+  if (p.halo_grid > 0) gx = std::min(gx, p.halo_grid);
   static const bool dbg = getenv("UG_HALO_DEBUG") != nullptr;
   if (dbg) fprintf(stderr, "[halo] %dx%d M %d (m_off %d) N %d C %d+%d  %dx%d  tile %dx%d pitch %d  lds %zu  grid %d\n", BM, BN, p.M, p.m_off, p.N, p.C0, p.C1, p.Ho, p.Wo, TH, TW, PITCH, lds, gx);
   GemmP q = p; q.halo_lg = LG; q.halo_tw = TW; q.splitk = 1;
-  hipLaunchKernelGGL((conv_halo_kernel<BM, BN, LG, ST>), dim3(gx), dim3(12 * 64), lds, s, q);
+  hipLaunchKernelGGL((conv_halo_kernel<BM, BN, LG, ST, GN>), dim3(gx), dim3(12 * 64), lds, s, q);
+}
+
+template <bool GN>
+static void launch_conv_halo_g(const GemmP& p, int bm, int bn, int lg, hipStream_t s) {
+  if (p.stat_part) {
+    UG_REQUIRE(bn == 128, "halo conv: epilogue statistics on 128-column tiles only");
+    if (bm == 192) launch_halo_t<192, 128, 4, true, GN>(p, s);
+    else if (lg == 4) launch_halo_t<256, 128, 4, true, GN>(p, s); else if (lg == 5) launch_halo_t<256, 128, 5, true, GN>(p, s); else launch_halo_t<256, 128, 6, true, GN>(p, s);
+    return;
+  }
+  if (bm == 256 && bn == 160) { if constexpr (GN) UG_REQUIRE(false, "halo conv: the 256 x 160 tile has no fused-GroupNorm variant"); else launch_halo_t<256, 160, 5>(p, s); }
+  else if (bm == 256) { if (lg == 4) launch_halo_t<256, 128, 4, false, GN>(p, s); else if (lg == 5) launch_halo_t<256, 128, 5, false, GN>(p, s); else launch_halo_t<256, 128, 6, false, GN>(p, s); }
+  else if (bn == 160) launch_halo_t<192, 160, 4, false, GN>(p, s);
+  else launch_halo_t<192, 128, 4, false, GN>(p, s);
 }
 
 void launch_conv_halo(const GemmP& p, int bm, int bn, hipStream_t s) {
   const int lg = halo_pick_lg(p, bm, bn);
   UG_REQUIRE(lg >= 0, "halo conv: no tile geometry");
-  if (p.stat_part) {
-    UG_REQUIRE(bn == 128, "halo conv: epilogue statistics on 128-column tiles only");
-    if (bm == 192) launch_halo_t<192, 128, 4, true>(p, s);
-    else if (lg == 4) launch_halo_t<256, 128, 4, true>(p, s); else if (lg == 5) launch_halo_t<256, 128, 5, true>(p, s); else launch_halo_t<256, 128, 6, true>(p, s);
-    return;
-  }
-  if (bm == 256 && bn == 160) launch_halo_t<256, 160, 5>(p, s);
-  else if (bm == 256) { if (lg == 4) launch_halo_t<256, 128, 4>(p, s); else if (lg == 5) launch_halo_t<256, 128, 5>(p, s); else launch_halo_t<256, 128, 6>(p, s); }
-  else if (bn == 160) launch_halo_t<192, 160, 4>(p, s);
-  else launch_halo_t<192, 128, 4>(p, s);
-}
+  if (p.gn_ab) {
+    UG_REQUIRE(conv_halo_gn_supported(bm, bn), "halo conv: no fused-GroupNorm variant of this tile");
+    UG_REQUIRE((long)p.T * (p.C0 + p.C1) * 8 < (1L << 31) && ((uintptr_t)p.gn_ab & 15) == 0, "halo conv: scale / shift array");
+    launch_conv_halo_g<true>(p, bm, bn, lg, s);
+  } else {
+    launch_conv_halo_g<false>(p, bm, bn, lg, s);
+  }
+}
diff --git a/unigeo_amd/csrc/kernels/gemm.hip b/unigeo_amd/csrc/kernels/gemm.hip
--- a/unigeo_amd/csrc/kernels/gemm.hip
+++ b/unigeo_amd/csrc/kernels/gemm.hip
@@ -1265,6 +1265,42 @@
   }
 }
 
+static int halo_choice(const GemmP& p, const GemmP& p0, int batch, int cfg, int split, bool* planned_o, bool* halo_l0_o) {
+  bool planned = p0.cfg_p1 == 0;
+  if (!planned && (p.tune_cfg_p1 - 1) < 0) { int c2, s2; gemm_plan(p0, batch, &c2, &s2); planned = (c2 == cfg && s2 == split); }
+  const bool halo_on = planned && !(p.tune_knobs & 16384) && split == 1 && (p.tune_cfg_p1 - 1) < 0 && !(p.flags & UG_F_GEGLU);
+  const bool halo_l0 = halo_on && p.N % 160 == 0 && p.N <= 320 && p.C1 == 0 && !(p.tune_knobs & 32768) && conv_halo_supported(p, batch, 256, 128);
+  if (planned_o) *planned_o = planned;
+  if (halo_l0_o) *halo_l0_o = halo_l0;
+  if (!halo_on) return -1;
+  int best = -1; double bfill = 0.0;
+  for (int c = 70; c <= 73; ++c) {
+    const int bm = c <= 71 ? 256 : 192, bn = (c == 70 || c == 73) ? 160 : 128;
+    if (!conv_halo_supported(p, batch, bm, bn)) continue;
+    const long tiles = (long)(p.M / bm) * cdiv(p.N, bn);
+    const double useful = (double)p.N / (cdiv(p.N, bn) * bn);
+    const double fill = (double)tiles / (cdiv(tiles, 256) * 256.0) * useful * (bm == 256 ? 1.0 : 0.97);
+    if (fill > bfill) { bfill = fill; best = c; }
+  }
+  if (halo_l0) best = 71;
+  else if (p.N % 160 == 0 && p.N <= 320) best = -1;
+  return best;
+}
+static void halo_cfg_tile(int c, int& bm, int& bn) { bm = c <= 71 ? 256 : 192; bn = (c == 70 || c == 73) ? 160 : 128; }
+
+bool conv_gn_fusable(const GemmP& p0, int batch) {
+  if (!p0.conv) return false;
+  GemmP p = p0;
+  int cfg = p.cfg_p1 - 1, split = p.splitk;
+  if (cfg < 0 || split < 1) { int c2, s2; gemm_plan(p, batch, &c2, &s2); if (cfg < 0) cfg = c2; if (split < 1) split = s2; }
+  p.splitk = split;
+  const int best = halo_choice(p, p0, batch, cfg, split, nullptr, nullptr);
+  if (best >= 0) cfg = best;
+  if (cfg < 70 || cfg > 73) return false;
+  int bm, bn; halo_cfg_tile(cfg, bm, bn);
+  return conv_halo_supported(p, batch, bm, bn) && conv_halo_gn_supported(bm, bn);
+}
+
 void launch_gemm(const GemmP& p0, int batch, hipStream_t s, int* stat_rb) {
   GemmP p = p0;
   if (stat_rb) *stat_rb = 0;
@@ -1290,10 +1326,12 @@
   if (cfg < 0 || split < 1) { int c2, s2; gemm_plan(p, batch, &c2, &s2); if (cfg < 0) cfg = c2; if (split < 1) split = s2; }
   if (p.flags & UG_F_GEGLU) UG_REQUIRE(cfg == 0 || cfg == 4 || cfg == 8 || cfg == 15 || cfg == 35 || cfg == 54 || cfg == 62 || cfg == 64, "GEGLU needs a 64-column wave tile");
   p.splitk = split;
-  bool planned = p0.cfg_p1 == 0;
-  if (!planned && (p.tune_cfg_p1 - 1) < 0) { int c2, s2; gemm_plan(p0, batch, &c2, &s2); planned = (c2 == cfg && s2 == split); }
-  const bool halo_on = planned && !(p.tune_knobs & 16384) && split == 1 && (p.tune_cfg_p1 - 1) < 0 && !(p.flags & UG_F_GEGLU);
-  const bool halo_l0 = halo_on && p.N % 160 == 0 && p.N <= 320 && p.C1 == 0 && !(p.tune_knobs & 32768) && conv_halo_supported(p, batch, 256, 128);
+  bool planned = false, halo_l0 = false;
+  const int halo_best = halo_choice(p, p0, batch, cfg, split, &planned, &halo_l0);
+  if (p.gn_ab) {
+    const int hc = halo_best >= 0 ? halo_best : cfg;
+    UG_REQUIRE(hc >= 70 && hc <= 73, "GemmP::gn_ab: this convolution does not run on a halo tile (conv_gn_fusable is the rule)");
+  }
   if (!halo_l0 && planned && p.conv && p.kt == 1 && p.ky == 3 && p.kx == 3 && p.N % 160 == 0 && p.N <= 320 && split == 1 && batch == 1 && !p.up_phase && !(p.flags & (UG_F_OUT_F32 | UG_F_GEGLU)) &&
       (p.tune_cfg_p1 - 1) < 0 && !(p.tune_knobs & 1024) && gemm_can_bufa(p, 64, true)) {
     const long ntn = p.N / 160, tiles = (long)cdiv(p.M, 256) * ntn, whole = tiles / 256 * 256, rem = tiles - whole;
@@ -1319,20 +1357,7 @@
       return;
     }
   }
-  if (halo_on) {
-    int best = -1; double bfill = 0.0;
-    for (int c = 70; c <= 73; ++c) {
-      const int bm = c <= 71 ? 256 : 192, bn = (c == 70 || c == 73) ? 160 : 128;
-      if (!conv_halo_supported(p, batch, bm, bn)) continue;
-      const long tiles = (long)(p.M / bm) * cdiv(p.N, bn);
-      const double useful = (double)p.N / (cdiv(p.N, bn) * bn);
-      const double fill = (double)tiles / (cdiv(tiles, 256) * 256.0) * useful * (bm == 256 ? 1.0 : 0.97);
-      if (fill > bfill) { bfill = fill; best = c; }
-    }
-    if (halo_l0) best = 71;
-    else if (p.N % 160 == 0 && p.N <= 320) best = -1;
-    if (best >= 0) cfg = best;
-  }
+  if (halo_best >= 0) cfg = halo_best;
   if (planned && !(p.tune_knobs & 65536) && (p.tune_cfg_p1 - 1) < 0 && split == 1 && gemm_stream_supported(p, batch)) {
     cfg = 80;
   }
diff --git a/unigeo_amd/csrc/kernels/gemm_common.h b/unigeo_amd/csrc/kernels/gemm_common.h
--- a/unigeo_amd/csrc/kernels/gemm_common.h
+++ b/unigeo_amd/csrc/kernels/gemm_common.h
@@ -13,7 +13,6 @@
   return copysignf(r, x);
 }
 __device__ __forceinline__ float gelu_f(float x) { return 0.5f * x * (1.0f + erf_as(x * 0.70710678118654752f)); }
-__device__ __forceinline__ float silu_f(float x) { return x * __builtin_amdgcn_rcpf(1.0f + __expf(-x)); }
 
 typedef float f32x2 __attribute__((ext_vector_type(2)));
 __device__ __forceinline__ f32x2 geglu2(f32x2 h, f32x2 g) {
diff --git a/unigeo_amd/csrc/kernels/norm.hip b/unigeo_amd/csrc/kernels/norm.hip
--- a/unigeo_amd/csrc/kernels/norm.hip
+++ b/unigeo_amd/csrc/kernels/norm.hip
@@ -6,7 +6,6 @@
 #define GN_THREADS 256
 #define GN_MAXV 3
 
-__device__ __forceinline__ float silu_f(float x) { return x * __builtin_amdgcn_rcpf(1.0f + __expf(-x)); }
 
 struct GnGeom { int nvec, tpr, rpi, vpt; };
 static __host__ __device__ inline GnGeom gn_geom(int C) {
@@ -225,27 +224,11 @@
 #pragma unroll
       for (int u = 0; u < 4; ++u) x[u] = gn_load(p, (long)t * p.HW + r + u * gg.rpi, c);
 #pragma unroll
-      for (int u = 0; u < 4; ++u) {
-        f16x8 y;
-#pragma unroll
-        for (int e = 0; e < 8; ++e) {
-          float f = (float)x[u][e] * a[0][e] + b[0][e];
-          if (SILU) f = silu_f(f);
-          y[e] = (f16)f;
-        }
-        *(f16x8*)(p.Y + ((long)t * p.HW + r + u * gg.rpi) * C + c) = y;
-      }
+      for (int u = 0; u < 4; ++u) *(f16x8*)(p.Y + ((long)t * p.HW + r + u * gg.rpi) * C + c) = gn_affine_act8<SILU>(x[u], a[0], b[0]);
     }
     for (; r < r1; r += gg.rpi) {
       const f16x8 x = gn_load(p, (long)t * p.HW + r, c);
-      f16x8 y;
-#pragma unroll
-      for (int e = 0; e < 8; ++e) {
-        float f = (float)x[e] * a[0][e] + b[0][e];
-        if (SILU) f = silu_f(f);
-        y[e] = (f16)f;
-      }
-      *(f16x8*)(p.Y + ((long)t * p.HW + r) * C + c) = y;
+      *(f16x8*)(p.Y + ((long)t * p.HW + r) * C + c) = gn_affine_act8<SILU>(x, a[0], b[0]);
     }
     return;
   }
@@ -256,14 +239,7 @@
       const int v = v0 + k * GN_THREADS;
       if (k < gg.vpt && v < gg.nvec) {
         const f16x8 x = gn_load(p, m, v * 8);
-        f16x8 y;
-#pragma unroll
-        for (int e = 0; e < 8; ++e) {
-          float f = (float)x[e] * a[k][e] + b[k][e];
-          if (SILU) f = silu_f(f);
-          y[e] = (f16)f;
-        }
-        *(f16x8*)(p.Y + m * C + v * 8) = y;
+        *(f16x8*)(p.Y + m * C + v * 8) = gn_affine_act8<SILU>(x, a[k], b[k]);
       }
     }
   }
@@ -514,19 +490,18 @@
   return mode == 1 || mode == 6;
 }
 
-bool launch_groupnorm(const GroupNormP& p, hipStream_t s) {
+static void gn_check(const GroupNormP& p) {
   const int C = p.C0 + p.C1;
   UG_REQUIRE(p.C0 % 8 == 0 && p.C1 % 8 == 0, "GroupNorm channels must be multiples of 8");
   UG_REQUIRE(C % p.G == 0 && p.G <= 256 && 256 % p.G == 0, "GroupNorm group count must divide 256");
   UG_REQUIRE(C <= GN_MAXV * GN_THREADS * 8, "GroupNorm too many channels");
-  const int cpg = C / p.G;
-  int snt = 0, svmax = 0, tnt = 0, tvmax = 0;
-  int mode = gn_pick_mode(p, &snt, &svmax, &tnt, &tvmax);
-  if (p.part && p.mode == 0 && (mode == 1 || mode == 6)) {
+}
+static float* gn_stats_finalize(const GroupNormP& p, bool from_part, int& nchunk, int& rpc, hipStream_t s) {
+  const int C = p.C0 + p.C1, cpg = C / p.G;
+  gn_chunks2(p.T, p.HW, C, nchunk, rpc);
+  float* ab = p.ws + (size_t)p.T * nchunk * p.G * 2;
+  if (from_part) {
     UG_REQUIRE(p.C1 == 0 && p.part_rb > 0 && p.HW % p.part_rb == 0, "GroupNorm: epilogue statistics need a single source and whole blocks per frame");
-    int nchunk, rpc;
-    gn_chunks2(p.T, p.HW, C, nchunk, rpc);
-    float* ab = p.ws + (size_t)p.T * nchunk * p.G * 2;
     const long nitem = (long)(p.temporal ? p.T : 1) * (p.HW / p.part_rb) * cpg;
     const long per_frame = (long)(p.HW / p.part_rb) * cpg;
     if (p.temporal && p.T > 1 && per_frame >= 2048 && (size_t)p.T * p.G * 4 <= (size_t)p.T * nchunk * p.G * 2) {
@@ -536,7 +511,24 @@
     } else {
       hipLaunchKernelGGL(gn_finalize_cols<false>, dim3(p.G, p.temporal ? 1 : p.T), dim3(nitem > 2048 ? 1024 : 256), 0, s, p, ab, (double2*)nullptr);
     }
-    launch_gn_apply(p, nchunk, rpc, (const float*)ab, s);
+    return ab;
+  }
+  const GnGeom gg = gn_geom(C);
+  const size_t lds = (size_t)gg.rpi * C * 2 * sizeof(float);
+  hipLaunchKernelGGL(gn_stats, dim3(nchunk, p.T), dim3(GN_THREADS), lds, s, p, nchunk, rpc);
+  const int fin_threads = ((p.temporal ? p.T : 1) * nchunk > 64) ? 1024 : 256;
+  hipLaunchKernelGGL(gn_finalize, dim3(p.T), dim3(fin_threads), 0, s, p, nchunk, ab);
+  return ab;
+}
+
+bool launch_groupnorm(const GroupNormP& p, hipStream_t s) {
+  gn_check(p);
+  int snt = 0, svmax = 0, tnt = 0, tvmax = 0;
+  int mode = gn_pick_mode(p, &snt, &svmax, &tnt, &tvmax);
+  if (p.part && p.mode == 0 && (mode == 1 || mode == 6)) {
+    int nchunk, rpc;
+    const float* ab = gn_stats_finalize(p, true, nchunk, rpc, s);
+    launch_gn_apply(p, nchunk, rpc, ab, s);
     UG_CHECK(hipGetLastError());
     return true;
   }
@@ -549,17 +541,26 @@
     hipLaunchKernelGGL(gn_small, dim3(p.G, p.T), dim3(256), 0, s, p);
   } else {
     int nchunk, rpc;
-    gn_chunks2(p.T, p.HW, C, nchunk, rpc);
-    const GnGeom gg = gn_geom(C);
-    const size_t lds = (size_t)gg.rpi * C * 2 * sizeof(float);
-    float* ab = p.ws + (size_t)p.T * nchunk * p.G * 2;
-    hipLaunchKernelGGL(gn_stats, dim3(nchunk, p.T), dim3(GN_THREADS), lds, s, p, nchunk, rpc);
-    const int fin_threads = ((p.temporal ? p.T : 1) * nchunk > 64) ? 1024 : 256;
-    hipLaunchKernelGGL(gn_finalize, dim3(p.T), dim3(fin_threads), 0, s, p, nchunk, ab);
-    launch_gn_apply(p, nchunk, rpc, (const float*)ab, s);
+    const float* ab = gn_stats_finalize(p, false, nchunk, rpc, s);
+    launch_gn_apply(p, nchunk, rpc, ab, s);
   }
   UG_CHECK(hipGetLastError());
   return false;
+}
+
+bool groupnorm_splits(const GroupNormP& p) {
+  if (p.temporal || !p.silu || (p.C0 + p.C1) % p.G != 0) return false;
+  return gn_pick_mode(p) == 1;
+}
+const float* launch_groupnorm_stats(const GroupNormP& p, hipStream_t s, bool* from_part) {
+  gn_check(p);
+  UG_REQUIRE(groupnorm_splits(p), "launch_groupnorm_stats: this GroupNorm does not take the three-launch scheme");
+  const bool fp = p.part && p.mode == 0;
+  int nchunk, rpc;
+  const float* ab = gn_stats_finalize(p, fp, nchunk, rpc, s);
+  UG_CHECK(hipGetLastError());
+  if (from_part) *from_part = fp;
+  return ab;
 }
 
 template <int VPL>
```

Result: slower. 25.77 frames/s (-7.7%).
